# mrluin/TextualDegRemoval

Measured on AMD Instinct MI355X. Metric: train images/sec (512x512, bs=4/GPU), higher is better.
Workload: dtype f32 (3xbf16-split MFMA: 24-bit operand significands on the full fp32 exponent range, fp32 accumulate; unscaled gradients, no loss scale, no step-skip guard; tensors fp32 -- the MASA-encoder ResidualBlock activations / gradients as three bf16 planes whose sum IS the fp32 value, bit for bit)

## Files before the change

include/tdr.h:

```cpp
#ifndef TDR_H
#define TDR_H
#include <stdint.h>
#ifdef __cplusplus
extern "C" {
#endif

#define TDR_ABI_VERSION 112
int tdr_version(void);
const char* tdr_last_error(void);

typedef struct TdrStepGuard {
    float scale, inv_scale, max_scale;
    int good, growth_interval;
    int step, skipped, finite;
    float bc1, bc2_sqrt;
} TdrStepGuard;

typedef struct TdrConvDesc {
    int N, Cin, H, W;
    int Cout, OH, OW;
    int KH, stride, dil, pad;
    const float* in;  int64_t in_ns;
    int gate;
    const float* kscale; int64_t kscale_ns;
    const void* wp;  int64_t wp_ns;  int Mpad;
    int wp_fmt;
    float* out; int64_t out_ns;
    int epi;
    const float* bias;  int64_t bias_ns;
    const float* scale; int64_t scale_ns;
    const float* bias2; int64_t bias2_ns; float bias2_mul;
    const float* res;   int64_t res_ns;
    const float* mask;  int64_t mask_ns;
    const float* aux;   int64_t aux_ns;
    int relu;
} TdrConvDesc;

int tdr_conv_forward(const TdrConvDesc* d, void* stream);

int tdr_conv_ck(int KH_eff);
int64_t tdr_packed_weight_floats(int M, int Kch, int KH_eff);
int tdr_pack_weights(const float* w, int Cout, int Cin, int KH, int mode, float* wp, void* stream);
int64_t tdr_packed_weight_bytes_bx3(int M, int Kch, int KH_eff);
int tdr_pack_weights_bx3(const float* w, int Cout, int Cin, int KH, int mode, void* wp, void* stream);
int tdr_pack_weights_bx3_batch(const float* w, int64_t w_stride, int B, int Cout, int Cin, int KH, int mode, void* wp,
                               void* stream);
int64_t tdr_packed_weight_bytes_hx2(int M, int Kch, int KH_eff);
int tdr_pack_weights_hx2(const float* w, int Cout, int Cin, int KH, int mode, void* wp, void* stream);
int tdr_conv_force_cfg(int kh, int cfg);
int tdr_conv1x1_bx3_staged_set(int on);
int tdr_conv1x1_bx3_staged_takes(const TdrConvDesc* d);
typedef struct TdrPackJob {
    const float* w; void* wp;
    int Cout, Cin, KH, mode, fmt;
    int M, Kch, KHe, CK, Mx;
    int64_t total;
    int64_t first_block;
} TdrPackJob;
int tdr_pack_job_init(TdrPackJob* job, const float* w, int Cout, int Cin, int KH, int mode, int fmt, void* wp);
int tdr_pack_weights_multi(const TdrPackJob* jobs_dev, int n_jobs, int64_t total_blocks, void* stream);
int tdr_pack_patches(const float* blk, int B, int G, int C, int BH, int BW, int PH, int PW, int pstep, int dil,
                     int off, float* wp, void* stream);

typedef struct TdrConvP16Desc {
    int N, Cin, H, W, Cout;
    const void* in;
    const void* wp; int Mpad; int wp_fmt;
    const float* bias;
    const float* res32;  int64_t res32_ns;
    const void*  res16;
    const float* mask32; int64_t mask32_ns;
    const void*  mask16;
    int relu;
    float* out32; int64_t out32_ns;
    void*  out16;
} TdrConvP16Desc;
int64_t tdr_p16_bytes(int N, int C, int H, int W);
int tdr_p16_from_f32(const float* src, int64_t src_ns, int N, int C, int H, int W, void* dst, void* stream);
int tdr_p16_to_f32(const void* src, int N, int C, int H, int W, float* dst, int64_t dst_ns, void* stream);
int64_t tdr_p16_bytes_fmt(int N, int C, int H, int W, int fmt);
int tdr_p16_from_f32_fmt(const float* src, int64_t src_ns, int N, int C, int H, int W, void* dst, int fmt, void* stream);
int tdr_p16_to_f32_fmt(const void* src, int N, int C, int H, int W, float* dst, int64_t dst_ns, int fmt, void* stream);
int tdr_conv3x3_p16(const TdrConvP16Desc* d, void* stream);
int tdr_conv3x3_p16_force_cfg(int cfg);
typedef struct TdrWgradP16Desc {
    int N, Cin, H, W, Cout;
    const void* in16;
    const void* dout16;
    float* g;
    float* db;
    float* ws; int64_t ws_floats;
    int fmt;
} TdrWgradP16Desc;
int64_t tdr_wgrad3x3_p16_ws_floats(const TdrWgradP16Desc* d);
int tdr_wgrad3x3_p16(const TdrWgradP16Desc* d, void* stream);

typedef struct TdrWgradDesc {
    int N, Cin, H, W, Cout, OH, OW, KH, stride, pad;
    const float* in;   int64_t in_ns;  int gate;
    const float* dout; int64_t dout_ns;
    float* g;
    float* db;
    int per_image;
    float* ws; int64_t ws_floats;
    int math;
} TdrWgradDesc;
int64_t tdr_wgrad_ws_floats(const TdrWgradDesc* d);
int tdr_conv_wgrad(const TdrWgradDesc* d, void* stream);

typedef struct TdrWg1GroupEntry {
    const float* in; const float* dout; float* part; float* dbpart; float* g; float* db;
} TdrWg1GroupEntry;
int tdr_wgrad1x1_group_supported(const TdrWgradDesc* d);
int64_t tdr_wgrad1x1_group_ws_floats(const TdrWgradDesc* d, int nprob);
int tdr_wgrad1x1_group(const TdrWgradDesc* d, int nprob, const void* table, void* stream);

int64_t tdr_wgrad3x3_p16_group_ws_floats(const TdrWgradP16Desc* d, int nprob);
int tdr_wgrad3x3_p16_group_plan(const TdrWgradP16Desc* d, int nprob, int* nsplit, int* units, int* units_per_wg);
int tdr_wgrad3x3_p16_group(const TdrWgradP16Desc* d, int nprob, const void* table, void* stream);

int tdr_layernorm2d_fwd(const float* x, int64_t x_ns, const float* w, const float* b, float eps, int center,
                        int N, int C, int HW, float* y, float* mu, float* rstd, void* stream);
int64_t tdr_ln_ws_floats(int N, int C, int HW);
int tdr_layernorm2d_bwd(const float* go, const float* x, int64_t x_ns, const float* mu, const float* rstd,
                        const float* w, const float* add, int64_t add_ns, int add_C, int center,
                        int N, int C, int HW, float* gx, float* gw, float* gb, float* ws, void* stream);

int64_t tdr_dwsg_ws_floats(int N, int C, int H, int W);
int tdr_dwsg_fwd(const float* t, const float* w, const float* b, int N, int C, int H, int W,
                 float* g, float* pooled, float* ws, void* stream);
int tdr_dwsg_bwd(const float* dg, const float* t, const float* w, const float* b, int N, int C, int H, int W,
                 float* dt, float* dw, float* db, float* ws, void* stream);
int tdr_dwsg_bwd_biased(const float* dg, const float* dg_bias, float dg_bias_mul, const float* t, const float* w, const float* b,
                        int N, int C, int H, int W, float* dt, float* dw, float* db, float* ws, void* stream);
int tdr_dwsg_bwd_parts_supported(int W);
int tdr_dw_param_finish(const float* ws, int N, int C, int H, int W, float* dw , float* db , void* stream);

int tdr_dwgelu_fwd(const float* t, const float* w, const float* b, int N, int C, int H, int W, float* g, void* stream);
int tdr_dwgelu_bwd(const float* dg, const float* t, const float* w, const float* b, int N, int C, int H, int W,
                   float* dt, float* dw, float* db, float* ws, void* stream);
int tdr_dwconv_fwd(const float* t, const float* w, const float* b, int N, int planes, int H, int W, float* out,
                   void* stream);
int tdr_dwconv_bwd(const float* dout, const float* t, const float* w, int N, int planes, int H, int W, float* dt,
                   float* dw, float* db, float* ws, void* stream);
int tdr_dwconv_act_fwd(const float* t, const float* w, const float* b, int N, int planes, int H, int W, int relu, float* out,
                       void* stream);
int tdr_dwconv_act_bwd(const float* dout, const float* act, const float* t, const float* w, int N, int planes, int H, int W,
                       float* dt, float* dw, float* db, float* ws, void* stream);
int tdr_dwpair_fwd(const float* t, const float* w, const float* b, int N, int C, int H, int W, int relu, float* out,
                   int64_t out_ns, void* stream);
int tdr_dwpair_bwd(const float* dout, int64_t dout_ns, const float* act, int64_t act_ns, const float* t, const float* w, int N,
                   int C, int H, int W, float* dt, float* dw, float* db, float* ws, void* stream);
int tdr_dwconv_halves_fwd(const float* t, const float* w, const float* b, int N, int planes, int H, int W, int relu, float* outA,
                          float* outB, int64_t out_ns, void* stream);
int tdr_dwconv_halves_bwd(const float* doutA, const float* doutB, int64_t dout_ns, const float* actA, const float* actB,
                          int64_t act_ns, const float* t, const float* w, int N, int planes, int H, int W, float* dt, float* dw,
                          float* db, float* ws, void* stream);

int tdr_row_sumsq(const float* x, int64_t x_ns, int N, int rows, int HW, float* out, void* stream);
int tdr_mdta_pad(int C);
int tdr_mdta_softmax(const float* G, const float* ss, const float* temp, int N, int C, int heads, float* A, float* AT,
                     void* stream);
int tdr_mdta_bwd(const float* G, const float* ss, const float* temp, const float* A, const float* dA, int N, int C,
                 int heads, float* W, float* dtemp, float* ws, void* stream);
int tdr_attn_fold_proj(const float* AT, const float* Wo, int N, int C, int heads, float* Wf, void* stream);
int tdr_axpby_dev(const float* a, const float* alpha, const float* b, int64_t numel, float* out, void* stream);
int tdr_dot(const float* a, const float* b, int64_t numel, float* out, float* ws, void* stream);
int tdr_pixel_shuffle2(const float* in, int N, int C, int H, int W, float* out, void* stream);

int tdr_sca_fwd(const float* pooled, const float* wsca, const float* bsca, int N, int C, float* s, void* stream);
int tdr_sca_bwd(const float* G3, const float* S3, const float* w3, const float* b3, const float* beta,
                const float* s, const float* pooled, const float* wsca, int N, int C,
                float* dw3, float* db3, float* dbeta, float* dwsca, float* dbsca, float* dpooled,
                float* ws , void* stream);
int tdr_scaled_conv_param_grads(const float* G, const float* S, const float* w, const float* b,
                                const float* gamma, int Cout, int Cin, float* dw, float* db, float* dgamma,
                                void* stream);

int64_t tdr_chansum_ws_floats(int N, int C, int HW);
int tdr_channel_sum(const float* x, int64_t x_ns, int N, int C, int HW, float* out, float* ws, void* stream);

int tdr_copy_rows(const float* src, int64_t src_ns, float* dst, int64_t dst_ns, int N, int64_t len, void* stream);
int tdr_add_rows(const float* src, int64_t src_ns, float* dst, int64_t dst_ns, int N, int64_t len, void* stream);
int tdr_pixel_unshuffle2(const float* in, int N, int C, int H, int W, float* out, void* stream);
int tdr_pad_crop(const float* src, int N, int C, int Hs, int Ws, float* dst, int Hd, int Wd, void* stream);
int tdr_crop_augment(const float* src, int64_t src_ns, int N, int C, int Hs, int Ws, const int* top, const int* left,
                     const int* mode, const float* noise, const float* sigma, int P, float* out, void* stream);

int64_t tdr_ssim3d_ws_floats(int H, int W);
int tdr_ssim3d(const float* img1, const float* img2, int H, int W, int C, float max_value, float* ws, float* out,
               void* stream);

int64_t tdr_ssim_y64_ws_doubles(int H, int W);
int tdr_ssim_y64(const float* img1, const float* img2, int H, int W, double* ws, double* out, void* stream);

int64_t tdr_niqe_ws_floats(int H, int W);
int tdr_niqe_features(const float* y, int H, int W, int block, const double* window, const double* tables, int table_len,
                      float* ws, double* feats_out, void* stream);
int tdr_img_u8_to_planes(const uint8_t* img, int N, int H, int W, int C, int swap_rb, float* out, int Hp, int Wp, void* stream);
int tdr_planes_to_img_u8(const float* in, int N, int C, int Hp, int Wp, int swap_rb, uint8_t* img, int H, int W, void* stream);

int64_t tdr_local_avgpool_ws_floats(int planes, int H, int W, int k1);
int tdr_local_avgpool(const float* in, int planes, int H, int W, int k1, int k2, float* ws, float* out, void* stream);

int tdr_relu_bwd(const float* go, const float* act, int64_t numel, float* out, void* stream);

int tdr_l1_loss(const float* pred, const float* target, int64_t numel, float loss_weight, float grad_scale,
                float* loss, float* dpred, float* ws, void* stream);
int tdr_l1_loss_guarded(const float* pred, const float* target, int64_t numel, float loss_weight, const TdrStepGuard* guard,
                        float* loss, float* dpred, float* ws, void* stream);

int tdr_pixel_loss(int kind, const float* pred, const float* target, int N, int64_t chw, int64_t hw, float loss_weight, float eps,
                   float grad_scale, const TdrStepGuard* guard, float* loss, float* dpred, float* ws, void* stream);

int tdr_lr_blocks_fwd(const float* feat, int N, int C, int H, int W, int py, int px, int ky, int kx,
                      float* blk, void* stream);
int tdr_lr_blocks_bwd(const float* dblk, int N, int C, int H, int W, int py, int px, int ky, int kx,
                      float* dfeat, void* stream);
int tdr_patch_inv_norm(const float* x, int B, int C, int H, int W, int OH, int OW, int dil, int pad,
                       int step, int off, float* inv, void* stream);
int tdr_coarse_argmax_box(const float* dots, const float* invq, const float* invk, int ND, int N, int P, int Hr,
                          int Wr, int diameter, int* index, int* y1, int* x1, void* stream);
int tdr_gather_ref_block(const float* feat, int N, int C, int H, int W, const int* y1, const int* x1, int P,
                         int side, int s, float* out, void* stream);
int tdr_fine_argmax(const float* dots, const float* invq, const float* invk, int B, int P, int R,
                    int* index_all, float* soft_att, void* stream);
int tdr_fine_search_bwd(const float* datt, const float* soft_att, const int* index_all, const float* lrb,
                        const float* refb, const float* invq, const float* invk, int B, int C, int K, int D,
                        float* dlrb, float* drefb, void* stream);
int tdr_transfer_fwd(const float* feat, int N, int C, int H, int W, const int* y1, const int* x1,
                     const int* index_all, const float* soft_att, int py, int px, int K, int side, int s,
                     float* out, int64_t out_ns, void* stream);
int64_t tdr_transfer_ws_floats(int N, int C, int H, int W, int py, int px, int K, int s);
int tdr_transfer_bwd(const float* dout, int64_t dout_ns, const float* feat, int N, int C, int H, int W,
                     const int* y1, const int* x1, const int* index_all, const float* soft_att, int py, int px,
                     int K, int side, int s, int deterministic, float* dfeat, float* datt, float* ws, void* stream);
int tdr_scatter_ref_block(const float* dblk, int N, int C, int H, int W, const int* y1, const int* x1, int P,
                          int side, float* dfeat, void* stream);

int tdr_absmax_bits(const float* x, int64_t x_ns, int N, int64_t per, unsigned* slot, void* stream);

int tdr_tksa_softmax(const float* G, const float* ss, const float* temp, const float* am, const int* k4 , int N, int C,
                     int heads, float* A, float* AT, void* stream);
int tdr_tksa_bwd(const float* G, const float* ss, const float* temp, const float* am, const int* k4 , const float* dA, int N,
                 int C, int heads, float* W, float* dtemp, float* dam, float* ws, void* stream);
int tdr_dwk_fwd(const float* x, int64_t x_ns, const float* w, const float* b , int N, int Cout, int mult, int H, int W,
                int K, int dil , int relu, float* y, int64_t y_ns, void* stream);
int64_t tdr_dwk_bwd_ws_floats(int N, int Cout, int mult, int H, int W, int K);
int tdr_dwk_bwd(const float* dy, int64_t dy_ns, const float* yact, int64_t y_ns, const float* x, int64_t x_ns, const float* w, int N,
                int Cout, int mult, int H, int W, int K, int dil, float* dx, int64_t dx_ns, float* dw, float* db ,
                float* ws , void* stream);
int tdr_dwk_bwd_can_accumulate(int W, int K, int dil, int64_t dy_ns, int64_t y_ns, int64_t x_ns, int64_t dx_ns);
int tdr_dwk_bwd_acc(const float* dy, int64_t dy_ns, const float* yact, int64_t y_ns, const float* x, int64_t x_ns, const float* w,
                    int N, int Cout, int mult, int H, int W, int K, int dil, float* dx, int64_t dx_ns, int accumulate, float* dw,
                    float* db, float* ws, void* stream);
int tdr_avgpool3(const float* in, int planes, int H, int W, int adjoint, float* out, void* stream);
int tdr_add_relu(const float* a, const float* b, int64_t numel, float* out, void* stream);
int tdr_linear_small_fwd(const float* x, const float* W, const float* b, int N, int Cin, int Cout, int relu, float* y, void* stream);
int tdr_linear_small_bwd(const float* dy, const float* yact , const float* x, const float* W, int N, int Cin, int Cout,
                         float* dx, float* dW, float* db, void* stream);
int tdr_softmax_rows(const float* x, const float* dy , int rows, int L, float* out, void* stream);
int tdr_scale_copy(const float* src, int64_t src_ns, const float* w, int w_stride, int N, int64_t len, float* dst, int64_t dst_ns,
                   void* stream);
int tdr_rows_dot(const float* a, int64_t a_ns, const float* b, int64_t b_ns, int N, int64_t len, float* out, int out_stride, float* ws,
                 void* stream);

int tdr_plane_mean(const float* x, int64_t x_ns, int N, int C, int HW, float* out , void* stream);
int tdr_plane_add(float* x, int64_t x_ns, const float* v, float scale, int N, int C, int HW, void* stream);
int tdr_prompt_weights_fwd(const float* emb, const float* W , const float* b , int N, int C, int L,
                           float* w , void* stream);
int tdr_prompt_weights_bwd(const float* emb, const float* W, const float* w, const float* dw, int N, int C, int L,
                           float* dW, float* db , float* demb , void* stream);
int tdr_prompt_mix_fwd(const float* w, const float* P , int N, int L, int64_t E, float* out , void* stream);
int64_t tdr_prompt_mix_bwd_ws_floats(int N, int L);
int tdr_prompt_mix_bwd(const float* w, const float* P, const float* d , int N, int L, int64_t E, float* dP ,
                       float* dw , float* ws, void* stream);
int tdr_resize_bilinear_bwd(const float* ddst, int planes, int Hs, int Ws, int Hd, int Wd, float* dsrc, void* stream);

int tdr_resize_bilinear(const float* src, int planes, int Hs, int Ws, float* dst, int Hd, int Wd, void* stream);
int tdr_unfold_windows(const float* ref, int B, int C, int Hr, int Wr, int h, int stride, float* out, void* stream);
int tdr_patchify(const float* x, int B, int Ci, int H, int W, int p, int LD, int flat, float* out, void* stream);
int tdr_vit_assemble(float* tok, const float* cls, const float* pos, int B, int D, int T, int LD, int flat, void* stream);
int tdr_attention_fwd(const float* qkv, int B, int C, int heads, int T, int LD, float scale, float* out, void* stream);
int tdr_attention_fwd_math(const float* qkv, int B, int C, int heads, int T, int LD, float scale, int math, int flat,
                           float* out, void* stream);
int tdr_token_match(const float* fl, const float* fr, const float* windows, int B, int N, int D, int T1, int LD, int64_t per,
                    float* corr, int* index, float* ref_in, void* stream);

int tdr_transpose_f32(const float* src, int batch, int R, int C, float* dst, void* stream);
int tdr_tok_layernorm(const float* x, const float* w, const float* b, int64_t P, int D, float eps, int out_f16, void* out,
                      void* stream);
int tdr_tok16_gemm(const void* x16, const void* w16, const float* bias, int64_t P, int N, int K, int epi, void* y16, float* res,
                   const float* ls, void* stream);
int tdr_tok16x2_gemm(const void* x16x2, const void* w16x2, const float* bias, int64_t P, int N, int K, int epi, int act, void* y16x2,
                     float* out32, void* stream);
int tdr_cm_to_tok16x2(const float* src, int C, int64_t P, void* dst16x2, void* stream);
int tdr_tok16x3_gemm(const void* x16x3, const void* w16x3, const float* bias, int64_t P, int N, int K, int epi, int act, void* y16x3,
                     float* out32, const float* ls, void* stream);
int tdr_cm_to_tok16x3(const float* src, int C, int64_t P, void* dst16x3, void* stream);
int tdr_tok16_attention(const void* qkv16, int B, int C, int heads, int T, int LD, float scale, void* out16, void* stream);

int tdr_leaky_relu_fwd(const float* x, int64_t numel, float slope, float* y, void* stream);
int tdr_leaky_relu_bwd(const float* go, const float* y, int64_t numel, float slope, float* gx, void* stream);
int tdr_gather_col(const float* src, int B, int D, int LD, int col, float* dst, void* stream);
int tdr_mapper_combine(const float* cls, const float* patch, int B, int D, int LD, int T, int words, int word, float* out,
                       void* stream);
int tdr_mapper_combine_bwd(const float* go, int B, int D, int LD, int T, int words, int word, float* dcls, float* dpatch,
                           void* stream);
int tdr_cross_attention_fwd(const float* q, const float* k, const float* v, int B, int C, int heads, int Tq, int LDq,
                            int Tk, int LDk, float scale, float* out, float* lse, void* stream);
int tdr_cross_attention_bwd(const float* q, const float* k, const float* v, const float* out, const float* dout,
                            const float* lse, int B, int C, int heads, int Tq, int LDq, int Tk, int LDk, float scale,
                            float* dq, float* dk, float* dv, float* ws, void* stream);
int tdr_transpose_pad(const float* src, int B, int R, int C, int LDd, float* dst, void* stream);
int tdr_group_ln_act_fwd(const float* z, const float* w, const float* b, float eps, float slope, int G, int C, int P,
                         float* y, float* mu, float* rstd, void* stream);
int64_t tdr_group_ln_ws_floats(int G, int C, int P);
int tdr_group_ln_act_bwd(const float* dy, const float* y, const float* z, const float* mu, const float* rstd, const float* w,
                         float slope, int G, int C, int P, float* dz, float* gw, float* gb, float* gs, float* ws, void* stream);
int tdr_mapper_combine_all(const float* cls, const float* patch, int B, int G, int D, int LD, int T, float* out, void* stream);
int tdr_mapper_combine_all_bwd(const float* go, int B, int G, int D, int LD, int T, float* dcls, float* dpatch,
                               float* gsum , void* stream);
int tdr_gather_col_strided(const float* src, int B, int D, int64_t img_stride, int64_t ch_stride, int col, float* dst, void* stream);
int tdr_splitk_finish(const float* part, int S, int C, int64_t P, const float* bias, const float* scale, const float* res, int relu,
                      float* out, void* stream);
int tdr_text_inject_fwd(const int* ids, const float* tok_emb, const float* pos_emb, const float* inj, const int* idx,
                        int B, int S, int D, int L, int LD, float* out, void* stream);
int tdr_text_inject_bwd(const float* dnew, const int* idx, int B, int S, int D, int L, int LD, float* dinj, void* stream);
int tdr_add_noise(const float* x, const float* noise, const int* t, const float* alphas_cumprod, int B, int64_t per,
                  float* out, void* stream);
int tdr_pool_time(const float* x, const int* t, int B, int C, int H, int W, int f, float* out, void* stream);
int tdr_upsample_nearest_add(const float* src, int planes, int H, int W, int f, int accumulate, float* dst, void* stream);
int tdr_pool_sum(const float* src, int planes, int H, int W, int f, float* dst, void* stream);

int tdr_optim_chunk(void);
int tdr_multi_copy(const float* const* src, float* const* dst, const int64_t* sizes, const int* chunk_tensor,
                   const int* chunk_index, int n_chunks, float scale, void* stream);
int tdr_grad_sumsq(const float* const* grads, const int64_t* sizes, const int* chunk_tensor, const int* chunk_index,
                   int n_chunks, double* partial, double* sumsq, void* stream);
int tdr_adamw_step(float* const* params, const float* const* grads, float* const* exp_avg, float* const* exp_avg_sq,
                   const int64_t* sizes, const int* group, const int* chunk_tensor, const int* chunk_index, int n_chunks,
                   const double* sumsq, const float* group_lr, int n_groups, float max_norm, int use_clip, float beta1,
                   float beta2, float eps, float weight_decay, int step, void* stream);
int tdr_adamw_step_dev(float* const* params, const float* const* grads, float* const* exp_avg, float* const* exp_avg_sq,
                       const int64_t* sizes, const int* group, const int* chunk_tensor, const int* chunk_index, int n_chunks,
                       const double* sumsq, const float* hp, float max_norm, int use_clip, float beta1, float beta2,
                       float eps, float weight_decay, void* stream);
typedef struct TdrNafTailDesc {
    int N, C, HW, w_fmt;
    int c_out;
    float eps;
    const float* g;   int64_t g_ns;
    const float* sca;
    const float* x;   int64_t x_ns;
    const void *w3, *w4, *w5;
    const float *b3, *beta, *lnw, *lnb, *b4, *b5, *gamma;
    float* y;   int64_t y_ns;
    float *mu, *rs;
    float* yn;  int64_t yn_ns;
    float* t4;  int64_t t4_ns;
    float* out; int64_t out_ns;
} TdrNafTailDesc;
int tdr_naf_tail_supported(int C, int HW);
int tdr_naf_tail_fwd(const TdrNafTailDesc* d, void* stream);
int tdr_naf_tail_infer(const TdrNafTailDesc* d, void* stream);
typedef struct TdrNafTailLocalDesc {
    int N, C, HW, w_fmt;
    float eps;
    const float* g;    int64_t g_ns;
    const float* pool; int64_t pool_ns;
    const float* x;    int64_t x_ns;
    const void *wsca, *w3, *w4, *w5;
    const float *bsca, *b3, *beta, *lnw, *lnb, *b4, *b5, *gamma;
    float* out; int64_t out_ns;
} TdrNafTailLocalDesc;
int tdr_naf_tail_infer_local(const TdrNafTailLocalDesc* d, void* stream);
typedef struct TdrNafTailBwdDesc {
    int N, C, HW, w_fmt;
    int c_out;
    const float* dout; int64_t dout_ns;
    const float* gamma;
    const float* t4;   int64_t t4_ns;
    const float* y;    int64_t y_ns;
    const float *mu, *rs, *lnw;
    const void *w5t, *w4t;
    float* dt4; int64_t dt4_ns;
    float* dy;  int64_t dy_ns;
    float *gw, *gb;
    float* ws;
    const void* w3t; const float* beta; const float* sca ;
    float* dgp; int64_t dgp_ns;
} TdrNafTailBwdDesc;
int64_t tdr_naf_tail_bwd_ws_floats(int N, int C, int HW);
int tdr_naf_tail_bwd(const TdrNafTailBwdDesc* d, void* stream);
typedef struct TdrNafHeadFwdDesc {
    int N, C, HW, w_fmt;
    const float* x; int64_t x_ns;
    const float *lnw, *lnb; float eps;
    const void* w1; const float* b1;
    float *mu, *rs;
    float* xn; int64_t xn_ns;
    float* t1; int64_t t1_ns;
} TdrNafHeadFwdDesc;
int tdr_naf_head_fwd(const TdrNafHeadFwdDesc* d, void* stream);
int tdr_naf_head_infer(const TdrNafHeadFwdDesc* d, void* stream);
typedef struct TdrNafHeadBwdDesc {
    int N, C, HW, w_fmt;
    const float* dt1; int64_t dt1_ns;
    const float* x;   int64_t x_ns;
    const float *mu, *rs, *lnw;
    const void* w1t;
    const float* res; int64_t res_ns;
    float* dx; int64_t dx_ns;
    float *gw, *gb;
    float* ws;
} TdrNafHeadBwdDesc;
int tdr_naf_head_bwd(const TdrNafHeadBwdDesc* d, void* stream);
int64_t tdr_pair_sum_mid_floats(int nparts, int C);
int tdr_pair_sum_partials(const float* part, int nparts, int C, float* o0, float* o1, float* mid, void* stream);
int tdr_pair_sum_partials_multi(const void* table, int nprob, int max_C, void* stream);
int tdr_dw_param_finish_nb(int H, int W);
int tdr_dw_param_finish_multi(const void* table, int nprob, int max_C, void* stream);
int tdr_scaled_conv_param_grads_multi(const void* table, int nprob, int max_Cout, void* stream);

typedef struct TdrComm TdrComm;
int tdr_comm_available(void);
int tdr_comm_unique_id_bytes(void);
int tdr_comm_unique_id(void* id_out);
int tdr_comm_init(TdrComm** comm, int rank, int world, const void* unique_id);
int tdr_comm_allreduce(TdrComm* comm, float* buf, int64_t count, int average, void* stream);
int tdr_comm_reduce(TdrComm* comm, float* buf, int64_t count, int root, void* stream);
int tdr_comm_broadcast(TdrComm* comm, float* buf, int64_t count, int root, void* stream);
int tdr_comm_rank(const TdrComm* comm);
int tdr_comm_world(const TdrComm* comm);
int tdr_comm_destroy(TdrComm* comm);

int tdr_multi_ema(const float* const* src, float* const* dst, const int64_t* sizes, const int* chunk_tensor,
                  const int* chunk_index, int n_chunks, float decay, void* stream);
int tdr_multi_copy_guarded(const float* const* src, float* const* dst, const int64_t* sizes, const int* chunk_tensor,
                           const int* chunk_index, int n_chunks, const TdrStepGuard* guard, void* stream);
int tdr_grad_sumsq_guarded(const float* const* grads, const int64_t* sizes, const int* group, const int* chunk_tensor,
                           const int* chunk_index, int n_chunks, double* partial, double* sumsq, TdrStepGuard* guard,
                           float beta1, float beta2, void* stream);
int tdr_adamw_step_guarded(float* const* params, const float* const* grads, float* const* exp_avg, float* const* exp_avg_sq,
                           const int64_t* sizes, const int* group, const int* chunk_tensor, const int* chunk_index,
                           int n_chunks, const double* sumsq, const float* hp, const TdrStepGuard* guard, float max_norm,
                           int use_clip, int coupled_decay, float beta1, float beta2, float eps, float weight_decay,
                           void* stream);

int tdr_gelu_fwd(const float* x, const float* bias, int C, int HW, float* z_out, float* y, int64_t n, void* stream);
int tdr_gelu_bwd(const float* dy, const float* z, float* dz, int64_t n, void* stream);
int tdr_subsample2(const float* x, int planes, int H, int W, float* y, void* stream);
int tdr_instnorm_fwd(const float* x, const float* w, const float* b, float eps, int N, int C, int HW, float* y, float* mu, float* rs, void* stream);
int tdr_instnorm_bwd(const float* dy, const float* x, const float* mu, const float* rs, const float* w, int N, int C, int HW, float* dx,
                     float* dw, float* db, float* ws, void* stream);
int tdr_region_affine_fwd(const float* x, int64_t x_ns, const float* ph, const float* pl, float shift, int q, int N, int C, int H, int W,
                          float* y, int64_t y_ns, float* mean, void* stream);
int tdr_region_affine_bwd(const float* dy, int64_t dy_ns, const float* x, int64_t x_ns, const float* ph, const float* pl, float shift,
                          const float* mean, int q, int N, int C, int H, int W, float* dx, int64_t dx_ns, float* dph, float* dpl, float* ws,
                          void* stream);
typedef struct TdrSfDynVecDesc {
    int N, c, GK, KK, d;
    float eps, momentum;
    const float *ap, *wconv, *bn_w, *bn_b, *fc_w, *fc_b, *f0_w, *f0_b, *f1_w, *f1_b;
    float *run_mean, *run_var; int64_t* nbt;
    float *taps, *ah, *al, *xhat, *rstd, *z, *att;
    int use_running;
} TdrSfDynVecDesc;
int tdr_sf_dyn_vec_fwd(const TdrSfDynVecDesc* d, void* stream);
typedef struct TdrSfDynVecBwdDesc {
    int N, c, GK, KK, d;
    const float *ap, *wconv, *bn_w, *fc_w, *f0_w, *f1_w, *taps, *xhat, *rstd, *z, *att, *dtaps, *dah, *dal;
    float *dap, *g_wconv, *g_bn_w, *g_bn_b, *g_fc_w, *g_fc_b, *g_f0_w, *g_f0_b, *g_f1_w, *g_f1_b;
    float* ws;
} TdrSfDynVecBwdDesc;
int tdr_sf_dyn_vec_bwd(const TdrSfDynVecBwdDesc* d, void* stream);
int tdr_sf_dynfilt_fwd(const float* x, int64_t x_ns, const float* taps, const float* ah, const float* al, int N, int C, int groups, int H,
                       int W, int k, float* low, float* mix, void* stream);
int tdr_sf_dynfilt_bwd_reduce(const float* dmix, const float* x, int64_t x_ns, const float* low, const float* ah, const float* al, int N, int C,
                              int groups, int H, int W, int k, float* dah, float* dal, float* dtaps, void* stream);
int tdr_sf_dynfilt_bwd_dx(const float* dmix, const float* taps, const float* ah, const float* al, const float* dap, int N, int C, int groups,
                          int H, int W, int k, float* dx, int64_t dx_ns, void* stream);
int tdr_convt4_weight_to_3x3(const float* w, const float* b, int Cin, int Cout, float* w3, float* b4, void* stream);
int tdr_convt4_grad_from_3x3(const float* dw3, const float* db4, int Cin, int Cout, float* dw, float* db, void* stream);
int tdr_sf_region_split(const float* x, int64_t x_ns, int q, int N, int C, int H, int W, float* out, void* stream);
int tdr_sf_local_affine(const float* x, int64_t x_ns, const float* m, const float* ph, const float* pl, float shift, int q, int N, int C, int H, int W,
                        float* y, int64_t y_ns, void* stream);
int tdr_sf_emerge(const float* x, int64_t x_ns, const float* low, int N, int C, int HW, float* out, void* stream);
int tdr_sf_softmax_mix(const float* x, int64_t x_ns, const float* low, const float* lh, const float* ll, int N, int C, int HW, float* mix, void* stream);

int tdr_kvproj_tile_rows(void);
int tdr_kvproj_fwd(const void* table, int nseg, int64_t ntiles, const float* kv, int N, int K, float* out, int64_t ld, void* stream);
int tdr_kvproj_wgrad(const void* table, const void* gtable, int nseg, int64_t ntiles, const float* kv, const float* dk, int64_t ld, int N,
                     int K, void* stream);
int tdr_kvproj_dkv_parts(int64_t ntiles);
int64_t tdr_kvproj_dkv_ws_floats(int64_t ntiles, int N, int K);
int tdr_kvproj_dkv(const void* table, int nseg, int64_t ntiles, const float* dk, int64_t ld, int N, int K, float* dkv, float* ws,
                   void* stream);
int tdr_modln_fwd(const float* x, const float* a, const float* b, int64_t ab_ns, const float* w, const float* lb, float eps, int N, int C,
                  int HW, float* y, float* mu, float* rstd, void* stream);
int tdr_nc_affine(const float* x, const float* a, const float* b, int64_t ab_ns, int N, int C, int HW, float* y, void* stream);
int tdr_nc_affine_bwd(const float* dm, const float* x, const float* a, int64_t ab_ns, const float* add, int N, int C, int HW, float* dx,
                      float* da, float* db, int64_t d_ns, void* stream);
int tdr_modgate_fwd(const float* t, const float* a, const float* b, int64_t ab_ns, int N, int c, int HW, float* g, float* pooled,
                    void* stream);
int tdr_modgate_bwd(const float* dg, const float* dgb, float dgb_mul, const float* t, const float* a, const float* b, int64_t ab_ns, int N,
                    int c, int HW, float* dt, float* da, float* db, int64_t d_ns, void* stream);
typedef struct TdrDynHeadDesc {
    int N, C, HW, w_fmt;
    const float* x; int64_t x_ns;
    const float *a0, *b0; int64_t ab_ns;
    const float *lnw, *lnb; float eps;
    const void* w1; const float* b1;
    float* t1; int64_t t1_ns;
} TdrDynHeadDesc;
int tdr_dyn_head_infer(const TdrDynHeadDesc* d, void* stream);
typedef struct TdrDynDwsgDesc {
    int N, C, H, W;
    const float* t;
    const float *w, *b;
    const float *a1, *b1; int64_t ab_ns;
    float* g;
    float* pooled;
    float* ws;
} TdrDynDwsgDesc;
int64_t tdr_dyn_dwsg_ws_floats(int N, int C, int H, int W);
int tdr_dyn_dwsg_fwd(const TdrDynDwsgDesc* d, void* stream);
typedef struct TdrDynTailDesc {
    int N, C, HW, w_fmt;
    float eps;
    const float* g;   int64_t g_ns;
    const float* sca;
    const float* x;   int64_t x_ns;
    const void *w3, *w4, *w5;
    const float *b3, *beta, *lnw, *lnb, *b4, *b5, *gamma;
    const float *a2, *b2; int64_t ab_ns;
    float* out; int64_t out_ns;
} TdrDynTailDesc;
int tdr_dyn_tail_infer(const TdrDynTailDesc* d, void* stream);
// ... 6 lines not shown
```

textualdegremoval_amd/_lib.py:

```python
import ctypes as C
import os

import torch

_HERE = os.path.dirname(os.path.abspath(__file__))
LIB_PATH = os.environ.get('TDR_LIB_PATH', os.path.join(_HERE, 'libtdr_hip.so'))

ABI_VERSION = 112
c_fp = C.c_void_p
i32, i64, f32 = C.c_int, C.c_int64, C.c_float


class TdrConvDesc(C.Structure):
    _fields_ = [
        ('N', i32), ('Cin', i32), ('H', i32), ('W', i32),
        ('Cout', i32), ('OH', i32), ('OW', i32),
        ('KH', i32), ('stride', i32), ('dil', i32), ('pad', i32),
        ('inp', c_fp), ('in_ns', i64),
        ('gate', i32),
        ('kscale', c_fp), ('kscale_ns', i64),
        ('wp', c_fp), ('wp_ns', i64), ('Mpad', i32), ('wp_fmt', i32),
        ('out', c_fp), ('out_ns', i64),
        ('epi', i32),
        ('bias', c_fp), ('bias_ns', i64),
        ('scale', c_fp), ('scale_ns', i64),
        ('bias2', c_fp), ('bias2_ns', i64), ('bias2_mul', f32),
        ('res', c_fp), ('res_ns', i64),
        ('mask', c_fp), ('mask_ns', i64),
        ('aux', c_fp), ('aux_ns', i64),
        ('relu', i32),
    ]


class TdrConvP16Desc(C.Structure):
    _fields_ = [
        ('N', i32), ('Cin', i32), ('H', i32), ('W', i32), ('Cout', i32),
        ('inp', c_fp),
        ('wp', c_fp), ('Mpad', i32), ('wp_fmt', i32),
        ('bias', c_fp),
        ('res32', c_fp), ('res32_ns', i64),
        ('res16', c_fp),
        ('mask32', c_fp), ('mask32_ns', i64),
        ('mask16', c_fp),
        ('relu', i32),
        ('out32', c_fp), ('out32_ns', i64),
        ('out16', c_fp),
    ]


class TdrWgradP16Desc(C.Structure):
    _fields_ = [('N', i32), ('Cin', i32), ('H', i32), ('W', i32), ('Cout', i32),
                ('in16', c_fp), ('dout16', c_fp), ('g', c_fp), ('db', c_fp), ('ws', c_fp), ('ws_floats', i64), ('fmt', i32)]


class TdrPackJob(C.Structure):
    _fields_ = [
        ('w', c_fp), ('wp', c_fp),
        ('Cout', i32), ('Cin', i32), ('KH', i32), ('mode', i32), ('fmt', i32),
        ('M', i32), ('Kch', i32), ('KHe', i32), ('CK', i32), ('Mx', i32),
        ('total', i64), ('first_block', i64),
    ]


class TdrWgradDesc(C.Structure):
    _fields_ = [
        ('N', i32), ('Cin', i32), ('H', i32), ('W', i32), ('Cout', i32), ('OH', i32), ('OW', i32),
        ('KH', i32), ('stride', i32), ('pad', i32),
        ('inp', c_fp), ('in_ns', i64), ('gate', i32),
        ('dout', c_fp), ('dout_ns', i64),
        ('g', c_fp),
        ('db', c_fp),
        ('per_image', i32),
        ('ws', c_fp), ('ws_floats', i64),
        ('math', i32),
    ]


class TdrNafTailDesc(C.Structure):
    _fields_ = [('N', i32), ('C', i32), ('HW', i32), ('w_fmt', i32), ('c_out', i32), ('eps', f32),
                ('g', c_fp), ('g_ns', i64), ('sca', c_fp), ('x', c_fp), ('x_ns', i64),
                ('w3', c_fp), ('w4', c_fp), ('w5', c_fp),
                ('b3', c_fp), ('beta', c_fp), ('lnw', c_fp), ('lnb', c_fp), ('b4', c_fp), ('b5', c_fp), ('gamma', c_fp),
                ('y', c_fp), ('y_ns', i64), ('mu', c_fp), ('rs', c_fp), ('yn', c_fp), ('yn_ns', i64),
                ('t4', c_fp), ('t4_ns', i64), ('out', c_fp), ('out_ns', i64)]


class TdrNafTailLocalDesc(C.Structure):
    _fields_ = [('N', i32), ('C', i32), ('HW', i32), ('w_fmt', i32), ('eps', f32),
                ('g', c_fp), ('g_ns', i64), ('pool', c_fp), ('pool_ns', i64), ('x', c_fp), ('x_ns', i64),
                ('wsca', c_fp), ('w3', c_fp), ('w4', c_fp), ('w5', c_fp),
                ('bsca', c_fp), ('b3', c_fp), ('beta', c_fp), ('lnw', c_fp), ('lnb', c_fp), ('b4', c_fp), ('b5', c_fp), ('gamma', c_fp),
                ('out', c_fp), ('out_ns', i64)]


class TdrNafTailBwdDesc(C.Structure):
    _fields_ = [('N', i32), ('C', i32), ('HW', i32), ('w_fmt', i32), ('c_out', i32),
                ('dout', c_fp), ('dout_ns', i64), ('gamma', c_fp), ('t4', c_fp), ('t4_ns', i64), ('y', c_fp), ('y_ns', i64),
                ('mu', c_fp), ('rs', c_fp), ('lnw', c_fp), ('w5t', c_fp), ('w4t', c_fp),
                ('dt4', c_fp), ('dt4_ns', i64), ('dy', c_fp), ('dy_ns', i64), ('gw', c_fp), ('gb', c_fp), ('ws', c_fp),
                ('w3t', c_fp), ('beta', c_fp), ('sca', c_fp), ('dgp', c_fp), ('dgp_ns', i64)]


class TdrNafHeadBwdDesc(C.Structure):
    _fields_ = [('N', i32), ('C', i32), ('HW', i32), ('w_fmt', i32),
                ('dt1', c_fp), ('dt1_ns', i64), ('x', c_fp), ('x_ns', i64), ('mu', c_fp), ('rs', c_fp), ('lnw', c_fp),
                ('w1t', c_fp), ('res', c_fp), ('res_ns', i64), ('dx', c_fp), ('dx_ns', i64), ('gw', c_fp), ('gb', c_fp), ('ws', c_fp)]


class TdrNafHeadFwdDesc(C.Structure):
    _fields_ = [('N', i32), ('C', i32), ('HW', i32), ('w_fmt', i32),
                ('x', c_fp), ('x_ns', i64), ('lnw', c_fp), ('lnb', c_fp), ('eps', f32), ('w1', c_fp), ('b1', c_fp),
                ('mu', c_fp), ('rs', c_fp), ('xn', c_fp), ('xn_ns', i64), ('t1', c_fp), ('t1_ns', i64)]


class TdrDynHeadDesc(C.Structure):
    _fields_ = [('N', i32), ('C', i32), ('HW', i32), ('w_fmt', i32),
                ('x', c_fp), ('x_ns', i64), ('a0', c_fp), ('b0', c_fp), ('ab_ns', i64), ('lnw', c_fp), ('lnb', c_fp), ('eps', f32),
                ('w1', c_fp), ('b1', c_fp), ('t1', c_fp), ('t1_ns', i64)]


class TdrDynDwsgDesc(C.Structure):
    _fields_ = [('N', i32), ('C', i32), ('H', i32), ('W', i32),
                ('t', c_fp), ('w', c_fp), ('b', c_fp), ('a1', c_fp), ('b1', c_fp), ('ab_ns', i64), ('g', c_fp), ('pooled', c_fp), ('ws', c_fp)]


class TdrDynTailDesc(C.Structure):
    _fields_ = [('N', i32), ('C', i32), ('HW', i32), ('w_fmt', i32), ('eps', f32),
                ('g', c_fp), ('g_ns', i64), ('sca', c_fp), ('x', c_fp), ('x_ns', i64),
                ('w3', c_fp), ('w4', c_fp), ('w5', c_fp),
                ('b3', c_fp), ('beta', c_fp), ('lnw', c_fp), ('lnb', c_fp), ('b4', c_fp), ('b5', c_fp), ('gamma', c_fp),
                ('a2', c_fp), ('b2', c_fp), ('ab_ns', i64), ('out', c_fp), ('out_ns', i64)]


class TdrSfDynVecDesc(C.Structure):
    _fields_ = [('N', i32), ('c', i32), ('GK', i32), ('KK', i32), ('d', i32), ('eps', f32), ('momentum', f32)] + \
               [(k, c_fp) for k in ('ap', 'wconv', 'bn_w', 'bn_b', 'fc_w', 'fc_b', 'f0_w', 'f0_b', 'f1_w', 'f1_b', 'run_mean', 'run_var', 'nbt',
                                    'taps', 'ah', 'al', 'xhat', 'rstd', 'z', 'att')] + [('use_running', i32)]


class TdrSfDynVecBwdDesc(C.Structure):
    _fields_ = [('N', i32), ('c', i32), ('GK', i32), ('KK', i32), ('d', i32)] + \
               [(k, c_fp) for k in ('ap', 'wconv', 'bn_w', 'fc_w', 'f0_w', 'f1_w', 'taps', 'xhat', 'rstd', 'z', 'att', 'dtaps', 'dah', 'dal',
                                    'dap', 'g_wconv', 'g_bn_w', 'g_bn_b', 'g_fc_w', 'g_fc_b', 'g_f0_w', 'g_f0_b', 'g_f1_w', 'g_f1_b', 'ws')]


class TdrStepGuard(C.Structure):
    _fields_ = [('scale', f32), ('inv_scale', f32), ('max_scale', f32), ('good', i32), ('growth_interval', i32),
                ('step', i32), ('skipped', i32), ('finite', i32), ('bc1', f32), ('bc2_sqrt', f32)]


SIGNATURES = {
    'tdr_version': (i32, []),
    'tdr_last_error': (C.c_char_p, []),
    'tdr_conv_forward': (i32, [C.POINTER(TdrConvDesc), c_fp]),
    'tdr_conv_ck': (i32, [i32]),
    'tdr_ssim_y64_ws_doubles': (i64, [i32, i32]),
    'tdr_ssim_y64': (i32, [c_fp, c_fp, i32, i32, c_fp, c_fp, c_fp]),
    'tdr_local_avgpool_ws_floats': (i64, [i32, i32, i32, i32]),
    'tdr_local_avgpool': (i32, [c_fp, i32, i32, i32, i32, i32, c_fp, c_fp, c_fp]),
    'tdr_p16_bytes': (i64, [i32, i32, i32, i32]),
    'tdr_p16_bytes_fmt': (i64, [i32, i32, i32, i32, i32]),
    'tdr_p16_from_f32_fmt': (i32, [c_fp, i64, i32, i32, i32, i32, c_fp, i32, c_fp]),
    'tdr_p16_to_f32_fmt': (i32, [c_fp, i32, i32, i32, i32, c_fp, i64, i32, c_fp]),
    'tdr_p16_from_f32': (i32, [c_fp, i64, i32, i32, i32, i32, c_fp, c_fp]),
    'tdr_p16_to_f32': (i32, [c_fp, i32, i32, i32, i32, c_fp, i64, c_fp]),
    'tdr_conv3x3_p16': (i32, [C.POINTER(TdrConvP16Desc), c_fp]),
    'tdr_conv3x3_p16_force_cfg': (i32, [i32]),
    'tdr_wgrad3x3_p16_ws_floats': (i64, [C.POINTER(TdrWgradP16Desc)]),
    'tdr_wgrad3x3_p16': (i32, [C.POINTER(TdrWgradP16Desc), c_fp]),
    'tdr_packed_weight_floats': (i64, [i32, i32, i32]),
    'tdr_pack_weights': (i32, [c_fp, i32, i32, i32, i32, c_fp, c_fp]),
    'tdr_packed_weight_bytes_bx3': (i64, [i32, i32, i32]),
    'tdr_pack_weights_bx3': (i32, [c_fp, i32, i32, i32, i32, c_fp, c_fp]),
    'tdr_pack_job_init': (i32, [C.POINTER(TdrPackJob), c_fp, i32, i32, i32, i32, i32, c_fp]),
    'tdr_pack_weights_multi': (i32, [c_fp, i32, i64, c_fp]),
    'tdr_pack_patches': (i32, [c_fp, i32, i32, i32, i32, i32, i32, i32, i32, i32, i32, c_fp, c_fp]),
    'tdr_wgrad_ws_floats': (i64, [C.POINTER(TdrWgradDesc)]),
    'tdr_conv_wgrad': (i32, [C.POINTER(TdrWgradDesc), c_fp]),
    'tdr_wgrad1x1_group_supported': (i32, [C.POINTER(TdrWgradDesc)]),
    'tdr_wgrad1x1_group_ws_floats': (i64, [C.POINTER(TdrWgradDesc), i32]),
    'tdr_wgrad1x1_group': (i32, [C.POINTER(TdrWgradDesc), i32, c_fp, c_fp]),
    'tdr_wgrad3x3_p16_group_ws_floats': (i64, [C.POINTER(TdrWgradP16Desc), i32]),
    'tdr_wgrad3x3_p16_group_plan': (i32, [C.POINTER(TdrWgradP16Desc), i32, C.POINTER(i32), C.POINTER(i32), C.POINTER(i32)]),
    'tdr_wgrad3x3_p16_group': (i32, [C.POINTER(TdrWgradP16Desc), i32, c_fp, c_fp]),
    'tdr_layernorm2d_fwd': (i32, [c_fp, i64, c_fp, c_fp, f32, i32, i32, i32, i32, c_fp, c_fp, c_fp, c_fp]),
    'tdr_ln_ws_floats': (i64, [i32, i32, i32]),
    'tdr_layernorm2d_bwd': (i32, [c_fp, c_fp, i64, c_fp, c_fp, c_fp, c_fp, i64, i32, i32, i32, i32, i32, c_fp, c_fp, c_fp,
                                  c_fp, c_fp]),
    'tdr_dwsg_ws_floats': (i64, [i32, i32, i32, i32]),
    'tdr_dwsg_fwd': (i32, [c_fp, c_fp, c_fp, i32, i32, i32, i32, c_fp, c_fp, c_fp, c_fp]),
    'tdr_dwsg_bwd': (i32, [c_fp, c_fp, c_fp, c_fp, i32, i32, i32, i32, c_fp, c_fp, c_fp, c_fp, c_fp]),
    'tdr_dwsg_bwd_biased': (i32, [c_fp, c_fp, f32, c_fp, c_fp, c_fp, i32, i32, i32, i32, c_fp, c_fp, c_fp, c_fp, c_fp]),
    'tdr_dwsg_bwd_parts_supported': (i32, [i32]),
    'tdr_dw_param_finish': (i32, [c_fp, i32, i32, i32, i32, c_fp, c_fp, c_fp]),
    'tdr_dwgelu_fwd': (i32, [c_fp, c_fp, c_fp, i32, i32, i32, i32, c_fp, c_fp]),
    'tdr_dwgelu_bwd': (i32, [c_fp, c_fp, c_fp, c_fp, i32, i32, i32, i32, c_fp, c_fp, c_fp, c_fp, c_fp]),
    'tdr_dwconv_fwd': (i32, [c_fp, c_fp, c_fp, i32, i32, i32, i32, c_fp, c_fp]),
    'tdr_dwconv_act_fwd': (i32, [c_fp, c_fp, c_fp, i32, i32, i32, i32, i32, c_fp, c_fp]),
    'tdr_dwconv_act_bwd': (i32, [c_fp, c_fp, c_fp, c_fp, i32, i32, i32, i32, c_fp, c_fp, c_fp, c_fp, c_fp]),
    'tdr_dwpair_fwd': (i32, [c_fp, c_fp, c_fp, i32, i32, i32, i32, i32, c_fp, i64, c_fp]),
    'tdr_dwpair_bwd': (i32, [c_fp, i64, c_fp, i64, c_fp, c_fp, i32, i32, i32, i32, c_fp, c_fp, c_fp, c_fp, c_fp]),
    'tdr_dwconv_halves_fwd': (i32, [c_fp, c_fp, c_fp, i32, i32, i32, i32, i32, c_fp, c_fp, i64, c_fp]),
    'tdr_dwconv_halves_bwd': (i32, [c_fp, c_fp, i64, c_fp, c_fp, i64, c_fp, c_fp, i32, i32, i32, i32, c_fp, c_fp, c_fp, c_fp, c_fp]),
    'tdr_dwconv_bwd': (i32, [c_fp, c_fp, c_fp, i32, i32, i32, i32, c_fp, c_fp, c_fp, c_fp, c_fp]),
    'tdr_row_sumsq': (i32, [c_fp, i64, i32, i32, i32, c_fp, c_fp]),
    'tdr_mdta_pad': (i32, [i32]),
    'tdr_mdta_softmax': (i32, [c_fp, c_fp, c_fp, i32, i32, i32, c_fp, c_fp, c_fp]),
    'tdr_mdta_bwd': (i32, [c_fp, c_fp, c_fp, c_fp, c_fp, i32, i32, i32, c_fp, c_fp, c_fp, c_fp]),
    'tdr_attn_fold_proj': (i32, [c_fp, c_fp, i32, i32, i32, c_fp, c_fp]),
    'tdr_axpby_dev': (i32, [c_fp, c_fp, c_fp, i64, c_fp, c_fp]),
    'tdr_dot': (i32, [c_fp, c_fp, i64, c_fp, c_fp, c_fp]),
    'tdr_pixel_shuffle2': (i32, [c_fp, i32, i32, i32, i32, c_fp, c_fp]),
    'tdr_leaky_relu_fwd': (i32, [c_fp, i64, f32, c_fp, c_fp]),
    'tdr_leaky_relu_bwd': (i32, [c_fp, c_fp, i64, f32, c_fp, c_fp]),
    'tdr_gather_col': (i32, [c_fp, i32, i32, i32, i32, c_fp, c_fp]),
    'tdr_mapper_combine': (i32, [c_fp, c_fp, i32, i32, i32, i32, i32, i32, c_fp, c_fp]),
    'tdr_mapper_combine_bwd': (i32, [c_fp, i32, i32, i32, i32, i32, i32, c_fp, c_fp, c_fp]),
    'tdr_cross_attention_fwd': (i32, [c_fp, c_fp, c_fp, i32, i32, i32, i32, i32, i32, i32, f32, c_fp, c_fp, c_fp]),
    'tdr_cross_attention_bwd': (i32, [c_fp, c_fp, c_fp, c_fp, c_fp, c_fp, i32, i32, i32, i32, i32, i32, i32, f32, c_fp, c_fp,
                                      c_fp, c_fp, c_fp]),
    'tdr_transpose_pad': (i32, [c_fp, i32, i32, i32, i32, c_fp, c_fp]),
    'tdr_conv_force_cfg': (i32, [i32, i32]),
    'tdr_conv1x1_bx3_staged_set': (i32, [i32]),
    'tdr_conv1x1_bx3_staged_takes': (i32, [C.POINTER(TdrConvDesc)]),
    'tdr_packed_weight_bytes_hx2': (i64, [i32, i32, i32]),
    'tdr_pack_weights_hx2': (i32, [c_fp, i32, i32, i32, i32, c_fp, c_fp]),
    'tdr_pack_weights_bx3_batch': (i32, [c_fp, i64, i32, i32, i32, i32, i32, c_fp, c_fp]),
    'tdr_sca_fwd': (i32, [c_fp, c_fp, c_fp, i32, i32, c_fp, c_fp]),
    'tdr_sca_bwd': (i32, [c_fp] * 8 + [i32, i32] + [c_fp] * 7 + [c_fp]),
    'tdr_gelu_fwd': (i32, [c_fp, c_fp, i32, i32, c_fp, c_fp, i64, c_fp]),
    'tdr_gelu_bwd': (i32, [c_fp, c_fp, c_fp, i64, c_fp]),
    'tdr_subsample2': (i32, [c_fp, i32, i32, i32, c_fp, c_fp]),
    'tdr_instnorm_fwd': (i32, [c_fp, c_fp, c_fp, f32, i32, i32, i32, c_fp, c_fp, c_fp, c_fp]),
    'tdr_instnorm_bwd': (i32, [c_fp] * 5 + [i32, i32, i32] + [c_fp] * 5),
    'tdr_region_affine_fwd': (i32, [c_fp, i64, c_fp, c_fp, f32, i32, i32, i32, i32, i32, c_fp, i64, c_fp, c_fp]),
    'tdr_region_affine_bwd': (i32, [c_fp, i64, c_fp, i64, c_fp, c_fp, f32, c_fp, i32, i32, i32, i32, i32, c_fp, i64, c_fp, c_fp, c_fp, c_fp]),
    'tdr_sf_dyn_vec_fwd': (i32, [C.POINTER(TdrSfDynVecDesc), c_fp]),
    'tdr_sf_dyn_vec_bwd': (i32, [C.POINTER(TdrSfDynVecBwdDesc), c_fp]),
    'tdr_sf_dynfilt_fwd': (i32, [c_fp, i64, c_fp, c_fp, c_fp, i32, i32, i32, i32, i32, i32, c_fp, c_fp, c_fp]),
    'tdr_sf_dynfilt_bwd_reduce': (i32, [c_fp, c_fp, i64, c_fp, c_fp, c_fp, i32, i32, i32, i32, i32, i32, c_fp, c_fp, c_fp, c_fp]),
    'tdr_sf_dynfilt_bwd_dx': (i32, [c_fp] * 5 + [i32] * 6 + [c_fp, i64, c_fp]),
    'tdr_convt4_weight_to_3x3': (i32, [c_fp, c_fp, i32, i32, c_fp, c_fp, c_fp]),
    'tdr_convt4_grad_from_3x3': (i32, [c_fp, c_fp, i32, i32, c_fp, c_fp, c_fp]),
    'tdr_sf_region_split': (i32, [c_fp, i64, i32, i32, i32, i32, i32, c_fp, c_fp]),
    'tdr_sf_local_affine': (i32, [c_fp, i64, c_fp, c_fp, c_fp, f32, i32, i32, i32, i32, i32, c_fp, i64, c_fp]),
    'tdr_sf_emerge': (i32, [c_fp, i64, c_fp, i32, i32, i32, c_fp, c_fp]),
    'tdr_sf_softmax_mix': (i32, [c_fp, i64, c_fp, c_fp, c_fp, i32, i32, i32, c_fp, c_fp]),
    'tdr_scaled_conv_param_grads': (i32, [c_fp] * 5 + [i32, i32] + [c_fp] * 3 + [c_fp]),
    'tdr_pair_sum_partials_multi': (i32, [c_fp, i32, i32, c_fp]),
    'tdr_dw_param_finish_nb': (i32, [i32, i32]),
    'tdr_dw_param_finish_multi': (i32, [c_fp, i32, i32, c_fp]),
    'tdr_scaled_conv_param_grads_multi': (i32, [c_fp, i32, i32, c_fp]),
    'tdr_chansum_ws_floats': (i64, [i32, i32, i32]),
    'tdr_channel_sum': (i32, [c_fp, i64, i32, i32, i32, c_fp, c_fp, c_fp]),
    'tdr_copy_rows': (i32, [c_fp, i64, c_fp, i64, i32, i64, c_fp]),
    'tdr_add_rows': (i32, [c_fp, i64, c_fp, i64, i32, i64, c_fp]),
    'tdr_pixel_unshuffle2': (i32, [c_fp, i32, i32, i32, i32, c_fp, c_fp]),
    'tdr_pad_crop': (i32, [c_fp, i32, i32, i32, i32, c_fp, i32, i32, c_fp]),
    'tdr_relu_bwd': (i32, [c_fp, c_fp, i64, c_fp, c_fp]),
    'tdr_l1_loss': (i32, [c_fp, c_fp, i64, f32, f32, c_fp, c_fp, c_fp, c_fp]),
    'tdr_lr_blocks_fwd': (i32, [c_fp] + [i32] * 8 + [c_fp, c_fp]),
    'tdr_lr_blocks_bwd': (i32, [c_fp] + [i32] * 8 + [c_fp, c_fp]),
    'tdr_patch_inv_norm': (i32, [c_fp] + [i32] * 10 + [c_fp, c_fp]),
    'tdr_coarse_argmax_box': (i32, [c_fp, c_fp, c_fp] + [i32] * 6 + [c_fp, c_fp, c_fp, c_fp]),
    'tdr_gather_ref_block': (i32, [c_fp, i32, i32, i32, i32, c_fp, c_fp, i32, i32, i32, c_fp, c_fp]),
    'tdr_scatter_ref_block': (i32, [c_fp, i32, i32, i32, i32, c_fp, c_fp, i32, i32, c_fp, c_fp]),
    'tdr_fine_argmax': (i32, [c_fp, c_fp, c_fp, i32, i32, i32, c_fp, c_fp, c_fp]),
    'tdr_fine_search_bwd': (i32, [c_fp] * 7 + [i32] * 4 + [c_fp, c_fp, c_fp]),
    'tdr_transfer_fwd': (i32, [c_fp, i32, i32, i32, i32, c_fp, c_fp, c_fp, c_fp, i32, i32, i32, i32, i32, c_fp, i64, c_fp]),
    'tdr_transfer_ws_floats': (i64, [i32, i32, i32, i32, i32, i32, i32, i32]),
    'tdr_transfer_bwd': (i32, [c_fp, i64, c_fp, i32, i32, i32, i32, c_fp, c_fp, c_fp, c_fp, i32, i32, i32, i32, i32, i32,
                               c_fp, c_fp, c_fp, c_fp]),
    'tdr_resize_bilinear': (i32, [c_fp, i32, i32, i32, c_fp, i32, i32, c_fp]),
    'tdr_unfold_windows': (i32, [c_fp, i32, i32, i32, i32, i32, i32, c_fp, c_fp]),
    'tdr_patchify': (i32, [c_fp, i32, i32, i32, i32, i32, i32, i32, c_fp, c_fp]),
    'tdr_vit_assemble': (i32, [c_fp, c_fp, c_fp, i32, i32, i32, i32, i32, c_fp]),
    'tdr_attention_fwd_math': (i32, [c_fp, i32, i32, i32, i32, i32, f32, i32, i32, c_fp, c_fp]),
    'tdr_attention_fwd': (i32, [c_fp, i32, i32, i32, i32, i32, f32, c_fp, c_fp]),
    'tdr_token_match': (i32, [c_fp, c_fp, c_fp, i32, i32, i32, i32, i32, i64, c_fp, c_fp, c_fp, c_fp]),
    'tdr_transpose_f32': (i32, [c_fp, i32, i32, i32, c_fp, c_fp]),
    'tdr_tok_layernorm': (i32, [c_fp, c_fp, c_fp, i64, i32, f32, i32, c_fp, c_fp]),
    'tdr_tok16_gemm': (i32, [c_fp, c_fp, c_fp, i64, i32, i32, i32, c_fp, c_fp, c_fp, c_fp]),
    'tdr_tok16x2_gemm': (i32, [c_fp, c_fp, c_fp, i64, i32, i32, i32, i32, c_fp, c_fp, c_fp]),
    'tdr_cm_to_tok16x2': (i32, [c_fp, i32, i64, c_fp, c_fp]),
    'tdr_tok16x3_gemm': (i32, [c_fp, c_fp, c_fp, i64, i32, i32, i32, i32, c_fp, c_fp, c_fp, c_fp]),
    'tdr_cm_to_tok16x3': (i32, [c_fp, i32, i64, c_fp, c_fp]),
    'tdr_tok16_attention': (i32, [c_fp, i32, i32, i32, i32, i32, f32, c_fp, c_fp]),
    'tdr_optim_chunk': (i32, []),
    'tdr_multi_copy': (i32, [c_fp, c_fp, c_fp, c_fp, c_fp, i32, f32, c_fp]),
    'tdr_grad_sumsq': (i32, [c_fp, c_fp, c_fp, c_fp, i32, c_fp, c_fp, c_fp]),
    'tdr_adamw_step': (i32, [c_fp] * 8 + [i32, c_fp, C.POINTER(f32), i32, f32, i32, f32, f32, f32, f32, i32, c_fp]),
    'tdr_adamw_step_dev': (i32, [c_fp] * 8 + [i32, c_fp, c_fp, f32, i32, f32, f32, f32, f32, c_fp]),
    'tdr_naf_tail_supported': (i32, [i32, i32]),
    'tdr_naf_tail_fwd': (i32, [C.POINTER(TdrNafTailDesc), c_fp]),
    'tdr_naf_tail_bwd_ws_floats': (i64, [i32, i32, i32]),
    'tdr_naf_tail_bwd': (i32, [C.POINTER(TdrNafTailBwdDesc), c_fp]),
    'tdr_naf_head_bwd': (i32, [C.POINTER(TdrNafHeadBwdDesc), c_fp]),
    'tdr_naf_head_fwd': (i32, [C.POINTER(TdrNafHeadFwdDesc), c_fp]),
    'tdr_naf_tail_infer': (i32, [C.POINTER(TdrNafTailDesc), c_fp]),
    'tdr_naf_head_infer': (i32, [C.POINTER(TdrNafHeadFwdDesc), c_fp]),
    'tdr_naf_tail_infer_local': (i32, [C.POINTER(TdrNafTailLocalDesc), c_fp]),
    'tdr_absmax_bits': (i32, [c_fp, i64, i32, i64, c_fp, c_fp]),
    'tdr_pair_sum_partials': (i32, [c_fp, i32, i32, c_fp, c_fp, c_fp, c_fp]),
    'tdr_pair_sum_mid_floats': (i64, [i32, i32]),
    'tdr_tksa_softmax': (i32, [c_fp, c_fp, c_fp, c_fp, C.POINTER(i32), i32, i32, i32, c_fp, c_fp, c_fp]),
    'tdr_tksa_bwd': (i32, [c_fp, c_fp, c_fp, c_fp, C.POINTER(i32), c_fp, i32, i32, i32, c_fp, c_fp, c_fp, c_fp, c_fp]),
    'tdr_dwk_fwd': (i32, [c_fp, i64, c_fp, c_fp, i32, i32, i32, i32, i32, i32, i32, i32, c_fp, i64, c_fp]),
    'tdr_dwk_bwd_can_accumulate': (i32, [i32, i32, i32, i64, i64, i64, i64]),
    'tdr_dwk_bwd_acc': (i32, [c_fp, i64, c_fp, i64, c_fp, i64, c_fp, i32, i32, i32, i32, i32, i32, i32, c_fp, i64, i32, c_fp, c_fp, c_fp, c_fp]),
    'tdr_dwk_bwd': (i32, [c_fp, i64, c_fp, i64, c_fp, i64, c_fp, i32, i32, i32, i32, i32, i32, i32, c_fp, i64, c_fp, c_fp, c_fp, c_fp]),
    'tdr_avgpool3': (i32, [c_fp, i32, i32, i32, i32, c_fp, c_fp]),
    'tdr_add_relu': (i32, [c_fp, c_fp, i64, c_fp, c_fp]),
    'tdr_linear_small_fwd': (i32, [c_fp, c_fp, c_fp, i32, i32, i32, i32, c_fp, c_fp]),
    'tdr_linear_small_bwd': (i32, [c_fp, c_fp, c_fp, c_fp, i32, i32, i32, c_fp, c_fp, c_fp, c_fp]),
    'tdr_softmax_rows': (i32, [c_fp, c_fp, i32, i32, c_fp, c_fp]),
    'tdr_scale_copy': (i32, [c_fp, i64, c_fp, i32, i32, i64, c_fp, i64, c_fp]),
    'tdr_rows_dot': (i32, [c_fp, i64, c_fp, i64, i32, i64, c_fp, i32, c_fp, c_fp]),
    'tdr_dwk_bwd_ws_floats': (i64, [i32, i32, i32, i32, i32, i32]),
    'tdr_crop_augment': (i32, [c_fp, i64, i32, i32, i32, i32, c_fp, c_fp, c_fp, c_fp, c_fp, i32, c_fp, c_fp]),
    'tdr_ssim3d_ws_floats': (i64, [i32, i32]),
    'tdr_ssim3d': (i32, [c_fp, c_fp, i32, i32, i32, f32, c_fp, c_fp, c_fp]),
    'tdr_plane_mean': (i32, [c_fp, i64, i32, i32, i32, c_fp, c_fp]),
    'tdr_plane_add': (i32, [c_fp, i64, c_fp, f32, i32, i32, i32, c_fp]),
    'tdr_prompt_weights_fwd': (i32, [c_fp, c_fp, c_fp, i32, i32, i32, c_fp, c_fp]),
    'tdr_prompt_weights_bwd': (i32, [c_fp, c_fp, c_fp, c_fp, i32, i32, i32, c_fp, c_fp, c_fp, c_fp]),
    'tdr_prompt_mix_fwd': (i32, [c_fp, c_fp, i32, i32, i64, c_fp, c_fp]),
    'tdr_prompt_mix_bwd_ws_floats': (i64, [i32, i32]),
    'tdr_prompt_mix_bwd': (i32, [c_fp, c_fp, c_fp, i32, i32, i64, c_fp, c_fp, c_fp, c_fp]),
    'tdr_resize_bilinear_bwd': (i32, [c_fp, i32, i32, i32, i32, i32, c_fp, c_fp]),
    'tdr_group_ln_act_fwd': (i32, [c_fp, c_fp, c_fp, f32, f32, i32, i32, i32, c_fp, c_fp, c_fp, c_fp]),
    'tdr_group_ln_ws_floats': (i64, [i32, i32, i32]),
    'tdr_group_ln_act_bwd': (i32, [c_fp, c_fp, c_fp, c_fp, c_fp, c_fp, f32, i32, i32, i32, c_fp, c_fp, c_fp, c_fp, c_fp, c_fp]),
    'tdr_mapper_combine_all': (i32, [c_fp, c_fp, i32, i32, i32, i32, i32, c_fp, c_fp]),
    'tdr_mapper_combine_all_bwd': (i32, [c_fp, i32, i32, i32, i32, i32, c_fp, c_fp, c_fp, c_fp]),
    'tdr_gather_col_strided': (i32, [c_fp, i32, i32, i64, i64, i32, c_fp, c_fp]),
    'tdr_splitk_finish': (i32, [c_fp, i32, i32, i64, c_fp, c_fp, c_fp, i32, c_fp, c_fp]),
    'tdr_text_inject_fwd': (i32, [c_fp, c_fp, c_fp, c_fp, c_fp, i32, i32, i32, i32, i32, c_fp, c_fp]),
    'tdr_text_inject_bwd': (i32, [c_fp, c_fp, i32, i32, i32, i32, i32, c_fp, c_fp]),
    'tdr_add_noise': (i32, [c_fp, c_fp, c_fp, c_fp, i32, i64, c_fp, c_fp]),
    'tdr_pool_time': (i32, [c_fp, c_fp, i32, i32, i32, i32, i32, c_fp, c_fp]),
    'tdr_upsample_nearest_add': (i32, [c_fp, i32, i32, i32, i32, i32, c_fp, c_fp]),
    'tdr_pool_sum': (i32, [c_fp, i32, i32, i32, i32, c_fp, c_fp]),
    'tdr_comm_available': (i32, []),
    'tdr_comm_unique_id_bytes': (i32, []),
    'tdr_comm_unique_id': (i32, [c_fp]),
    'tdr_comm_init': (i32, [C.POINTER(c_fp), i32, i32, c_fp]),
    'tdr_comm_allreduce': (i32, [c_fp, c_fp, i64, i32, c_fp]),
    'tdr_comm_reduce': (i32, [c_fp, c_fp, i64, i32, c_fp]),
    'tdr_comm_broadcast': (i32, [c_fp, c_fp, i64, i32, c_fp]),
    'tdr_comm_rank': (i32, [c_fp]),
    'tdr_comm_world': (i32, [c_fp]),
    'tdr_comm_destroy': (i32, [c_fp]),
    'tdr_multi_ema': (i32, [c_fp, c_fp, c_fp, c_fp, c_fp, i32, f32, c_fp]),
    'tdr_pixel_loss': (i32, [i32, c_fp, c_fp, i32, i64, i64, f32, f32, f32, c_fp, c_fp, c_fp, c_fp, c_fp]),
    'tdr_l1_loss_guarded': (i32, [c_fp, c_fp, i64, f32, c_fp, c_fp, c_fp, c_fp, c_fp]),
    'tdr_multi_copy_guarded': (i32, [c_fp, c_fp, c_fp, c_fp, c_fp, i32, c_fp, c_fp]),
    'tdr_grad_sumsq_guarded': (i32, [c_fp] * 5 + [i32, c_fp, c_fp, c_fp, f32, f32, c_fp]),
    'tdr_adamw_step_guarded': (i32, [c_fp] * 8 + [i32, c_fp, c_fp, c_fp, f32, i32, i32, f32, f32, f32, f32, c_fp]),
    'tdr_kvproj_tile_rows': (i32, []),
    'tdr_kvproj_fwd': (i32, [c_fp, i32, i64, c_fp, i32, i32, c_fp, i64, c_fp]),
    'tdr_kvproj_wgrad': (i32, [c_fp, c_fp, i32, i64, c_fp, c_fp, i64, i32, i32, c_fp]),
    'tdr_kvproj_dkv_parts': (i32, [i64]),
    'tdr_kvproj_dkv_ws_floats': (i64, [i64, i32, i32]),
    'tdr_kvproj_dkv': (i32, [c_fp, i32, i64, c_fp, i64, i32, i32, c_fp, c_fp, c_fp]),
    'tdr_modln_fwd': (i32, [c_fp, c_fp, c_fp, i64, c_fp, c_fp, f32, i32, i32, i32, c_fp, c_fp, c_fp, c_fp]),
    'tdr_nc_affine': (i32, [c_fp, c_fp, c_fp, i64, i32, i32, i32, c_fp, c_fp]),
    'tdr_nc_affine_bwd': (i32, [c_fp, c_fp, c_fp, i64, c_fp, i32, i32, i32, c_fp, c_fp, c_fp, i64, c_fp]),
    'tdr_modgate_fwd': (i32, [c_fp, c_fp, c_fp, i64, i32, i32, i32, c_fp, c_fp, c_fp]),
    'tdr_dyn_head_infer': (i32, [C.POINTER(TdrDynHeadDesc), c_fp]),
    'tdr_dyn_dwsg_ws_floats': (i64, [i32, i32, i32, i32]),
    'tdr_dyn_dwsg_fwd': (i32, [C.POINTER(TdrDynDwsgDesc), c_fp]),
    'tdr_dyn_tail_infer': (i32, [C.POINTER(TdrDynTailDesc), c_fp]),
    'tdr_modgate_bwd': (i32, [c_fp, c_fp, f32, c_fp, c_fp, c_fp, i64, i32, i32, i32, c_fp, c_fp, c_fp, i64, c_fp]),
    'tdr_niqe_ws_floats': (i64, [i32, i32]),
    'tdr_niqe_features': (i32, [c_fp, i32, i32, i32, c_fp, c_fp, i32, c_fp, c_fp, c_fp]),
    'tdr_img_u8_to_planes': (i32, [c_fp, i32, i32, i32, i32, i32, c_fp, i32, i32, c_fp]),
    'tdr_planes_to_img_u8': (i32, [c_fp, i32, i32, i32, i32, i32, c_fp, i32, i32, c_fp]),
}

_lib = None


class TdrError(RuntimeError):
    pass


def load():
    global _lib
    if _lib is not None:
        return _lib
    if not os.path.exists(LIB_PATH):
        raise TdrError(f'{LIB_PATH} is missing: build it first (python -c "import __graft_entry__ as g; g.build()"). '
                       'There is no CPU fallback on the product path.')
    lib = C.CDLL(LIB_PATH)
    for name, (res, args) in SIGNATURES.items():
        fn = getattr(lib, name)
        fn.restype = res
        fn.argtypes = args
    have = lib.tdr_version()
    if have != ABI_VERSION:
        raise TdrError(f'{LIB_PATH} exports C-ABI version {have}, this package binds version {ABI_VERSION}: a stale build would be '
                       'called with shifted arguments -- rebuild it (python -c "import __graft_entry__ as g; g.build()")')
    _lib = lib
    return lib


def check(rc, what):
    if rc != 0:
        msg = load().tdr_last_error().decode('utf-8', 'replace')
        raise TdrError(f'{what} failed (code {rc}): {msg}')
```

textualdegremoval_amd/csrc/tdr_masa.hip:

```cpp
#include "tdr_common.h"
#include "../../include/tdr.h"

namespace {

__device__ __forceinline__ int wrap_idx(int v, int n) { return v < 0 ? v + n : v; }

__global__ void lr_blocks_fwd_kernel(const float* __restrict__ feat, int C, int H, int W, int py, int px, int ky, int kx,
                                     long total, float* __restrict__ blk) {
    const int BH = ky + 2, BW = kx + 2;
    for (long i = blockIdx.x * (long)blockDim.x + threadIdx.x; i < total; i += (long)gridDim.x * blockDim.x) {
        const int u = (int)(i % BW); long r = i / BW;
        const int v = (int)(r % BH); r /= BH;
        const int c = (int)(r % C); r /= C;
        const int p = (int)(r % (py * px)); const long n = r / (py * px);
        const int by = p / px, bx = p % px;
        const int y = min(max(by * ky + v - 1, 0), H - 1), x = min(max(bx * kx + u - 1, 0), W - 1);
        blk[i] = feat[((n * C + c) * H + y) * W + x];
    }
}

__global__ void lr_blocks_bwd_kernel(const float* __restrict__ dblk, int C, int H, int W, int py, int px, int ky, int kx,
                                     long total, float* __restrict__ dfeat) {
    const int BH = ky + 2, BW = kx + 2, P = py * px;
    for (long i = blockIdx.x * (long)blockDim.x + threadIdx.x; i < total; i += (long)gridDim.x * blockDim.x) {
        const int x = (int)(i % W); long r = i / W;
        const int y = (int)(r % H); r /= H;
        const int c = (int)(r % C); const long n = r / C;
        float s = 0.f;
        for (int Y = (y == 0 ? 0 : y + 1); Y <= (y == H - 1 ? H + 1 : y + 1); ++Y) {
            for (int X = (x == 0 ? 0 : x + 1); X <= (x == W - 1 ? W + 1 : x + 1); ++X) {
                for (int by = max(0, (Y - 2) / ky - 1); by < py && by * ky <= Y; ++by) {
                    const int v = Y - by * ky;
                    if (v < 0 || v >= BH) continue;
                    for (int bx = max(0, (X - 2) / kx - 1); bx < px && bx * kx <= X; ++bx) {
                        const int u = X - bx * kx;
                        if (u < 0 || u >= BW) continue;
                        s += dblk[(((n * P + by * px + bx) * C + c) * BH + v) * BW + u];
                    }
                }
            }
        }
        dfeat[i] = s;
    }
}

__global__ __launch_bounds__(1024) void patch_inv_norm_kernel(const float* __restrict__ x, int C, int H, int W, int OH,
                                                             int OW, int dil, int step, int off, long npos,
                                                             float* __restrict__ inv) {
    __shared__ float red[16][64];
    const int lane = threadIdx.x & 63, sl = threadIdx.x >> 6;
    const long pos = blockIdx.x * 64L + lane;
    const bool live = pos < npos;
    const long pc = live ? pos : npos - 1;
    const int ox = (int)(pc % OW); const long r = pc / OW;
    const int oy = (int)(r % OH); const long b = r / OH;
    int offs[9];
#pragma unroll
    for (int k = 0; k < 9; ++k) {
        const int yy = oy * step + off + (k / 3) * dil, xx = ox * step + off + (k % 3) * dil;
        offs[k] = (yy >= 0 && yy < H && xx >= 0 && xx < W) ? yy * W + xx : -1;
    }
    float s = 0.f;
    const long HW = (long)H * W;
    for (int c = sl; c < C; c += 16) {
        const float* xc = x + (b * C + c) * HW;
#pragma unroll
        for (int k = 0; k < 9; ++k) {
            const float v = offs[k] >= 0 ? xc[offs[k]] : 0.f;
            s += v * v;
        }
    }
    red[sl][lane] = s;
    __syncthreads();
    if (sl == 0 && live) {
        float t = 0.f;
#pragma unroll
        for (int q = 0; q < 16; ++q) t += red[q][lane];
        inv[pos] = 1.0f / fmaxf(sqrtf(t), 1e-12f);
    }
}

__global__ __launch_bounds__(256) void patch_inv_norm_wave_kernel(const float* __restrict__ x, int C, int H, int W, int OH,
                                                                 int OW, int dil, int step, int off, long npos,
                                                                 float* __restrict__ inv) {
    const long pos = blockIdx.x * 4L + (threadIdx.x >> 6);
    if (pos >= npos) return;
    const int lane = threadIdx.x & 63;
    const int ox = (int)(pos % OW); long r = pos / OW;
    const int oy = (int)(r % OH); const long b = r / OH;
    float s = 0.f;
    for (int c = lane; c < C; c += 64) {
        const float* xc = x + (b * C + c) * (long)H * W;
#pragma unroll
        for (int k = 0; k < 9; ++k) {
            const int yy = oy * step + off + (k / 3) * dil, xx = ox * step + off + (k % 3) * dil;
            if (yy >= 0 && yy < H && xx >= 0 && xx < W) {
                const float v = xc[(long)yy * W + xx];
                s += v * v;
            }
        }
    }
    s = wave_sum(s);
    if (lane == 0) inv[pos] = 1.0f / fmaxf(sqrtf(s), 1e-12f);
}

__device__ __forceinline__ int box_start(int idx, int size, int diameter) {
    int lo = idx - diameter / 2 - 1, hi = idx + diameter / 2 + 1;
    if (lo < 0) { lo = 0; hi = diameter + 1; }
    if (hi > size - 1) { hi = size - 1; lo = hi - (diameter + 1); }
    return lo;
}

__global__ __launch_bounds__(256) void coarse_argmax_box_kernel(const float* __restrict__ dots,
                                                               const float* __restrict__ invq,
                                                               const float* __restrict__ invk, int ND, int N, int P,
                                                               int Hr, int Wr, int diameter, int* __restrict__ index,
                                                               int* __restrict__ y1, int* __restrict__ x1) {
    __shared__ float sv[256];
    __shared__ int si[256];
    const int np = blockIdx.x, n = np / P;
    const int R = Hr * Wr;
    float best = -INFINITY; int bi = 0x7fffffff;
    for (int r = threadIdx.x; r < R; r += 256) {
        float s = 0.f;
        for (int d = 0; d < ND; ++d)
            s += dots[((long)d * N * P + np) * R + r] * invq[(long)d * N * P + np] * invk[((long)d * N + n) * R + r];
        if (s > best) { best = s; bi = r; }
    }
    sv[threadIdx.x] = best; si[threadIdx.x] = bi;
    __syncthreads();
    for (int o = 128; o > 0; o >>= 1) {
        if (threadIdx.x < o) {
            const float v2 = sv[threadIdx.x + o]; const int i2 = si[threadIdx.x + o];
            if (v2 > sv[threadIdx.x] || (v2 == sv[threadIdx.x] && i2 < si[threadIdx.x])) { sv[threadIdx.x] = v2; si[threadIdx.x] = i2; }
        }
        __syncthreads();
    }
    if (threadIdx.x == 0) {
        const int idx = si[0];
        index[np] = idx;
        x1[np] = box_start(idx % Wr, Wr, diameter);
        y1[np] = box_start(idx / Wr, Hr, diameter);
    }
}

__global__ void gather_ref_block_kernel(const float* __restrict__ feat, int C, int H, int W, const int* __restrict__ y1,
                                        const int* __restrict__ x1, int P, int side, int s, long total,
                                        float* __restrict__ out) {
    const int SS = side * s;
    for (long i = blockIdx.x * (long)blockDim.x + threadIdx.x; i < total; i += (long)gridDim.x * blockDim.x) {
        const int u = (int)(i % SS); long r = i / SS;
        const int v = (int)(r % SS); r /= SS;
        const int c = (int)(r % C); const long b = r / C;
        const long n = b / P;
        const int y = wrap_idx(y1[b] * s + v, H), x = wrap_idx(x1[b] * s + u, W);
        out[i] = feat[((n * C + c) * H + y) * W + x];
    }
}

__global__ void scatter_ref_block_kernel(const float* __restrict__ dblk, int C, int H, int W, const int* __restrict__ y1,
                                         const int* __restrict__ x1, int P, int side, long total,
                                         float* __restrict__ dfeat) {
    for (long i = blockIdx.x * (long)blockDim.x + threadIdx.x; i < total; i += (long)gridDim.x * blockDim.x) {
        const int x = (int)(i % W); long r = i / W;
        const int y = (int)(r % H); r /= H;
        const int c = (int)(r % C); const long n = r / C;
        float acc = 0.f;
        for (int p = 0; p < P; ++p) {
            const long b = n * P + p;
            const int by = y1[b], bx = x1[b];
#pragma unroll
            for (int wy = 0; wy < 2; ++wy) {
                const int v = y - wy * H - by;
                if (v < 0 || v >= side || (wy == 1) != (by + v < 0)) continue;
#pragma unroll
                for (int wx = 0; wx < 2; ++wx) {
                    const int u = x - wx * W - bx;
                    if (u < 0 || u >= side || (wx == 1) != (bx + u < 0)) continue;
                    acc += dblk[((b * C + c) * side + v) * side + u];
                }
            }
        }
        dfeat[i] += acc;
    }
}

__global__ __launch_bounds__(256) void fine_argmax_kernel(const float* __restrict__ dots, const float* __restrict__ invq,
                                                         const float* __restrict__ invk, long rows, int P, int R,
                                                         int* __restrict__ index_all, float* __restrict__ soft_att) {
    const long row = blockIdx.x * 4L + (threadIdx.x >> 6);
    if (row >= rows) return;
    const int lane = threadIdx.x & 63;
    const long b = row / P;
    const float iq = invq[row];
    float best = -INFINITY; int bi = 0x7fffffff;
    for (int r = lane; r < R; r += 64) {
        const float v = dots[row * R + r] * iq * invk[b * R + r];
        if (v > best) { best = v; bi = r; }
    }
#pragma unroll
    for (int o = 32; o > 0; o >>= 1) {
        const float v2 = __shfl_xor(best, o, 64); const int i2 = __shfl_xor(bi, o, 64);
        if (v2 > best || (v2 == best && i2 < bi)) { best = v2; bi = i2; }
    }
    if (lane == 0) { index_all[row] = bi; soft_att[row] = best; }
}

__global__ __launch_bounds__(256) void fine_search_bwd_kernel(const float* __restrict__ datt,
                                                             const float* __restrict__ soft_att,
                                                             const int* __restrict__ index_all,
                                                             const float* __restrict__ lrb, const float* __restrict__ refb,
                                                             const float* __restrict__ invq, const float* __restrict__ invk,
                                                             int C, int K, int D, float* __restrict__ dlrb,
                                                             float* __restrict__ drefb) {
    extern __shared__ float sm[];
    const int b = blockIdx.y, c = blockIdx.x;
    const int P = K * K, BS = K + 2, R1 = D - 2;
    float* s_da = sm;
    float* s_at = s_da + P;
    float* s_iq = s_at + P;
    float* s_ik = s_iq + P;
    int* s_ix = reinterpret_cast<int*>(s_ik + P);
    float* s_q = reinterpret_cast<float*>(s_ix + P);
    float* s_k = s_q + BS * BS;
    int* s_ry = reinterpret_cast<int*>(s_k + D * D);
    int* s_rx = s_ry + P;
    int* s_qo = s_rx + P;
    for (int p = threadIdx.x; p < P; p += 256) {
        const int ix = index_all[(long)b * P + p];
        s_da[p] = datt[(long)b * P + p];
        s_at[p] = soft_att[(long)b * P + p];
        s_iq[p] = invq[(long)b * P + p];
        s_ik[p] = invk[(long)b * R1 * R1 + ix];
        s_ix[p] = ix;
        s_ry[p] = ix / R1;
        s_rx[p] = ix % R1;
        s_qo[p] = (p / K) * BS + (p % K);
    }
    for (int i = threadIdx.x; i < BS * BS; i += 256) s_q[i] = lrb[((long)b * C + c) * BS * BS + i];
    for (int i = threadIdx.x; i < D * D; i += 256) s_k[i] = refb[((long)b * C + c) * D * D + i];
    __syncthreads();
    for (int i = threadIdx.x; i < BS * BS; i += 256) {
        const int y = i / BS, x = i % BS;
        float s = 0.f;
#pragma unroll
        for (int k = 0; k < 9; ++k) {
            const int pyy = y - k / 3, pxx = x - k % 3;
            if (pyy < 0 || pyy >= K || pxx < 0 || pxx >= K) continue;
            const int p = pyy * K + pxx;
            const int ry = s_ry[p], rx = s_rx[p];
            const float kv = s_k[(ry + k / 3) * D + rx + k % 3];
            s += s_da[p] * s_iq[p] * (kv * s_ik[p] - s_at[p] * s_q[i] * s_iq[p]);
        }
        dlrb[((long)b * C + c) * BS * BS + i] = s;
    }
    for (int i = threadIdx.x; i < D * D; i += 256) {
        const int v = i / D, u = i % D;
        float s = 0.f;
        for (int p = 0; p < P; ++p) {
            const int kyy = v - s_ry[p], kxx = u - s_rx[p];
            if (kyy < 0 || kyy > 2 || kxx < 0 || kxx > 2) continue;
            const float qv = s_q[s_qo[p] + kyy * BS + kxx];
            s += s_da[p] * s_ik[p] * (qv * s_iq[p] - s_at[p] * s_k[i] * s_ik[p]);
        }
        drefb[((long)b * C + c) * D * D + i] = s;
    }
}

struct TrGeom {
    int src[9];
    float wgt;
    float inv_cnt;
    int a00, a01, a10, a11; float w00, w01, w10, w11;
};

__device__ __forceinline__ void tr_geometry(int Yl, int Xl, int b, const int* __restrict__ y1, const int* __restrict__ x1,
                                            const int* __restrict__ index_all, const float* __restrict__ soft_att, int K,
                                            int side, int s, int H, int W, TrGeom& g) {
    const int R1 = side - 2;
    const int i0 = Yl / s, j0 = Xl / s;
    int cnt = 0;
#pragma unroll
    for (int k = 0; k < 9; ++k) {
        const int i = i0 + k / 3 - 1, j = j0 + k % 3 - 1;
        g.src[k] = -1;
        if (i < 0 || i >= K || j < 0 || j >= K) continue;
        const int idx = index_all[(long)b * K * K + i * K + j];
        const int ry = idx / R1, rx = idx % R1;
        const int sy = ry * s + Yl - i * s + s, sx = rx * s + Xl - j * s + s;
        const int gy = wrap_idx(y1[b] * s + sy, H), gx = wrap_idx(x1[b] * s + sx, W);
        g.src[k] = gy * W + gx;
        ++cnt;
    }
    g.inv_cnt = 1.0f / (float)cnt;
    const float fy = fmaxf(((float)Yl + 0.5f) / (float)s - 0.5f, 0.f), fx = fmaxf(((float)Xl + 0.5f) / (float)s - 0.5f, 0.f);
    const int yy0 = min((int)fy, K - 1), xx0 = min((int)fx, K - 1);
    const int yy1 = min(yy0 + 1, K - 1), xx1 = min(xx0 + 1, K - 1);
    const float ly = fy - (float)yy0, lx = fx - (float)xx0;
    g.a00 = yy0 * K + xx0; g.a01 = yy0 * K + xx1; g.a10 = yy1 * K + xx0; g.a11 = yy1 * K + xx1;
    g.w00 = (1.f - ly) * (1.f - lx); g.w01 = (1.f - ly) * lx; g.w10 = ly * (1.f - lx); g.w11 = ly * lx;
    const float* at = soft_att + (long)b * K * K;
    const float top = at[g.a00] * (1.f - lx) + at[g.a01] * lx;
    const float bot = at[g.a10] * (1.f - lx) + at[g.a11] * lx;
    g.wgt = (top * (1.f - ly) + bot * ly);
}

constexpr int TR_CG = 8;

__global__ __launch_bounds__(256) void transfer_fwd_kernel(const float* __restrict__ feat, int C, int H, int W,
                                                          const int* __restrict__ y1, const int* __restrict__ x1,
                                                          const int* __restrict__ index_all,
                                                          const float* __restrict__ soft_att, int py, int px, int K,
                                                          int side, int s, float* __restrict__ out, long out_ns) {
    const int OW = px * K * s, OH = py * K * s;
    const int pix = blockIdx.x * 256 + threadIdx.x, n = blockIdx.z;
    if (pix >= OH * OW) return;
    const int Y = pix / OW, X = pix % OW;
    const int by = Y / (K * s), bx = X / (K * s);
    const int b = (n * py + by) * px + bx;
    TrGeom g;
    tr_geometry(Y - by * K * s, X - bx * K * s, b, y1, x1, index_all, soft_att, K, side, s, H, W, g);
    const long HWf = (long)H * W, HWo = (long)OH * OW;
    float mult[9];
#pragma unroll
    for (int k = 0; k < 9; ++k) {
        int m = 0;
        bool first = g.src[k] >= 0;
#pragma unroll
        for (int q = 0; q < 9; ++q) {
            const bool same = g.src[q] == g.src[k];
            m += same ? 1 : 0;
            if (q < k && same) first = false;
        }
        mult[k] = first ? (float)m : 0.f;
    }
    const int c0 = blockIdx.y * TR_CG;
    float accs[TR_CG];
#pragma unroll
    for (int i = 0; i < TR_CG; ++i) {
        const float* f = feat + ((long)n * C + min(c0 + i, C - 1)) * HWf;
        float acc = 0.f;
#pragma unroll
        for (int k = 0; k < 9; ++k)
            if (mult[k] != 0.f) acc += mult[k] * f[g.src[k]];
        accs[i] = acc;
    }
#pragma unroll
    for (int i = 0; i < TR_CG; ++i)
        if (c0 + i < C) out[(long)n * out_ns + (long)(c0 + i) * HWo + pix] = accs[i] * g.inv_cnt * g.wgt;
}

__global__ __launch_bounds__(256) void absmax_bits_kernel(const float* __restrict__ x, long x_ns, long per4, int N,
                                                         unsigned* __restrict__ out) {
    float m = 0.f;
    const f32x4* p = reinterpret_cast<const f32x4*>(x + (long)blockIdx.y * x_ns);
    for (long i = blockIdx.x * 256L + threadIdx.x; i < per4; i += (long)gridDim.x * 256) {
        const f32x4 v = p[i];
        m = fmaxf(fmaxf(m, fmaxf(fabsf(v[0]), fabsf(v[1]))), fmaxf(fabsf(v[2]), fabsf(v[3])));
    }
    m = wave_max(m);
    if ((threadIdx.x & 63) == 0) atomicMax(out, __float_as_uint(m));
}
__device__ __forceinline__ int fixed_shift(unsigned amax_bits) {
    const int e = (int)((amax_bits >> 23) & 0xff) - 127;
    return 46 - (e + 1);
}
__global__ void fixed_to_float_kernel(const long long* __restrict__ acc, long n, const unsigned* __restrict__ amax_bits,
                                      float* __restrict__ out) {
    const double inv = ldexp(1.0, -fixed_shift(amax_bits[0]));
    for (long i = blockIdx.x * 256L + threadIdx.x; i < n; i += (long)gridDim.x * 256) out[i] += (float)((double)acc[i] * inv);
}

template <bool FIXED>
__global__ __launch_bounds__(256) void transfer_bwd_kernel(const float* __restrict__ dout, long dout_ns,
                                                          const float* __restrict__ feat, int C, int H, int W,
                                                          const int* __restrict__ y1, const int* __restrict__ x1,
                                                          const int* __restrict__ index_all,
                                                          const float* __restrict__ soft_att, int py, int px, int K,
                                                          int side, int s, int cpb , int N,
                                                          const unsigned* __restrict__ amax_bits,
                                                          unsigned long long* __restrict__ dfacc ,
                                                          float* __restrict__ dfeat ,
                                                          float* __restrict__ dA ) {
    const int OW = px * K * s, OH = py * K * s;
    const int pix = blockIdx.x * 256 + threadIdx.x, n = blockIdx.z;
    if (pix >= OH * OW) return;
    const int Y = pix / OW, X = pix % OW;
    const int by = Y / (K * s), bx = X / (K * s);
    const int b = (n * py + by) * px + bx;
    TrGeom g;
    tr_geometry(Y - by * K * s, X - bx * K * s, b, y1, x1, index_all, soft_att, K, side, s, H, W, g);
    const long HWf = (long)H * W, HWo = (long)OH * OW;
    const float coef = g.inv_cnt * g.wgt;
    float mult[9];
#pragma unroll
    for (int k = 0; k < 9; ++k) {
        int m = 0;
        bool first = g.src[k] >= 0;
#pragma unroll
        for (int q = 0; q < 9; ++q) {
            const bool same = g.src[q] == g.src[k];
            m += same ? 1 : 0;
            if (q < k && same) first = false;
        }
        mult[k] = first ? (float)m : 0.f;
    }
    float da = 0.f;
    const int c0 = blockIdx.y * cpb, c1 = min(c0 + cpb, C);
    const float fscale = FIXED ? ldexpf(1.f, fixed_shift(amax_bits[0])) : 1.f;
    for (int c = c0; c < c1; ++c) {
        const float* f = feat + ((long)n * C + c) * HWf;
        const float go = dout[(long)n * dout_ns + (long)c * HWo + pix];
        float acc = 0.f;
        const float gv = go * coef;
#pragma unroll
        for (int k = 0; k < 9; ++k)
            if (mult[k] > 0.f) {
                acc += mult[k] * f[g.src[k]];
                if (FIXED) atomicAdd(&dfacc[((long)n * C + c) * HWf + g.src[k]], (unsigned long long)__float2ll_rn(gv * mult[k] * fscale));
                else atomicAdd(&dfeat[((long)n * C + c) * HWf + g.src[k]], gv * mult[k]);
            }
        da += go * acc * g.inv_cnt;
    }
    dA[((long)blockIdx.y * N + n) * HWo + pix] = da;
}

__global__ __launch_bounds__(64) void transfer_datt_kernel(const float* __restrict__ dA, int py, int px, int K, int s,
                                                          int chunks, long chunk_stride, float* __restrict__ datt) {
    const int b = blockIdx.x, e = blockIdx.y;
    const int P = py * px, n = b / P, by = (b % P) / px, bx = b % px;
    const int i = e / K, j = e % K;
    const int OW = px * K * s, OH = py * K * s, KS = K * s;
    const int ylo = max((i - 1) * s, 0), yhi = min((i + 2) * s, KS);
    const int xlo = max((j - 1) * s, 0), xhi = min((j + 2) * s, KS);
    const int nw = xhi - xlo, tot = (yhi - ylo) * nw;
    float acc = 0.f;
    for (int t = threadIdx.x; t < tot; t += 64) {
        const int Yl = ylo + t / nw, Xl = xlo + t % nw;
        const float fy = fmaxf(((float)Yl + 0.5f) / (float)s - 0.5f, 0.f), fx = fmaxf(((float)Xl + 0.5f) / (float)s - 0.5f, 0.f);
        const int yy0 = min((int)fy, K - 1), xx0 = min((int)fx, K - 1);
        const int yy1 = min(yy0 + 1, K - 1), xx1 = min(xx0 + 1, K - 1);
        const float ly = fy - (float)yy0, lx = fx - (float)xx0;
        float wgt = 0.f;
        if (yy0 == i && xx0 == j) wgt += (1.f - ly) * (1.f - lx);
        if (yy0 == i && xx1 == j) wgt += (1.f - ly) * lx;
        if (yy1 == i && xx0 == j) wgt += ly * (1.f - lx);
        if (yy1 == i && xx1 == j) wgt += ly * lx;
        if (wgt != 0.f) {
            const long o = (long)n * OH * OW + (long)(by * KS + Yl) * OW + bx * KS + Xl;
            float v = 0.f;
            for (int q = 0; q < chunks; ++q) v += dA[q * chunk_stride + o];
            acc += wgt * v;
        }
    }
    acc = wave_sum(acc);
    if (threadIdx.x == 0) datt[(long)b * K * K + e] += acc;
}

inline int grid1d(long total, int cap = 8192) {
    long b = (total + 255) / 256;
    return (int)(b < cap ? (b < 1 ? 1 : b) : cap);
}

}

extern "C" int tdr_lr_blocks_fwd(const float* feat, int N, int C, int H, int W, int py, int px, int ky, int kx, float* blk,
                                 void* stream) {
    TDR_REQUIRE(feat && blk, "tdr_lr_blocks_fwd: null pointer");
    const long total = (long)N * py * px * C * (ky + 2) * (kx + 2);
    hipLaunchKernelGGL(lr_blocks_fwd_kernel, dim3(grid1d(total)), dim3(256), 0, (hipStream_t)stream, feat, C, H, W, py, px, ky,
                       kx, total, blk);
    TDR_LAUNCH_CHECK("lr_blocks_fwd");
    return TDR_OK;
}

extern "C" int tdr_lr_blocks_bwd(const float* dblk, int N, int C, int H, int W, int py, int px, int ky, int kx,
                                 float* dfeat, void* stream) {
    TDR_REQUIRE(dblk && dfeat, "tdr_lr_blocks_bwd: null pointer");
    const long total = (long)N * C * H * W;
    hipLaunchKernelGGL(lr_blocks_bwd_kernel, dim3(grid1d(total)), dim3(256), 0, (hipStream_t)stream, dblk, C, H, W, py, px, ky,
                       kx, total, dfeat);
    TDR_LAUNCH_CHECK("lr_blocks_bwd");
    return TDR_OK;
}

extern "C" int tdr_patch_inv_norm(const float* x, int B, int C, int H, int W, int OH, int OW, int dil, int pad, int step,
                                  int off, float* inv, void* stream) {
    TDR_REQUIRE(x && inv, "tdr_patch_inv_norm: null pointer");
    const long npos = (long)B * OH * OW;
    if (npos >= 1024)
        hipLaunchKernelGGL(patch_inv_norm_kernel, dim3((unsigned)((npos + 63) / 64)), dim3(1024), 0, (hipStream_t)stream, x, C, H,
                           W, OH, OW, dil, step, off - pad, npos, inv);
    else
        hipLaunchKernelGGL(patch_inv_norm_wave_kernel, dim3((unsigned)((npos + 3) / 4)), dim3(256), 0, (hipStream_t)stream, x, C,
                           H, W, OH, OW, dil, step, off - pad, npos, inv);
    TDR_LAUNCH_CHECK("patch_inv_norm");
    return TDR_OK;
}

extern "C" int tdr_coarse_argmax_box(const float* dots, const float* invq, const float* invk, int ND, int N, int P, int Hr,
                                     int Wr, int diameter, int* index, int* y1, int* x1, void* stream) {
    TDR_REQUIRE(dots && invq && invk && index && y1 && x1, "tdr_coarse_argmax_box: null pointer");
    hipLaunchKernelGGL(coarse_argmax_box_kernel, dim3(N * P), dim3(256), 0, (hipStream_t)stream, dots, invq, invk, ND, N, P, Hr,
                       Wr, diameter, index, y1, x1);
    TDR_LAUNCH_CHECK("coarse_argmax_box");
    return TDR_OK;
}

extern "C" int tdr_gather_ref_block(const float* feat, int N, int C, int H, int W, const int* y1, const int* x1, int P,
                                    int side, int s, float* out, void* stream) {
    TDR_REQUIRE(feat && y1 && x1 && out, "tdr_gather_ref_block: null pointer");
    const long total = (long)N * P * C * side * s * side * s;
    hipLaunchKernelGGL(gather_ref_block_kernel, dim3(grid1d(total)), dim3(256), 0, (hipStream_t)stream, feat, C, H, W, y1, x1,
                       P, side, s, total, out);
    TDR_LAUNCH_CHECK("gather_ref_block");
    return TDR_OK;
}

extern "C" int tdr_scatter_ref_block(const float* dblk, int N, int C, int H, int W, const int* y1, const int* x1, int P,
                                     int side, float* dfeat, void* stream) {
    TDR_REQUIRE(dblk && y1 && x1 && dfeat, "tdr_scatter_ref_block: null pointer");
    const long total = (long)N * C * H * W;
    hipLaunchKernelGGL(scatter_ref_block_kernel, dim3(grid1d(total)), dim3(256), 0, (hipStream_t)stream, dblk, C, H, W, y1, x1,
                       P, side, total, dfeat);
    TDR_LAUNCH_CHECK("scatter_ref_block");
    return TDR_OK;
}

extern "C" int tdr_fine_argmax(const float* dots, const float* invq, const float* invk, int B, int P, int R, int* index_all,
                               float* soft_att, void* stream) {
    TDR_REQUIRE(dots && invq && invk && index_all && soft_att, "tdr_fine_argmax: null pointer");
    const long rows = (long)B * P;
    hipLaunchKernelGGL(fine_argmax_kernel, dim3((unsigned)((rows + 3) / 4)), dim3(256), 0, (hipStream_t)stream, dots, invq, invk,
                       rows, P, R, index_all, soft_att);
    TDR_LAUNCH_CHECK("fine_argmax");
    return TDR_OK;
}

extern "C" int tdr_fine_search_bwd(const float* datt, const float* soft_att, const int* index_all, const float* lrb,
                                   const float* refb, const float* invq, const float* invk, int B, int C, int K, int D,
                                   float* dlrb, float* drefb, void* stream) {
    TDR_REQUIRE(datt && soft_att && index_all && lrb && refb && invq && invk && dlrb && drefb, "tdr_fine_search_bwd: null pointer");
    const size_t lds = (size_t)(8 * K * K + (K + 2) * (K + 2) + D * D) * sizeof(float);
    hipLaunchKernelGGL(fine_search_bwd_kernel, dim3(C, B), dim3(256), lds, (hipStream_t)stream, datt, soft_att, index_all, lrb,
                       refb, invq, invk, C, K, D, dlrb, drefb);
    TDR_LAUNCH_CHECK("fine_search_bwd");
    return TDR_OK;
}

extern "C" int tdr_transfer_fwd(const float* feat, int N, int C, int H, int W, const int* y1, const int* x1,
                                const int* index_all, const float* soft_att, int py, int px, int K, int side, int s,
                                float* out, int64_t out_ns, void* stream) {
    TDR_REQUIRE(feat && y1 && x1 && index_all && soft_att && out, "tdr_transfer_fwd: null pointer");
    const long opix = (long)py * K * s * px * K * s;
    hipLaunchKernelGGL(transfer_fwd_kernel, dim3((unsigned)((opix + 255) / 256), tdr_cdiv(C, TR_CG), N), dim3(256), 0,
                       (hipStream_t)stream, feat, C, H, W, y1, x1, index_all, soft_att, py, px, K, side, s, out, (long)out_ns);
    TDR_LAUNCH_CHECK("transfer_fwd");
    return TDR_OK;
}

static int tdr_transfer_chunks(int N, int C, int py, int px, int K, int s) {
    const long opix = (long)py * K * s * px * K * s;
    const long pix_blocks = ((opix + 255) / 256) * N;
    long chunks = (1024 + pix_blocks - 1) / pix_blocks;
    if (chunks > C / 8) chunks = C / 8;
    if (chunks < 1) chunks = 1;
    return (int)chunks;
}

extern "C" int64_t tdr_transfer_ws_floats(int N, int C, int H, int W, int py, int px, int K, int s) {
    const int64_t opix = (int64_t)py * K * s * px * K * s;
    return (int64_t)tdr_transfer_chunks(N, C, py, px, K, s) * N * opix + 4 + 2 * (int64_t)N * C * H * W;
}

extern "C" int tdr_transfer_bwd(const float* dout, int64_t dout_ns, const float* feat, int N, int C, int H, int W,
                                const int* y1, const int* x1, const int* index_all, const float* soft_att, int py, int px,
                                int K, int side, int s, int deterministic, float* dfeat, float* datt, float* ws, void* stream) {
    TDR_REQUIRE(dout && feat && y1 && x1 && index_all && soft_att && dfeat && datt && ws, "tdr_transfer_bwd: null pointer");
    const long opix = (long)py * K * s * px * K * s;
    hipStream_t st = (hipStream_t)stream;
    const int chunks = tdr_transfer_chunks(N, C, py, px, K, s);
    const int cpb = tdr_cdiv(C, chunks);
    float* dA = ws;
    const dim3 grid((unsigned)((opix + 255) / 256), tdr_cdiv(C, cpb), N);
    if (!deterministic) {
        hipLaunchKernelGGL(transfer_bwd_kernel<false>, grid, dim3(256), 0, st, dout, (long)dout_ns, feat, C, H, W, y1, x1, index_all,
                           soft_att, py, px, K, side, s, cpb, N, (const unsigned*)nullptr, (unsigned long long*)nullptr, dfeat, dA);
    } else {
        TDR_REQUIRE(opix % 4 == 0 && dout_ns % 4 == 0 && (reinterpret_cast<uintptr_t>(dout) & 15) == 0, "tdr_transfer_bwd: dout must be 16-byte aligned");
        char* tail = reinterpret_cast<char*>(ws + (long)chunks * N * opix);
        tail += (8 - reinterpret_cast<uintptr_t>(tail) % 8) % 8;
        unsigned* amax = reinterpret_cast<unsigned*>(tail);
        unsigned long long* acc = reinterpret_cast<unsigned long long*>(tail + 8);
        const long nacc = (long)N * C * H * W;
        if (hipMemsetAsync(tail, 0, 8 + (size_t)nacc * 8, st) != hipSuccess) {
            tdr_set_error("tdr_transfer_bwd: hipMemsetAsync failed");
            return TDR_ERR_HIP;
        }
        const long per4 = (long)C * opix / 4;
        hipLaunchKernelGGL(absmax_bits_kernel, dim3(grid1d(per4, 512), N), dim3(256), 0, st, dout, (long)dout_ns, per4, N, amax);
        hipLaunchKernelGGL(transfer_bwd_kernel<true>, grid, dim3(256), 0, st, dout, (long)dout_ns, feat, C, H, W, y1, x1, index_all,
                           soft_att, py, px, K, side, s, cpb, N, amax, acc, (float*)nullptr, dA);
        hipLaunchKernelGGL(fixed_to_float_kernel, dim3(grid1d(nacc, 4096)), dim3(256), 0, st, reinterpret_cast<const long long*>(acc),
                           nacc, amax, dfeat);
    }
    hipLaunchKernelGGL(transfer_datt_kernel, dim3(N * py * px, K * K), dim3(64), 0, st, ws, py, px, K, s, tdr_cdiv(C, cpb),
                       (long)N * opix, datt);
    TDR_LAUNCH_CHECK("transfer_bwd");
    return TDR_OK;
}

__global__ __launch_bounds__(256) void absmax_bits_any_kernel(const float* __restrict__ x, long x_ns, long per, unsigned* __restrict__ slot) {
    const float* p = x + (long)blockIdx.y * x_ns;
    float m = 0.f;
    unsigned bad = 0;
    for (long i = blockIdx.x * 256L + threadIdx.x; i < per; i += (long)gridDim.x * 256) {
        const float v = fabsf(p[i]);
        if (!(v <= 3.4028235e38f)) bad = 0x7fc00000u;
        m = fmaxf(m, v);
    }
    unsigned b = __float_as_uint(m) | bad;
#pragma unroll
    for (int o = 32; o > 0; o >>= 1) b = max(b, (unsigned)__shfl_xor((int)b, o, 64));
    if ((threadIdx.x & 63) == 0) atomicMax(slot, b);
}

extern "C" int tdr_absmax_bits(const float* x, int64_t x_ns, int N, int64_t per, unsigned* slot, void* stream) {
    TDR_REQUIRE(x && slot && N > 0 && per > 0, "tdr_absmax_bits: bad argument");
    hipLaunchKernelGGL(absmax_bits_any_kernel, dim3(grid1d(per, 256), N), dim3(256), 0, (hipStream_t)stream, x, (long)x_ns, (long)per, slot);
    TDR_LAUNCH_CHECK("absmax_bits");
    return TDR_OK;
}
```

textualdegremoval_amd/engine.py:

```python
import contextlib
import os
import types

import torch

from . import kernels as K
from . import leaves as L
from .kernels import (EPI_GATEBWD, EPI_PSHUF, PACK_DGRAD_2X2S2, PACK_DGRAD_3X3S2, PACK_DGRAD_S1, PACK_FWD)

LN_EPS = 1e-6
FUSE_TAIL = True
FUSE_HEAD = True
FUSE_CONV3_DGRAD = True
INFER_KERNELS = True
LOCAL_KERNELS = True


def _sub(P, pre):
    n = len(pre)
    return {k[n:]: v for k, v in P.items() if k.startswith(pre)}


def _put(G, pre, g):
    for k, v in g.items():
# ... 208 lines not shown

def conv_fwd(x, w, b, stride, pad, res=None, relu=False, out=None):
    Cout, Cin, KH, _ = w.shape
    wp, mp, *_ = K.pack_weights(w, PACK_FWD)
    out = K.conv_forward(x, wp, mp, Cout, KH, stride=stride, pad=pad, bias=b, res=res, relu=relu, out=out)
    return out


def conv_bwd(dout, x, w, stride, pad, need_dx=True, add_to_dx=None, bias=True, into=None):
    Cout, Cin, KH, _ = w.shape

    def leaf():
        if bias:
            gw, gb = K.conv_wgrad(x, dout, Cout, Cin, KH, stride=stride, pad=pad, want_db=True)
        else:
            gw, gb = K.conv_wgrad(x, dout, Cout, Cin, KH, stride=stride, pad=pad), None
        return gw.view(Cout, Cin, KH, KH), gb
    dw = db = None
    if into is not None:
        Gc, wname, bname = into
        L.set_prefix('')

        def leaf_named():
            gw, gb = leaf()
            return {wname: gw} if (gb is None or bname is None) else {wname: gw, bname: gb}
        L.leaf((x, dout), leaf_named, Gc)
    else:
        with K.on_side(x, dout):
            dw, db = leaf()
    dx = None
    if need_dx:
        N, _, OH, OW = dout.shape
        if stride == 1:
            wp, mp, *_ = K.pack_weights(w, PACK_DGRAD_S1)
            dx = K.conv_forward(dout, wp, mp, Cin, KH, pad=KH - 1 - pad, res=add_to_dx)
        elif KH == 2 and stride == 2 and pad == 0:
            wp, mp, *_ = K.pack_weights(w, PACK_DGRAD_2X2S2)
            dx = K.conv_forward(dout, wp, mp, 4 * Cin, 1, epi=EPI_PSHUF, res=add_to_dx)
        elif KH == 3 and stride == 2 and pad == 1:
            wp, mp, *_ = K.pack_weights(w, PACK_DGRAD_3X3S2)
            dx = K.conv_forward(dout, wp, mp, 4 * Cin, 2, pad=0, OH=OH, OW=OW, epi=EPI_PSHUF, res=add_to_dx)
        else:
            raise NotImplementedError(f'conv dgrad KH={KH} stride={stride} pad={pad}')
    L.maybe_join()
    return dx, dw, db


def up_fwd(x, w, skip):
    C2 = w.shape[0]
    wp, mp, *_ = K.pack_weights(w, PACK_FWD)
    return K.conv_forward(x, wp, mp, C2, 1, epi=EPI_PSHUF, res=skip)


def up_bwd(dout, x, w, into=None):
    C2, Cc = w.shape[0], w.shape[1]
    dT = K.pixel_unshuffle2(dout)
    dw = None
    if into is not None:
        L.set_prefix('')
        L.leaf((x, dT), lambda: {into[1]: K.conv_wgrad(x, dT, C2, Cc, 1).view(C2, Cc, 1, 1)}, into[0])
    else:
        with K.on_side(x, dT):
            dw = K.conv_wgrad(x, dT, C2, Cc, 1).view(C2, Cc, 1, 1)
    wp, mp, *_ = K.pack_weights(w, PACK_DGRAD_S1)
    dx = K.conv_forward(dT, wp, mp, Cc, 1)
    L.maybe_join()
    return dx, dw


def _enc_counts(ext):
    return [ext[0], ext[1], ext[2], ext[2], ext[2]]


P16_ON = True
P16_MIN_C = None


def _p16_level(Cc, n_blocks):
    fmt = K.plane_fmt()
    min_c = P16_MIN_C if P16_MIN_C is not None else (32 if fmt == K.FMT_BX3 else 64)
    return P16_ON and n_blocks > 0 and fmt is not None and K.p16_supported(Cc) and Cc >= min_c


def encoder_fwd(x, P, pre, ext_n_blocks, levels=5, keep=True, deep_only=False):
    feats, saved = [], []
    cnt = _enc_counts(ext_n_blocks)
    for lvl in range(levels):
        k = lvl + 1
        xin = x
        a = conv_fwd(xin, P[f'{pre}conv_L{k}.weight'], P[f'{pre}conv_L{k}.bias'], 1 if lvl == 0 else 2, 1, relu=True)
        blocks = []
        x = a
        Cc = a.shape[1]
        if _p16_level(Cc, cnt[lvl]):
            fmt = K.plane_fmt()
            tri = fmt == K.FMT_BX3
            x16, x32 = K.p16_from_f32(a, fmt=fmt), a
            for i in range(cnt[lvl]):
                bp = f'{pre}blk_L{k}.{i}.'
                wp1, mp1, *_ = K.pack_weights(P[bp + 'conv1.weight'], PACK_FWD)
                wp2, mp2, *_ = K.pack_weights(P[bp + 'conv2.weight'], PACK_FWD)
                last = i == cnt[lvl] - 1
                _, h16 = K.conv3x3_p16(x16, wp1, mp1, Cc, bias=P[bp + 'conv1.bias'], relu=True, want32=False, want16=True)
                o32, o16 = K.conv3x3_p16(h16, wp2, mp2, Cc, bias=P[bp + 'conv2.bias'], res=x16 if tri else x32,
                                         want32=last or not tri, want16=not last)
                if keep:
                    blocks.append((x16, h16))
                x16, x32 = o16, o32
            x = x32
        else:
            for i in range(cnt[lvl]):
                bp = f'{pre}blk_L{k}.{i}.'
                h = conv_fwd(x, P[bp + 'conv1.weight'], P[bp + 'conv1.bias'], 1, 1, relu=True)
                o = conv_fwd(h, P[bp + 'conv2.weight'], P[bp + 'conv2.bias'], 1, 1, res=x)
                if keep:
                    blocks.append((x, h))
                x = o
        feats.append(x if not deep_only or lvl == levels - 1 else None)
        if keep:
            saved.append((xin, a, blocks))
    return feats, (saved if keep else None)


def encoder_bwd(dfeats, P, pre, ext_n_blocks, saved, G):
    cnt = _enc_counts(ext_n_blocks)
    dnext = None
    with L.deferred_join():
        _encoder_bwd_levels(dfeats, P, pre, cnt, saved, G, dnext)
    L.maybe_join()
    return None


def _encoder_bwd_levels(dfeats, P, pre, cnt, saved, G, dnext):
    for lvl in reversed(range(len(dfeats))):
        k = lvl + 1
        xin, a, blocks = saved[lvl]
        d = dnext if dnext is not None else dfeats[lvl]
        if d is None:
            continue
        if blocks and isinstance(blocks[0][0], K.P16):
            d16, d32 = K.p16_from_f32(d, fmt=blocks[0][0].fmt), d
            fmts = {t.fmt for bl in blocks for t in bl} | {d16.fmt}
            grouped = GROUP_LEAVES and 2 * cnt[lvl] > 1 and len(fmts) == 1
            late = []
            for i in reversed(range(cnt[lvl])):
                bp = f'{pre}blk_L{k}.{i}.'
                x16, h16 = blocks[i]
                w1, w2 = P[bp + 'conv1.weight'], P[bp + 'conv2.weight']
                Cc = w1.shape[0]
                if grouped:
                    late.append((bp + 'conv2', h16, d16))
                else:
                    with K.on_side(h16.buf, d16.buf):
                        gw, G[bp + 'conv2.bias'] = K.wgrad3x3_p16(h16, d16, want_db=True)
                        G[bp + 'conv2.weight'] = gw.view(Cc, Cc, 3, 3)
                wp, mp, *_ = K.pack_weights(w2, PACK_DGRAD_S1)
                _, dh16 = K.conv3x3_p16(d16, wp, mp, Cc, mask=h16, want32=False, want16=True)
                if grouped:
                    late.append((bp + 'conv1', x16, dh16))
                else:
                    with K.on_side(x16.buf, dh16.buf):
                        gw, G[bp + 'conv1.bias'] = K.wgrad3x3_p16(x16, dh16, want_db=True)
                        G[bp + 'conv1.weight'] = gw.view(Cc, Cc, 3, 3)
                wp, mp, *_ = K.pack_weights(w1, PACK_DGRAD_S1)
                first = i == 0
                d32, d16 = K.conv3x3_p16(dh16, wp, mp, Cc, res=d32 if d32 is not None else d16, mask=a if first else None,
                                         want32=first, want16=not first)
            if late:
                with K.on_side(*[t.buf for _, x16, g16 in late for t in (x16, g16)]):
                    res = K.wgrad3x3_p16_group([(x16, g16) for _, x16, g16 in late], seq=('enc3x3', pre, lvl), want_db=True)
                    for (name, x16, g16), (gw, gb) in zip(late, res):
                        G[name + '.bias'] = gb
                        G[name + '.weight'] = gw.view(g16.C, x16.C, 3, 3)
                late.clear()
            d = d32
        else:
            for i in reversed(range(cnt[lvl])):
                bp = f'{pre}blk_L{k}.{i}.'
                x_in, h = blocks[i]
                w1, w2 = P[bp + 'conv1.weight'], P[bp + 'conv2.weight']
                Cc = w1.shape[0]
                with K.on_side(h, d):
                    gw, G[bp + 'conv2.bias'] = K.conv_wgrad(h, d, Cc, Cc, 3, pad=1, want_db=True)
                    G[bp + 'conv2.weight'] = gw.view(Cc, Cc, 3, 3)
                wp, mp, *_ = K.pack_weights(w2, PACK_DGRAD_S1)
                dh = K.conv_forward(d, wp, mp, Cc, 3, pad=1, mask=h)
                with K.on_side(x_in, dh):
                    gw, G[bp + 'conv1.bias'] = K.conv_wgrad(x_in, dh, Cc, Cc, 3, pad=1, want_db=True)
                    G[bp + 'conv1.weight'] = gw.view(Cc, Cc, 3, 3)
                wp, mp, *_ = K.pack_weights(w1, PACK_DGRAD_S1)
                d = K.conv_forward(dh, wp, mp, Cc, 3, pad=1, res=d, mask=a if i == 0 else None)
        dpre = d if cnt[lvl] > 0 else K.relu_bwd(d, a)
        w = P[f'{pre}conv_L{k}.weight']
        dnext, G[f'{pre}conv_L{k}.weight'], G[f'{pre}conv_L{k}.bias'] = conv_bwd(
            dpre, xin, w, 1 if lvl == 0 else 2, 1, need_dx=(lvl > 0), add_to_dx=dfeats[lvl - 1] if lvl > 0 else None)
    L.maybe_join()
    return None


class MasaGeom:
    def __init__(self, h, w, hr, wr, n_enc, lr_block_size, ref_down_block_size, dilations):
        padder = 2 ** n_enc
        self.px = w // padder // lr_block_size
        self.py = h // padder // lr_block_size
        self.kx = w // padder // self.px
        self.ky = h // padder // self.py
        self.dia_x = 2 * int(wr // padder // (2 * self.px) * ref_down_block_size) + 1
        self.dia_y = 2 * int(hr // padder // (2 * self.py) * ref_down_block_size) + 1
        if self.dia_x != self.dia_y or self.kx != self.ky:
            raise ValueError('MASA geometry must be square (the reference only runs for square geometry, :668-669)')
        self.dilations = list(dilations)
        self.P = self.py * self.px
        self.K = self.kx
        self.side = self.dia_x + 2


class Pyramids:
    __slots__ = ('N', 'stacked', 'inp_p', 'geo', 'feats', 'sv_enc', 'lq_deep', 'ref_feats', 'levels')


def pyramids_fwd(P, cfg, inp, ref, padder_log2, levels, keep=True):
    N, Ci, H0, W0 = inp.shape
    mult = (2 ** padder_log2) * cfg['lr_block_size']
    Hp, Wp = -(-H0 // mult) * mult, -(-W0 // mult) * mult
    Hr0, Wr0 = ref.shape[-2:]
    Hrp, Wrp = -(-Hr0 // mult) * mult, -(-Wr0 // mult) * mult
    if ref.shape[0] != N:
        raise ValueError('inp and ref must have the same batch size')
    py = Pyramids()
    py.N, py.levels = N, levels
    py.geo = MasaGeom(Hp, Wp, Hrp, Wrp, padder_log2, cfg['lr_block_size'], cfg['ref_down_block_size'], cfg['dilations'])
    py.stacked = (Hrp, Wrp) == (Hp, Wp)
    if py.stacked:
        both = torch.empty(2 * N, Ci, Hp, Wp, dtype=torch.float32, device=inp.device)
        _pad_into(inp.contiguous(), both[:N])
        _pad_into(ref.contiguous(), both[N:])
        py.inp_p = both[:N]
        py.feats, py.sv_enc = encoder_fwd(both, P, 'masa_enc.', cfg['ext_n_blocks'], levels=levels, keep=keep)
        py.lq_deep = py.feats[levels - 1][:N]
        py.ref_feats = [f[N:] for f in py.feats]
    else:
        py.inp_p = torch.empty(N, Ci, Hp, Wp, dtype=torch.float32, device=inp.device)
        ref_p = torch.empty(N, Ci, Hrp, Wrp, dtype=torch.float32, device=inp.device)
        _pad_into(inp.contiguous(), py.inp_p)
        _pad_into(ref.contiguous(), ref_p)
        fl, svl = encoder_fwd(py.inp_p, P, 'masa_enc.', cfg['ext_n_blocks'], levels=levels, keep=keep, deep_only=not keep)
        fr, svr = encoder_fwd(ref_p, P, 'masa_enc.', cfg['ext_n_blocks'], levels=levels, keep=keep)
        py.feats, py.sv_enc = (fl, fr), (svl, svr)
        py.lq_deep, py.ref_feats = fl[levels - 1], fr
    if not keep:
        py.feats = py.sv_enc = None
    return py, (H0, W0, Hp, Wp)


def pyramids_bwd(dwarp, py, P, cfg, sv_masa, G):
    N, L = py.N, py.levels
    if py.stacked:
        dfeats = [torch.zeros_like(f) for f in py.feats]
        masa_bwd(dwarp, py.lq_deep, py.ref_feats, N, py.geo, sv_masa, dfeats[L - 1][:N], [d[N:] for d in dfeats])
        encoder_bwd(dfeats, P, 'masa_enc.', cfg['ext_n_blocks'], py.sv_enc, G)
        return
    fl, fr = py.feats
    dlq = torch.empty_like(fl[L - 1])
    dref = [torch.zeros_like(f) for f in fr]
    masa_bwd(dwarp, py.lq_deep, py.ref_feats, N, py.geo, sv_masa, dlq, dref)
    Gl, Gr = {}, {}
    encoder_bwd([None] * (L - 1) + [dlq], P, 'masa_enc.', cfg['ext_n_blocks'], py.sv_enc[0], Gl)
    encoder_bwd(dref, P, 'masa_enc.', cfg['ext_n_blocks'], py.sv_enc[1], Gr)
    for k, g in Gr.items():
        G[k] = K.add_(g.contiguous().view(1, -1), Gl[k].contiguous().view(1, -1)).view(g.shape) if k in Gl else g


def masa_fwd(lq4, ref_feats, N, geo, outs=None, keep=True):
    P, Kk, side = geo.P, geo.K, geo.side
    L = len(ref_feats)
    ref4 = ref_feats[L - 1]
    _, Cc, H, W = lq4.shape
    Hr, Wr = ref4.shape[-2:]
    dev = lq4.device
    lrb = K.lr_blocks_fwd(lq4, geo.py, geo.px, Kk, Kk)
    ND = len(geo.dilations)
    R = Hr * Wr
    dots = torch.empty(ND, N, P, Hr, Wr, dtype=torch.float32, device=dev)
    invq = torch.empty(ND, N * P, dtype=torch.float32, device=dev)
    invk = torch.empty(ND, N, R, dtype=torch.float32, device=dev)
    cc = (Kk + 2) // 2
    for di, d in enumerate(geo.dilations):
        wp, mp, per_b = K.pack_patches(lrb, P, 1, 1, 1, d, cc - d)
        K.conv_forward(ref4, wp, mp, P, 3, dil=d, pad=d, wp_ns=per_b, out=dots[di])
        K.patch_inv_norm(lrb, 1, 1, dil=d, off=cc - d, out=invq[di])
        K.patch_inv_norm(ref4, Hr, Wr, dil=d, pad=d, out=invk[di])
    index, y1, x1 = K.coarse_argmax_box(dots, invq, invk, N, P, Hr, Wr, geo.dia_x)
    if not keep:
        dots = invq = invk = wp = None
    refb = K.gather_ref_block(ref4, y1, x1, P, side, 1)
    wp, mp, per_b = K.pack_patches(lrb, 1, Kk, Kk, 1, 1, 0)
    R1 = side - 2
    fdots = K.conv_forward(refb, wp, mp, Kk * Kk, 3, pad=0, wp_ns=per_b)
    finvq = K.patch_inv_norm(lrb, Kk, Kk)
    finvk = K.patch_inv_norm(refb, R1, R1)
    index_all, soft_att = K.fine_argmax(fdots, finvq, finvk, N * P, Kk * Kk, R1 * R1)
    if not keep:
        lq4 = ref4 = lrb = refb = wp = fdots = finvq = finvk = None
    warp = []
    for lvl in range(L):
        s = 2 ** (L - 1 - lvl)
        warp.append(K.transfer_fwd(ref_feats[lvl], y1, x1, index_all, soft_att, geo.py, geo.px, Kk, side, s,
                                   out=None if outs is None else outs[lvl]))
        if not keep:
            ref_feats[lvl] = None
    if not keep:
        return warp, None
    saved = (lrb, refb, finvq, finvk, index, y1, x1, index_all, soft_att)
    return warp, saved


def masa_bwd(dwarp, lq4, ref_feats, N, geo, saved, dlq_out, dref_out):
    lrb, refb, finvq, finvk, index, y1, x1, index_all, soft_att = saved
    P, Kk, side = geo.P, geo.K, geo.side
    L = len(ref_feats)
    dev = lq4.device
    datt = torch.zeros(N * P, Kk * Kk, dtype=torch.float32, device=dev)
    for lvl in range(L):
        s = 2 ** (L - 1 - lvl)
        K.transfer_bwd(dwarp[lvl], ref_feats[lvl], y1, x1, index_all, soft_att, geo.py, geo.px, Kk, side, s,
                       dref_out[lvl], datt)
    dlrb, drefb = K.fine_search_bwd(datt, soft_att, index_all, lrb, refb, finvq, finvk, Kk, side)
    K.scatter_ref_block(drefb, dref_out[L - 1], y1, x1, P, side)
    _, Cc, H, W = lq4.shape
    dlq4 = K.lr_blocks_bwd(dlrb, N, Cc, H, W, geo.py, geo.px, Kk, Kk)
    K.copy_rows(dlq4, Cc * H * W, dlq_out, Cc * H * W, N, Cc * H * W)


def _pad_into(src, dst_view):
    N, Cc, Hs, Ws = src.shape
    _, _, Hd, Wd = dst_view.shape
    if (Hs, Ws) == (Hd, Wd):
        K.copy_rows(src, Cc * Hs * Ws, dst_view, Cc * Hd * Wd, N, Cc * Hs * Ws)
    else:
        tmp = K.pad_crop(src, Hd, Wd)
        K.copy_rows(tmp, Cc * Hd * Wd, dst_view, Cc * Hd * Wd, N, Cc * Hd * Wd)


def tlsc_kernel_sizes(cfg, train_size):
    _, _, Ht, Wt = train_size
    n_enc = len(cfg['enc_blk_nums'])
    mult = 1 << n_enc
    Hp, Wp = -(-Ht // mult) * mult, -(-Wt // mult) * mult
    bh, bw = int(Ht * 1.5), int(Wt * 1.5)
    return [((Hp >> l) * bh // Ht, (Wp >> l) * bw // Wt) for l in range(n_enc + 1)]


def _level(cfg, l):
    if l == len(cfg['enc_blk_nums']):
        return 'middle_blks.', cfg['middle_blk_num'], 'masa_blk_middle.0.'
    return f'encoders.{l}.', cfg['enc_blk_nums'][l], f'masa_blk_enc.{l}.'


def walk_fwd(P, cfg, inp, ref=None, seq=naf_seq_fwd, local=None, keep=True):
    n_enc = len(cfg['enc_blk_nums'])
    N, _, H0, W0 = inp.shape
    chan = P['intro.weight'].shape[0]
    cats = sv_masa = None
    kw = {} if keep else {'keep': False}
    if ref is not None:
        pyr, sizes = pyramids_fwd(P, cfg, inp, ref, n_enc, n_enc + 1, **kw)
        Hp, Wp = sizes[2:]
        cats = [torch.empty(N, (chan << l) + pyr.ref_feats[l].shape[1], Hp >> l, Wp >> l, dtype=torch.float32, device=inp.device)
                for l in range(n_enc + 1)]
        warp, sv_masa = masa_fwd(pyr.lq_deep, pyr.ref_feats, N, pyr.geo, outs=[c[:, chan << l:] for l, c in enumerate(cats)], **kw)
        warp = None
        if not keep:
            pyr.lq_deep = pyr.ref_feats = None
    else:
        mult = 1 << n_enc
        Hp, Wp = -(-H0 // mult) * mult, -(-W0 // mult) * mult
        sizes = (H0, W0, Hp, Wp)
        pyr = types.SimpleNamespace(inp_p=inp.contiguous() if (Hp, Wp) == (H0, W0) else K.pad_crop(inp.contiguous(), Hp, Wp), geo=None)

    def stage(x, pre, n, l):
        return seq(x, P, pre, n, **kw) if local is None else seq(x, P, pre, n, local=local[l], **kw)
    S = types.SimpleNamespace(levels=[], dec=[]) if keep else None
    skips = []
    x = conv_fwd(pyr.inp_p, P['intro.weight'], P['intro.bias'], 1, 1, out=cats[0][:, :chan] if cats else None)
    for l in range(n_enc + 1):
        pre, n, fus = _level(cfg, l)
        sv_f = None
        if cats:
            x = None
            x, sv_f = naf_seq_fwd(cats[l] if keep else _take(cats, l), P, fus, cfg['reffusion_n_blocks'][l], c_out_last=chan << l, **kw)
        x, sv_e = stage(x, pre, n, l)
        skips.append(x if l < n_enc else None)
        if keep:
            S.levels.append((sv_f, sv_e, x))
        if l < n_enc:
            x = conv_fwd(x, P[f'downs.{l}.weight'], P[f'downs.{l}.bias'], 2, 0, out=cats[l + 1][:, :chan << (l + 1)] if cats else None)
    for l in range(len(cfg['dec_blk_nums'])):
        xin = x
        x = up_fwd(xin, P[f'ups.{l}.0.weight'], skips[n_enc - 1 - l] if keep else _take(skips, n_enc - 1 - l))
        if not keep:
            xin = None
        x, sv_d = stage(x, f'decoders.{l}.', cfg['dec_blk_nums'][l], n_enc - 1 - l)
        if keep:
            S.dec.append((xin, sv_d))
    out_p = conv_fwd(x, P['ending.weight'], P['ending.bias'], 1, 1, res=pyr.inp_p)
    out = out_p if (Hp, Wp) == (H0, W0) else K.pad_crop(out_p, H0, W0)
    if not keep:
        return out, None
    S.xe = x
    return out, (N, sizes, pyr.geo, pyr, None, None, sv_masa, S)


def _take(lst, i):
    t, lst[i] = lst[i], None
    return t


def walk_bwd(dout, P, cfg, saved, G=None, seq=naf_seq_bwd):
    G = {} if G is None else G
    N, (H0, W0, Hp, Wp), _, pyr, _, _, sv_masa, S = saved[:8]
    guided = sv_masa is not None
    n_enc = len(cfg['enc_blk_nums'])
    chan = P['intro.weight'].shape[0]
    with L.deferred_join(), (late_leaves(G, level_ok=True) if guided else contextlib.nullcontext()):
        dout = dout.contiguous()
        if (Hp, Wp) != (H0, W0):
            dout = K.pad_crop(dout, Hp, Wp)
        d, G['ending.weight'], G['ending.bias'] = conv_bwd(dout, S.xe, P['ending.weight'], 1, 1)
        dskips = [None] * n_enc
        for l in reversed(range(len(cfg['dec_blk_nums']))):
            xin, sv_d = S.dec[l]
            d = seq(d, P, f'decoders.{l}.', cfg['dec_blk_nums'][l], sv_d, G)
            L.level_end(G)
            dskips[n_enc - 1 - l] = d
            d, _ = up_bwd(d, xin, P[f'ups.{l}.0.weight'], into=(G, f'ups.{l}.0.weight'))
        dwarp = [None] * (n_enc + 1)
        for l in reversed(range(n_enc + 1)):
            pre, n, fus = _level(cfg, l)
            sv_f, sv_e, x_skip = S.levels[l]
            if l < n_enc:
                d, _, _ = conv_bwd(d, x_skip, P[f'downs.{l}.weight'], 2, 0, add_to_dx=dskips[l],
                                   into=(G, f'downs.{l}.weight', f'downs.{l}.bias'))
            d = seq(d, P, pre, n, sv_e, G)
            if guided:
                dcat = naf_seq_bwd(d, P, fus, cfg['reffusion_n_blocks'][l], sv_f, G)
                L.level_end(G)
                dwarp[l] = dcat[:, chan << l:]
                d = dcat[:, :chan << l]
        dinp, _, _ = conv_bwd(d, pyr.inp_p, P['intro.weight'], 1, 1, need_dx=not guided, add_to_dx=None if guided else dout,
                              into=(G, 'intro.weight', 'intro.bias'))
        if dinp is not None and (Hp, Wp) != (H0, W0):
            dinp = K.pad_crop(dinp, H0, W0)
        if guided:
            L.run_late_leaves(G, lambda: pyramids_bwd(dwarp, pyr, P, cfg, sv_masa, G))
    return dinp, G


def net_fwd(P, cfg, inp, ref, keep=True):
    return walk_fwd(P, cfg, inp, ref, keep=keep)


def net_bwd(dout, P, cfg, saved, G=None):
    return walk_bwd(dout, P, cfg, saved, G)[1]


def unet_fwd(P, cfg, inp, local=None, keep=True):
    return walk_fwd(P, cfg, inp, local=local, keep=keep)


def unet_bwd(dout, P, cfg, saved, G=None):
    return walk_bwd(dout, P, cfg, saved, G)
```

textualdegremoval_amd/kernels.py:

```python
import contextlib
import ctypes as C
import os

import torch

from . import _lib
from ._lib import TdrConvDesc, TdrConvP16Desc, TdrWgradDesc, TdrWgradP16Desc, check

EPI_STD, EPI_GATEBWD, EPI_PSHUF = 0, 1, 2
PACK_FWD, PACK_DGRAD_S1, PACK_DGRAD_2X2S2, PACK_DGRAD_3X3S2 = 0, 1, 2, 3

MATH = os.environ.get('TDR_MATH', 'bx3')
WGRAD_1X1_BX3 = True
FMT_F32, FMT_BX3, FMT_HX2, FMT_H1 = 0, 1, 2, 3


def fp16_path():
    return MATH in ('hx2', 'h1')


GRAD_SCALED = False
BACKWARD_PHASE = False


# ... 872 lines not shown
    return out


def naf_tail_infer_local(g, pooled, x, wscap, bsca, w3p, b3, beta, lnw, lnb, eps, w4p, b4, w5p, b5, gamma):
    N, Cc, H, W = g.shape
    assert pooled.shape == g.shape and x.shape == g.shape and g.is_contiguous() and pooled.is_contiguous() and x.is_contiguous()
    assert wscap.fmt == w3p.fmt == w4p.fmt == w5p.fmt
    out = torch.empty_like(g)
    d = _lib.TdrNafTailLocalDesc()
    d.N, d.C, d.HW, d.w_fmt, d.eps = N, Cc, H * W, w3p.fmt, float(eps)
    d.g, d.g_ns, d.pool, d.pool_ns, d.x, d.x_ns = g.data_ptr(), _dense_nchw(g), pooled.data_ptr(), _dense_nchw(pooled), x.data_ptr(), _dense_nchw(x)
    d.wsca, d.w3, d.w4, d.w5 = wscap.data_ptr(), w3p.data_ptr(), w4p.data_ptr(), w5p.data_ptr()
    d.bsca, d.b3, d.beta, d.lnw, d.lnb = bsca.data_ptr(), b3.data_ptr(), beta.data_ptr(), lnw.data_ptr(), lnb.data_ptr()
    d.b4, d.b5, d.gamma = b4.data_ptr(), b5.data_ptr(), gamma.data_ptr()
    d.out, d.out_ns = out.data_ptr(), _dense_nchw(out)
    check(_lib.load().tdr_naf_tail_infer_local(C.byref(d), _stream()), 'tdr_naf_tail_infer_local')
    return out


def _ln_partials_finish(ws, nparts, Cc):
    def fin():
        gw = torch.empty(Cc, dtype=torch.float32, device=ws.device)
        gb = torch.empty_like(gw)
        check(_lib.load().tdr_pair_sum_partials(ws.data_ptr(), nparts, Cc, gw.data_ptr(), gb.data_ptr(),
                                                ws.data_ptr() + 4 * nparts * 2 * Cc, _stream()), 'tdr_pair_sum_partials')
        return gw, gb
    return Finisher('ln' if nparts <= 1024 else None, ws, (nparts, Cc), fin)


def naf_tail_bwd(dout, gamma, t4, y, mu, rs, lnw, w5tp, w4tp, w3tp=None, beta=None, sca=None, defer_finish=False):
    lib = _lib.load()
    N, Cc, H, W = y.shape
    dev = y.device
    assert dout.is_contiguous()
    dt4 = torch.empty(N, 2 * Cc, H, W, dtype=torch.float32, device=dev)
    dy = torch.empty(N, Cc, H, W, dtype=torch.float32, device=dev)
    nws = lib.tdr_naf_tail_bwd_ws_floats(N, Cc, H * W)
    if defer_finish:
        gw = gb = None
        ws = torch.empty(int(nws), dtype=torch.float32, device=dev)
    else:
        gw = torch.empty(Cc, dtype=torch.float32, device=dev)
        gb = torch.empty_like(gw)
        ws = workspace(nws, dev, 'naftail')
    d = _lib.TdrNafTailBwdDesc()
    d.N, d.C, d.HW, d.c_out = N, Cc, H * W, dout.shape[1]
    assert w5tp.fmt == w4tp.fmt
    d.w_fmt = w5tp.fmt
    d.dout, d.dout_ns, d.gamma = dout.data_ptr(), _dense_nchw(dout), gamma.data_ptr()
    d.t4, d.t4_ns, d.y, d.y_ns = t4.data_ptr(), _dense_nchw(t4), y.data_ptr(), _dense_nchw(y)
    d.mu, d.rs, d.lnw, d.w5t, d.w4t = mu.data_ptr(), rs.data_ptr(), lnw.data_ptr(), w5tp.data_ptr(), w4tp.data_ptr()
    d.dt4, d.dt4_ns, d.dy, d.dy_ns = dt4.data_ptr(), _dense_nchw(dt4), dy.data_ptr(), _dense_nchw(dy)
    d.gw, d.gb, d.ws = _p(gw), _p(gb), ws.data_ptr()
    dgp = None
    if w3tp is not None:
        assert w3tp.fmt == w4tp.fmt and sca.is_contiguous()
        dgp = torch.empty(N, Cc, H, W, dtype=torch.float32, device=dev)
        d.w3t, d.beta, d.sca, d.dgp, d.dgp_ns = w3tp.data_ptr(), beta.data_ptr(), sca.data_ptr(), dgp.data_ptr(), _dense_nchw(dgp)
    if _survey is not None:
        _survey.probe(dout, 'grad')
    check(lib.tdr_naf_tail_bwd(C.byref(d), _stream()), 'tdr_naf_tail_bwd')
    if _survey is not None:
        _survey.probe(dt4, 'grad')
        if dgp is not None:
            _survey.probe(dy, 'grad')
    if defer_finish:
        gw = _ln_partials_finish(ws, N * (H * W // 64), Cc)
    return (dy, dt4, gw, gb) if dgp is None else (dy, dt4, gw, gb, dgp)


def _naf_head_desc(cls, x, lnw, lnb, eps, w1p, b1, t1):
    N, Cc, H, W = x.shape
    d = cls()
    d.N, d.C, d.HW, d.w_fmt = N, Cc, H * W, w1p.fmt
    d.x, d.x_ns, d.lnw, d.lnb, d.eps = x.data_ptr(), _dense_nchw(x), lnw.data_ptr(), lnb.data_ptr(), float(eps)
    d.w1, d.b1, d.t1, d.t1_ns = w1p.data_ptr(), b1.data_ptr(), t1.data_ptr(), _dense_nchw(t1)
    return d


def naf_head_fwd(x, lnw, lnb, eps, w1p, b1):
    lib = _lib.load()
    N, Cc, H, W = x.shape
    dev = x.device
    xn = torch.empty(N, Cc, H, W, dtype=torch.float32, device=dev)
    t1 = torch.empty(N, 2 * Cc, H, W, dtype=torch.float32, device=dev)
    mu = torch.empty(N, H * W, dtype=torch.float32, device=dev)
    rs = torch.empty_like(mu)
    d = _naf_head_desc(_lib.TdrNafHeadFwdDesc, x, lnw, lnb, eps, w1p, b1, t1)
    d.mu, d.rs, d.xn, d.xn_ns = mu.data_ptr(), rs.data_ptr(), xn.data_ptr(), _dense_nchw(xn)
    if _survey is not None:
        _survey.probe(x, 'fwd')
    check(lib.tdr_naf_head_fwd(C.byref(d), _stream()), 'tdr_naf_head_fwd')
    return xn, mu, rs, t1


def naf_head_infer(x, lnw, lnb, eps, w1p, b1):
    N, Cc, H, W = x.shape
    t1 = torch.empty(N, 2 * Cc, H, W, dtype=torch.float32, device=x.device)
    d = _naf_head_desc(_lib.TdrNafHeadFwdDesc, x, lnw, lnb, eps, w1p, b1, t1)
    check(_lib.load().tdr_naf_head_infer(C.byref(d), _stream()), 'tdr_naf_head_infer')
    return t1


def naf_head_bwd(dt1, x, mu, rs, lnw, w1tp, res, defer_finish=False):
    lib = _lib.load()
    N, Cc, H, W = x.shape
    dev = x.device
    assert dt1.is_contiguous()
    dx = torch.empty(N, Cc, H, W, dtype=torch.float32, device=dev)
    nws = lib.tdr_naf_tail_bwd_ws_floats(N, Cc, H * W)
    if defer_finish:
        gw = gb = None
        ws = torch.empty(int(nws), dtype=torch.float32, device=dev)
    else:
        gw = torch.empty(Cc, dtype=torch.float32, device=dev)
        gb = torch.empty_like(gw)
        ws = workspace(nws, dev, 'naftail')
    d = _lib.TdrNafHeadBwdDesc()
    d.N, d.C, d.HW, d.w_fmt = N, Cc, H * W, w1tp.fmt
    d.dt1, d.dt1_ns, d.x, d.x_ns = dt1.data_ptr(), _dense_nchw(dt1), x.data_ptr(), _dense_nchw(x)
    d.mu, d.rs, d.lnw, d.w1t = mu.data_ptr(), rs.data_ptr(), lnw.data_ptr(), w1tp.data_ptr()
    d.res, d.res_ns, d.dx, d.dx_ns = res.data_ptr(), _dense_nchw(res), dx.data_ptr(), _dense_nchw(dx)
    d.gw, d.gb, d.ws = _p(gw), _p(gb), ws.data_ptr()
    if _survey is not None:
        _survey.probe(dt1, 'grad')
    check(lib.tdr_naf_head_bwd(C.byref(d), _stream()), 'tdr_naf_head_bwd')
    if defer_finish:
        gw = _ln_partials_finish(ws, N * (H * W // 64), Cc)
    return dx, gw, gb


def sca_fwd(pooled, wsca, bsca):
    lib = _lib.load()
    N, Cc = pooled.shape
    s = torch.empty(N, Cc, dtype=torch.float32, device=pooled.device)
    check(lib.tdr_sca_fwd(pooled.data_ptr(), wsca.data_ptr(), bsca.data_ptr(), N, Cc, s.data_ptr(), _stream()), 'tdr_sca_fwd')
    return s


def sca_bwd(G3, S3, w3, b3, beta, s, pooled, wsca):
    lib = _lib.load()
    N, Cc = s.shape
    dev = s.device
    dw3 = torch.empty(Cc, Cc, 1, 1, dtype=torch.float32, device=dev)
    db3 = torch.empty(Cc, dtype=torch.float32, device=dev)
    dbeta = torch.empty(1, Cc, 1, 1, dtype=torch.float32, device=dev)
    dwsca = torch.empty(Cc, Cc, 1, 1, dtype=torch.float32, device=dev)
    dbsca = torch.empty(Cc, dtype=torch.float32, device=dev)
    dpooled = torch.empty(N, Cc, dtype=torch.float32, device=dev)
    ws = torch.empty(N * Cc, dtype=torch.float32, device=dev)
    check(lib.tdr_sca_bwd(G3.data_ptr(), S3.data_ptr(), w3.data_ptr(), b3.data_ptr(), beta.data_ptr(), s.data_ptr(),
                          pooled.data_ptr(), wsca.data_ptr(), N, Cc, dw3.data_ptr(), db3.data_ptr(), dbeta.data_ptr(),
                          dwsca.data_ptr(), dbsca.data_ptr(), dpooled.data_ptr(), ws.data_ptr(), _stream()), 'tdr_sca_bwd')
    return dw3, db3, dbeta, dwsca, dbsca, dpooled


def scaled_conv_param_grads(G, S, w, b, gamma):
    lib = _lib.load()
    Cout, Cin = G.shape[-2], G.shape[-1]
    dev = G.device
    dw = torch.empty(Cout, Cin, dtype=torch.float32, device=dev)
    db = torch.empty(Cout, dtype=torch.float32, device=dev)
    dg = torch.empty(Cout, dtype=torch.float32, device=dev)
    check(lib.tdr_scaled_conv_param_grads(G.data_ptr(), S.data_ptr(), w.data_ptr(), b.data_ptr(), gamma.data_ptr(), Cout,
                                          Cin, dw.data_ptr(), db.data_ptr(), dg.data_ptr(), _stream()),
          'tdr_scaled_conv_param_grads')
    return dw, db, dg


def channel_sum(x):
    lib = _lib.load()
    N, Cc, H, W = x.shape
    out = torch.empty(Cc, dtype=torch.float32, device=x.device)
    ws = workspace(lib.tdr_chansum_ws_floats(N, Cc, H * W), x.device)
    check(lib.tdr_channel_sum(x.data_ptr(), _dense_nchw(x), N, Cc, H * W, out.data_ptr(), ws.data_ptr(), _stream()),
          'tdr_channel_sum')
    return out


def multi_copy(src_tab, dst_tab, sizes, chunk_tensor, chunk_index, n_chunks, scale=1.0, guard=None):
    if guard is not None:
        check(_lib.load().tdr_multi_copy_guarded(src_tab.data_ptr(), dst_tab.data_ptr(), sizes.data_ptr(), chunk_tensor.data_ptr(),
                                                 chunk_index.data_ptr(), n_chunks, guard.data_ptr(), _stream()),
              'tdr_multi_copy_guarded')
        return
    check(_lib.load().tdr_multi_copy(src_tab.data_ptr(), dst_tab.data_ptr(), sizes.data_ptr(), chunk_tensor.data_ptr(),
                                     chunk_index.data_ptr(), n_chunks, float(scale), _stream()), 'tdr_multi_copy')


def copy_rows(src, src_ns, dst, dst_ns, N, length):
    check(_lib.load().tdr_copy_rows(src.data_ptr(), src_ns, dst.data_ptr(), dst_ns, N, length, _stream()), 'tdr_copy_rows')


def add_rows(src, src_ns, dst, dst_ns, N, length):
    check(_lib.load().tdr_add_rows(src.data_ptr(), src_ns, dst.data_ptr(), dst_ns, N, length, _stream()), 'tdr_add_rows')


def concat2(a, b):
    N, Ca, H, W = a.shape
    Cb = b.shape[1]
    out = torch.empty(N, Ca + Cb, H, W, dtype=torch.float32, device=a.device)
    tot = (Ca + Cb) * H * W
    copy_rows(a, _dense_nchw(a), out, tot, N, Ca * H * W)
    copy_rows(b, _dense_nchw(b), out[:, Ca:], tot, N, Cb * H * W)
    return out


def slice_channels(x, c0, c1):
    N, Cc, H, W = x.shape
    out = torch.empty(N, c1 - c0, H, W, dtype=torch.float32, device=x.device)
    copy_rows(x[:, c0:c1], _dense_nchw(x), out, (c1 - c0) * H * W, N, (c1 - c0) * H * W)
    return out


def add_(dst, src):
    N = dst.shape[0]
    per = dst[0].numel()
    add_rows(src, _dense_nchw(src) if src.dim() == 4 else per, dst, _dense_nchw(dst) if dst.dim() == 4 else per, N, per)
    return dst


def pixel_unshuffle2(x):
    N, Cc, H2, W2 = x.shape
    assert x.is_contiguous()
    out = torch.empty(N, 4 * Cc, H2 // 2, W2 // 2, dtype=torch.float32, device=x.device)
    check(_lib.load().tdr_pixel_unshuffle2(x.data_ptr(), N, Cc, H2 // 2, W2 // 2, out.data_ptr(), _stream()),
          'tdr_pixel_unshuffle2')
    return out


def pad_crop(x, Hd, Wd):
    N, Cc, Hs, Ws = x.shape
    assert x.is_contiguous()
    out = torch.empty(N, Cc, Hd, Wd, dtype=torch.float32, device=x.device)
    check(_lib.load().tdr_pad_crop(x.data_ptr(), N, Cc, Hs, Ws, out.data_ptr(), Hd, Wd, _stream()), 'tdr_pad_crop')
    return out


def img_u8_to_planes(img, Hp=None, Wp=None, swap_rb=True):
    assert img.dtype == torch.uint8 and img.dim() == 4 and img.is_contiguous()
    N, H, W, Cc = img.shape
    Hp, Wp = H if Hp is None else int(Hp), W if Wp is None else int(Wp)
    out = torch.empty(N, Cc, Hp, Wp, dtype=torch.float32, device=img.device)
    check(_lib.load().tdr_img_u8_to_planes(img.data_ptr(), N, H, W, Cc, int(bool(swap_rb)), out.data_ptr(), Hp, Wp, _stream()),
          'tdr_img_u8_to_planes')
    return out


def planes_to_img_u8(x, H=None, W=None, swap_rb=True):
    assert x.dtype == torch.float32 and x.dim() == 4 and x.is_contiguous()
    N, Cc, Hp, Wp = x.shape
    H, W = Hp if H is None else int(H), Wp if W is None else int(W)
    out = torch.empty(N, H, W, Cc, dtype=torch.uint8, device=x.device)
    check(_lib.load().tdr_planes_to_img_u8(x.data_ptr(), N, Cc, Hp, Wp, int(bool(swap_rb)), out.data_ptr(), H, W, _stream()),
          'tdr_planes_to_img_u8')
    return out


def relu_bwd(go, act):
    assert go.is_contiguous() and act.is_contiguous()
    out = torch.empty_like(go)
    check(_lib.load().tdr_relu_bwd(go.data_ptr(), act.data_ptr(), go.numel(), out.data_ptr(), _stream()), 'tdr_relu_bwd')
    return out


def l1_loss(pred, target, loss_weight=1.0, grad_scale=1.0, guard=None):
    assert pred.is_contiguous() and target.is_contiguous()
    loss = torch.empty(1, dtype=torch.float32, device=pred.device)
    dpred = torch.empty_like(pred)
    ws = workspace(4096, pred.device, 'l1')
    if guard is not None:
        check(_lib.load().tdr_l1_loss_guarded(pred.data_ptr(), target.data_ptr(), pred.numel(), float(loss_weight), guard.data_ptr(),
                                              loss.data_ptr(), dpred.data_ptr(), ws.data_ptr(), _stream()), 'tdr_l1_loss_guarded')
        return loss, dpred
    check(_lib.load().tdr_l1_loss(pred.data_ptr(), target.data_ptr(), pred.numel(), float(loss_weight), float(grad_scale), loss.data_ptr(),
                                  dpred.data_ptr(), ws.data_ptr(), _stream()), 'tdr_l1_loss')
    return loss, dpred


LOSS_L1, LOSS_MSE, LOSS_CHARBONNIER, LOSS_PSNR, LOSS_PSNR_Y = range(5)


def pixel_loss(kind, pred, target, loss_weight=1.0, eps=1e-3, grad_scale=1.0, guard=None):
    assert pred.is_contiguous() and target.is_contiguous() and pred.shape == target.shape and pred.dim() == 4
    N, Cc, H, W = pred.shape
    loss = torch.empty(1, dtype=torch.float32, device=pred.device)
    dpred = torch.empty_like(pred)
    ws = workspace(4096 + 128 * N, pred.device, 'l1')
    check(_lib.load().tdr_pixel_loss(int(kind), pred.data_ptr(), target.data_ptr(), N, Cc * H * W, H * W, float(loss_weight), float(eps),
                                     float(grad_scale), guard.data_ptr() if guard is not None else None, loss.data_ptr(),
                                     dpred.data_ptr(), ws.data_ptr(), _stream()), 'tdr_pixel_loss')
    return loss, dpred


def lr_blocks_fwd(feat, py, px, ky, kx):
    N, Cc, H, W = feat.shape
    assert feat.is_contiguous()
    blk = torch.empty(N * py * px, Cc, ky + 2, kx + 2, dtype=torch.float32, device=feat.device)
    check(_lib.load().tdr_lr_blocks_fwd(feat.data_ptr(), N, Cc, H, W, py, px, ky, kx, blk.data_ptr(), _stream()),
          'tdr_lr_blocks_fwd')
    return blk


def lr_blocks_bwd(dblk, N, Cc, H, W, py, px, ky, kx):
    dfeat = torch.empty(N, Cc, H, W, dtype=torch.float32, device=dblk.device)
    check(_lib.load().tdr_lr_blocks_bwd(dblk.data_ptr(), N, Cc, H, W, py, px, ky, kx, dfeat.data_ptr(), _stream()),
          'tdr_lr_blocks_bwd')
    return dfeat


def patch_inv_norm(x, OH, OW, dil=1, pad=0, step=1, off=0, out=None):
    B, Cc, H, W = x.shape
    assert x.is_contiguous()
    inv = out if out is not None else torch.empty(B, OH, OW, dtype=torch.float32, device=x.device)
    assert inv.is_contiguous() and inv.numel() == B * OH * OW
    check(_lib.load().tdr_patch_inv_norm(x.data_ptr(), B, Cc, H, W, OH, OW, dil, pad, step, off, inv.data_ptr(), _stream()),
          'tdr_patch_inv_norm')
    return inv


def coarse_argmax_box(dots, invq, invk, N, P, Hr, Wr, diameter):
    ND = dots.shape[0]
    dev = dots.device
    index = torch.empty(N * P, dtype=torch.int32, device=dev)
    y1 = torch.empty_like(index)
    x1 = torch.empty_like(index)
    check(_lib.load().tdr_coarse_argmax_box(dots.data_ptr(), invq.data_ptr(), invk.data_ptr(), ND, N, P, Hr, Wr, diameter,
                                            index.data_ptr(), y1.data_ptr(), x1.data_ptr(), _stream()),
          'tdr_coarse_argmax_box')
    return index, y1, x1


def gather_ref_block(feat, y1, x1, P, side, s):
    N, Cc, H, W = feat.shape
    out = torch.empty(N * P, Cc, side * s, side * s, dtype=torch.float32, device=feat.device)
    check(_lib.load().tdr_gather_ref_block(feat.data_ptr(), N, Cc, H, W, y1.data_ptr(), x1.data_ptr(), P, side, s,
                                           out.data_ptr(), _stream()), 'tdr_gather_ref_block')
    return out


def scatter_ref_block(dblk, dfeat, y1, x1, P, side):
    N, Cc, H, W = dfeat.shape
    check(_lib.load().tdr_scatter_ref_block(dblk.data_ptr(), N, Cc, H, W, y1.data_ptr(), x1.data_ptr(), P, side,
                                            dfeat.data_ptr(), _stream()), 'tdr_scatter_ref_block')


def fine_argmax(dots, invq, invk, B, P, R):
    dev = dots.device
    index_all = torch.empty(B, P, dtype=torch.int32, device=dev)
    soft_att = torch.empty(B, P, dtype=torch.float32, device=dev)
    check(_lib.load().tdr_fine_argmax(dots.data_ptr(), invq.data_ptr(), invk.data_ptr(), B, P, R, index_all.data_ptr(),
                                      soft_att.data_ptr(), _stream()), 'tdr_fine_argmax')
    return index_all, soft_att


def fine_search_bwd(datt, soft_att, index_all, lrb, refb, invq, invk, K, D):
    B, Cc = lrb.shape[0], lrb.shape[1]
    dlrb = torch.empty_like(lrb)
    drefb = torch.empty_like(refb)
    check(_lib.load().tdr_fine_search_bwd(datt.data_ptr(), soft_att.data_ptr(), index_all.data_ptr(), lrb.data_ptr(),
                                          refb.data_ptr(), invq.data_ptr(), invk.data_ptr(), B, Cc, K, D, dlrb.data_ptr(),
                                          drefb.data_ptr(), _stream()), 'tdr_fine_search_bwd')
    return dlrb, drefb


def transfer_fwd(feat, y1, x1, index_all, soft_att, py, px, K, side, s, out=None):
    N, Cc, H, W = feat.shape
    assert feat.is_contiguous()
    if out is None:
        out = torch.empty(N, Cc, py * K * s, px * K * s, dtype=torch.float32, device=feat.device)
    check(_lib.load().tdr_transfer_fwd(feat.data_ptr(), N, Cc, H, W, y1.data_ptr(), x1.data_ptr(), index_all.data_ptr(),
                                       soft_att.data_ptr(), py, px, K, side, s, out.data_ptr(), _dense_nchw(out),
                                       _stream()), 'tdr_transfer_fwd')
    return out


DETERMINISTIC = os.environ.get('TDR_DETERMINISTIC', '0') == '1'


def transfer_bwd(dout, feat, y1, x1, index_all, soft_att, py, px, K, side, s, dfeat, datt):
    N, Cc, H, W = feat.shape
    ws = workspace(_lib.load().tdr_transfer_ws_floats(N, Cc, H, W, py, px, K, s), feat.device, 'transfer')
    check(_lib.load().tdr_transfer_bwd(dout.data_ptr(), _dense_nchw(dout), feat.data_ptr(), N, Cc, H, W, y1.data_ptr(),
                                       x1.data_ptr(), index_all.data_ptr(), soft_att.data_ptr(), py, px, K, side, s,
                                       1 if DETERMINISTIC else 0, dfeat.data_ptr(), datt.data_ptr(), ws.data_ptr(), _stream()),
          'tdr_transfer_bwd')


def resize_bilinear(x, Hd, Wd):
    B, Cc, Hs, Ws = x.shape
    assert x.is_contiguous()
    out = torch.empty(B, Cc, Hd, Wd, dtype=torch.float32, device=x.device)
    check(_lib.load().tdr_resize_bilinear(x.data_ptr(), B * Cc, Hs, Ws, out.data_ptr(), Hd, Wd, _stream()), 'tdr_resize_bilinear')
    return out


def unfold_windows(ref, h, stride):
    B, Cc, Hr, Wr = ref.shape
    assert ref.is_contiguous()
    N = ((Hr - h) // stride + 1) * ((Wr - h) // stride + 1)
    out = torch.empty(B * N, Cc, h, h, dtype=torch.float32, device=ref.device)
    check(_lib.load().tdr_unfold_windows(ref.data_ptr(), B, Cc, Hr, Wr, h, stride, out.data_ptr(), _stream()), 'tdr_unfold_windows')
    return out, N


def token_ld(T):
    return (T + 1 + 31) // 32 * 32


def patchify(x, p, flat=False):
    B, Ci, H, W = x.shape
    assert x.is_contiguous()
    T = (H // p) * (W // p)
    LD = token_ld(T)
    shape = (1, Ci * p * p, B * LD // 32, 32) if flat else (B, Ci * p * p, LD // 32, 32)
    out = torch.empty(*shape, dtype=torch.float32, device=x.device)
    check(_lib.load().tdr_patchify(x.data_ptr(), B, Ci, H, W, p, LD, 1 if flat else 0, out.data_ptr(), _stream()), 'tdr_patchify')
    return out, T


def vit_assemble_(tok, cls, pos_cm, T, flat_batch=0):
    D = tok.shape[1]
    B = flat_batch or tok.shape[0]
    LD = tok.shape[2] * tok.shape[3] // (flat_batch or 1)
    check(_lib.load().tdr_vit_assemble(tok.data_ptr(), cls.data_ptr(), pos_cm.data_ptr(), B, D, T, LD, 1 if flat_batch else 0, _stream()),
          'tdr_vit_assemble')
    return tok


def attention_fwd(qkv, heads, scale, T1, flat_batch=0, single_product=False):
    B, C3 = (flat_batch or qkv.shape[0]), qkv.shape[1]
    Cc, LD = C3 // 3, qkv.shape[2] * qkv.shape[3] // (flat_batch or 1)
    assert qkv.is_contiguous()
    out = torch.empty(qkv.shape[0], Cc, qkv.shape[2], qkv.shape[3], dtype=torch.float32, device=qkv.device)
    math = 2 if (MATH in ('hx2', 'h1') and not ATTN_F32) else (1 if (MATH == 'bx3' and ATTN_BX3) else 0)
    if single_product and math == 2 and Cc // heads in (16, 32, 64):
        math = 3
    check(_lib.load().tdr_attention_fwd_math(qkv.data_ptr(), B, Cc, heads, T1, LD, float(scale), math, 1 if flat_batch else 0, out.data_ptr(),
                                             _stream()),
          'tdr_attention_fwd')
    return out


def transpose_f32(src):
    B, R, Cc = src.shape
    assert src.is_contiguous() and src.dtype == torch.float32
    dst = torch.empty(B, Cc, R, dtype=torch.float32, device=src.device)
    check(_lib.load().tdr_transpose_f32(src.data_ptr(), B, R, Cc, dst.data_ptr(), _stream()), 'tdr_transpose_f32')
    return dst


def tok_layernorm(x, w, b, eps, out_f16=True, planes=False):
    P, D = x.shape
    assert x.is_contiguous() and x.dtype == torch.float32
    planes = 2 if planes is True else int(planes)
    if planes == 3:
        out = torch.empty(3, P, D, dtype=torch.bfloat16, device=x.device)
    elif planes:
        out = torch.empty(2, P, D, dtype=torch.float16, device=x.device)
    else:
        out = torch.empty(P, D, dtype=torch.float16 if out_f16 else torch.float32, device=x.device)
    check(_lib.load().tdr_tok_layernorm(x.data_ptr(), w.data_ptr(), b.data_ptr(), P, D, float(eps), planes if planes else (1 if out_f16 else 0),
                                        out.data_ptr(), _stream()), 'tdr_tok_layernorm')
    return out


def split_planes(w):
    hi = w.to(torch.float16)
    return torch.stack([hi, (w - hi.to(torch.float32)).to(torch.float16)]).contiguous()


def split_planes3(w):
    h = w.to(torch.bfloat16)
    r = w - h.to(torch.float32)
    m = r.to(torch.bfloat16)
    return torch.stack([h, m, (r - m.to(torch.float32)).to(torch.bfloat16)]).contiguous()


def tok16x3_gemm(x3, w3, bias, epi, act=0, out32=None, ls=None):
    _, P, Kd = x3.shape
    N = w3.shape[1]
    assert x3.is_contiguous() and w3.is_contiguous() and x3.dtype == torch.bfloat16 and w3.dtype == torch.bfloat16 and w3.shape[2] == Kd
    assert x3.shape[0] == 3 and w3.shape[0] == 3
    y = None
    if epi == 2:
        assert out32 is not None and out32.is_contiguous() and out32.dtype == torch.float32 and tuple(out32.shape) == (P, N)
    elif epi == 3:
        out32 = torch.empty(N, P, dtype=torch.float32, device=x3.device)
    else:
        y = torch.empty(3, P, N, dtype=torch.bfloat16, device=x3.device)
    check(_lib.load().tdr_tok16x3_gemm(x3.data_ptr(), w3.data_ptr(), _p(bias), P, N, Kd, int(epi), int(act), _p(y), _p(out32), _p(ls),
                                       _stream()), 'tdr_tok16x3_gemm')
    return y if epi == 4 else out32


def cm_to_tok16x3(src):
    Cc, P = src.shape
    assert src.is_contiguous() and src.dtype == torch.float32
    out = torch.empty(3, P, Cc, dtype=torch.bfloat16, device=src.device)
    check(_lib.load().tdr_cm_to_tok16x3(src.data_ptr(), Cc, P, out.data_ptr(), _stream()), 'tdr_cm_to_tok16x3')
    return out


def tok16x2_gemm(x2, w2, bias, epi, act=0, out32=None):
    _, P, Kd = x2.shape
    N = w2.shape[1]
    assert x2.is_contiguous() and w2.is_contiguous() and x2.dtype == torch.float16 and w2.dtype == torch.float16 and w2.shape[2] == Kd
    y = None
    if epi == 2:
        assert out32 is not None and out32.is_contiguous() and out32.dtype == torch.float32 and tuple(out32.shape) == (P, N)
    elif epi == 3:
        out32 = torch.empty(N, P, dtype=torch.float32, device=x2.device)
    else:
        y = torch.empty(2, P, N, dtype=torch.float16, device=x2.device)
    check(_lib.load().tdr_tok16x2_gemm(x2.data_ptr(), w2.data_ptr(), _p(bias), P, N, Kd, int(epi), int(act), _p(y), _p(out32), _stream()),
          'tdr_tok16x2_gemm')
    return y if epi == 4 else out32


def cm_to_tok16x2(src):
    Cc, P = src.shape
    assert src.is_contiguous() and src.dtype == torch.float32
    out = torch.empty(2, P, Cc, dtype=torch.float16, device=src.device)
    check(_lib.load().tdr_cm_to_tok16x2(src.data_ptr(), Cc, P, out.data_ptr(), _stream()), 'tdr_cm_to_tok16x2')
    return out


def tok16_gemm(x16, w16, bias, epi=0, res=None, ls=None):
    P, Kd = x16.shape
    N = w16.shape[0]
    assert x16.is_contiguous() and w16.is_contiguous() and x16.dtype == torch.float16 and w16.dtype == torch.float16 and w16.shape[1] == Kd
    y = None
    if epi == 2:
        assert res is not None and res.is_contiguous() and res.dtype == torch.float32 and tuple(res.shape) == (P, N)
    else:
        y = torch.empty(P, N, dtype=torch.float16, device=x16.device)
    check(_lib.load().tdr_tok16_gemm(x16.data_ptr(), w16.data_ptr(), _p(bias), P, N, Kd, int(epi), _p(y), _p(res), _p(ls), _stream()),
          'tdr_tok16_gemm')
    return res if epi == 2 else y


def tok16_attention(qkv16, B, heads, scale, T1):
    P, C3 = qkv16.shape
    assert qkv16.is_contiguous() and qkv16.dtype == torch.float16 and P % B == 0
    out = torch.empty(P, C3 // 3, dtype=torch.float16, device=qkv16.device)
    check(_lib.load().tdr_tok16_attention(qkv16.data_ptr(), B, C3 // 3, heads, T1, P // B, float(scale), out.data_ptr(), _stream()),
          'tdr_tok16_attention')
    return out


def token_match(fl, fr, windows, N, T1):
    B, D = fl.shape[0], fl.shape[1]
    LD = fl.shape[2] * fl.shape[3]
    per = windows[0].numel()
    corr = torch.empty(B, N, dtype=torch.float32, device=fl.device)
    index = torch.empty(B, dtype=torch.int32, device=fl.device)
    ref_in = torch.empty((B,) + tuple(windows.shape[1:]), dtype=torch.float32, device=fl.device)
    check(_lib.load().tdr_token_match(fl.data_ptr(), fr.data_ptr(), windows.data_ptr(), B, N, D, T1, LD, per, corr.data_ptr(),
                                      index.data_ptr(), ref_in.data_ptr(), _stream()), 'tdr_token_match')
    return corr, index, ref_in


def dwgelu_fwd(t, w, b=None):
    N, C2, H, W = t.shape
    assert t.is_contiguous()
    g = torch.empty(N, C2 // 2, H, W, dtype=torch.float32, device=t.device)
    check(_lib.load().tdr_dwgelu_fwd(t.data_ptr(), w.data_ptr(), _p(b), N, C2 // 2, H, W, g.data_ptr(), _stream()), 'tdr_dwgelu_fwd')
    return g


def dwgelu_bwd(dg, t, w, b=None):
    lib = _lib.load()
    N, C2, H, W = t.shape
    Cc = C2 // 2
    assert dg.is_contiguous() and t.is_contiguous()
    dt = torch.empty_like(t)
    dw = torch.empty(C2, 1, 3, 3, dtype=torch.float32, device=t.device)
    db = torch.empty(C2, dtype=torch.float32, device=t.device) if b is not None else None
    ws = workspace(lib.tdr_dwsg_ws_floats(N, Cc, H, W), t.device)
    check(lib.tdr_dwgelu_bwd(dg.data_ptr(), t.data_ptr(), w.data_ptr(), _p(b), N, Cc, H, W, dt.data_ptr(), dw.data_ptr(),
                             _p(db), ws.data_ptr(), _stream()), 'tdr_dwgelu_bwd')
    return dt, dw, db


def dwconv_fwd(t, w, b=None):
    N, Pn, H, W = t.shape
    assert t.is_contiguous()
    out = torch.empty_like(t)
    check(_lib.load().tdr_dwconv_fwd(t.data_ptr(), w.data_ptr(), _p(b), N, Pn, H, W, out.data_ptr(), _stream()), 'tdr_dwconv_fwd')
    return out


def dwconv_bwd(dout, t, w, want_db=False):
    lib = _lib.load()
    N, Pn, H, W = t.shape
    assert dout.is_contiguous() and t.is_contiguous()
    dt = torch.empty_like(t)
    dw = torch.empty(Pn, 1, 3, 3, dtype=torch.float32, device=t.device)
    db = torch.empty(Pn, dtype=torch.float32, device=t.device) if want_db else None
    ws = workspace(lib.tdr_dwsg_ws_floats(N, Pn // 2, H, W), t.device)
    check(lib.tdr_dwconv_bwd(dout.data_ptr(), t.data_ptr(), w.data_ptr(), N, Pn, H, W, dt.data_ptr(), dw.data_ptr(), _p(db),
                             ws.data_ptr(), _stream()), 'tdr_dwconv_bwd')
    return dt, dw, db


def row_sumsq(x, rows):
    N, _, H, W = x.shape
    out = torch.empty(N, rows, dtype=torch.float32, device=x.device)
    check(_lib.load().tdr_row_sumsq(x.data_ptr(), _dense_nchw(x), N, rows, H * W, out.data_ptr(), _stream()), 'tdr_row_sumsq')
    return out


def pack_f32packed_to_bx3(Wt):
    lib = _lib.load()
    B, Kp, Mp = Wt.shape
    assert Wt.is_contiguous()
    per_b = lib.tdr_packed_weight_bytes_bx3(Mp, Kp, 1) // 4
    buf = torch.empty(B * per_b, dtype=torch.float32, device=Wt.device)
    check(lib.tdr_pack_weights_bx3_batch(Wt.data_ptr(), Kp * Mp, B, Kp, Mp, 1, 1, buf.data_ptr(), _stream()),
          'tdr_pack_weights_bx3_batch')
    return PackedWeights(buf, FMT_BX3), per_b


def mdta_pad(Cc):
    return (Cc + 31) // 32 * 32


def mdta_softmax(G, ss, temp, heads):
    N, Cc = G.shape[0], G.shape[-1]
    Cp = mdta_pad(Cc)
    A = torch.empty(N, Cp, Cp, dtype=torch.float32, device=G.device)
    AT = torch.empty_like(A)
    check(_lib.load().tdr_mdta_softmax(G.data_ptr(), ss.data_ptr(), temp.data_ptr(), N, Cc, heads, A.data_ptr(), AT.data_ptr(),
                                       _stream()), 'tdr_mdta_softmax')
    return A, AT


def attn_fold_proj(AT, w_out, heads):
    N, Cp = AT.shape[0], AT.shape[-1]
    Cc = w_out.shape[0]
    assert AT.is_contiguous() and w_out.is_contiguous() and AT.shape[1] == Cp == mdta_pad(Cc) and w_out.shape[1] == Cc
    Wf = torch.empty_like(AT)
    check(_lib.load().tdr_attn_fold_proj(AT.data_ptr(), w_out.data_ptr(), N, Cc, heads, Wf.data_ptr(), _stream()), 'tdr_attn_fold_proj')
    return Wf


def mdta_bwd(G, ss, temp, A, dA, heads):
    N, Cc = G.shape[0], G.shape[-1]
    Wp = mdta_pad(2 * Cc)
    W = torch.empty(N, Wp, Wp, dtype=torch.float32, device=G.device)
    dtemp = torch.empty(heads, 1, 1, dtype=torch.float32, device=G.device)
    ws = torch.empty(N * heads, dtype=torch.float32, device=G.device)
    check(_lib.load().tdr_mdta_bwd(G.data_ptr(), ss.data_ptr(), temp.data_ptr(), A.data_ptr(), dA.data_ptr(), N, Cc, heads,
                                   W.data_ptr(), dtemp.data_ptr(), ws.data_ptr(), _stream()), 'tdr_mdta_bwd')
    return W, dtemp


def axpby_dev(a, alpha, b=None):
    assert a.is_contiguous() and (b is None or b.is_contiguous())
    out = torch.empty_like(a)
    check(_lib.load().tdr_axpby_dev(a.data_ptr(), alpha.data_ptr(), _p(b), a.numel(), out.data_ptr(), _stream()), 'tdr_axpby_dev')
    return out


def dot(a, b):
    assert a.is_contiguous() and b.is_contiguous() and a.numel() == b.numel()
    out = torch.empty(1, dtype=torch.float32, device=a.device)
    ws = workspace(512, a.device, 'dot')
    check(_lib.load().tdr_dot(a.data_ptr(), b.data_ptr(), a.numel(), out.data_ptr(), ws.data_ptr(), _stream()), 'tdr_dot')
    return out


def pixel_shuffle2(x):
    N, C4, H, W = x.shape
    assert x.is_contiguous() and C4 % 4 == 0
    out = torch.empty(N, C4 // 4, 2 * H, 2 * W, dtype=torch.float32, device=x.device)
    check(_lib.load().tdr_pixel_shuffle2(x.data_ptr(), N, C4 // 4, H, W, out.data_ptr(), _stream()), 'tdr_pixel_shuffle2')
    return out


def leaky_relu_fwd(x, slope=0.01):
    assert x.is_contiguous()
    y = torch.empty_like(x)
    check(_lib.load().tdr_leaky_relu_fwd(x.data_ptr(), x.numel(), float(slope), y.data_ptr(), _stream()), 'tdr_leaky_relu_fwd')
    return y


def leaky_relu_bwd(go, y, slope=0.01):
    assert go.is_contiguous() and y.is_contiguous()
# ... 802 lines not shown
```

Baseline: 62.62.

## Batch MASA transfer levels into single launches and restructure fine-search backward

New measurement: 62.93, median of 6. Within noise of the previous version (+0.5%).

```diff
diff --git a/include/tdr.h b/include/tdr.h
--- a/include/tdr.h
+++ b/include/tdr.h
@@ -235,6 +235,20 @@
 int tdr_transfer_bwd(const float* dout, int64_t dout_ns, const float* feat, int N, int C, int H, int W,
                      const int* y1, const int* x1, const int* index_all, const float* soft_att, int py, int px,
                      int K, int side, int s, int deterministic, float* dfeat, float* datt, float* ws, void* stream);
+#define TDR_TRANSFER_MAX_LEVELS 8
+typedef struct TdrTransferLevel {
+    const float* feat;
+    int C, H, W, s;
+    float* io;
+    int64_t io_ns;
+    float* dfeat;
+} TdrTransferLevel;
+int tdr_transfer_fwd_levels(const TdrTransferLevel* lv, int L, int N, const int* y1, const int* x1, const int* index_all,
+                            const float* soft_att, int py, int px, int K, int side, void* stream);
+int64_t tdr_transfer_levels_ws_floats(const TdrTransferLevel* lv, int L, int N, int py, int px, int K, int deterministic);
+int tdr_transfer_bwd_levels(const TdrTransferLevel* lv, int L, int N, const int* y1, const int* x1, const int* index_all,
+                            const float* soft_att, int py, int px, int K, int side, int deterministic, float* datt,
+                            float* ws, void* stream);
 int tdr_scatter_ref_block(const float* dblk, int N, int C, int H, int W, const int* y1, const int* x1, int P,
                           int side, float* dfeat, void* stream);
 
diff --git a/textualdegremoval_amd/_lib.py b/textualdegremoval_amd/_lib.py
--- a/textualdegremoval_amd/_lib.py
+++ b/textualdegremoval_amd/_lib.py
@@ -91,6 +91,10 @@
                 ('wsca', c_fp), ('w3', c_fp), ('w4', c_fp), ('w5', c_fp),
                 ('bsca', c_fp), ('b3', c_fp), ('beta', c_fp), ('lnw', c_fp), ('lnb', c_fp), ('b4', c_fp), ('b5', c_fp), ('gamma', c_fp),
                 ('out', c_fp), ('out_ns', i64)]
+
+
+class TdrTransferLevel(C.Structure):
+    _fields_ = [('feat', c_fp), ('C', i32), ('H', i32), ('W', i32), ('s', i32), ('io', c_fp), ('io_ns', i64), ('dfeat', c_fp)]
 
 
 class TdrNafTailBwdDesc(C.Structure):
@@ -271,6 +275,9 @@
     'tdr_transfer_ws_floats': (i64, [i32, i32, i32, i32, i32, i32, i32, i32]),
     'tdr_transfer_bwd': (i32, [c_fp, i64, c_fp, i32, i32, i32, i32, c_fp, c_fp, c_fp, c_fp, i32, i32, i32, i32, i32, i32,
                                c_fp, c_fp, c_fp, c_fp]),
+    'tdr_transfer_fwd_levels': (i32, [C.POINTER(TdrTransferLevel), i32, i32, c_fp, c_fp, c_fp, c_fp, i32, i32, i32, i32, c_fp]),
+    'tdr_transfer_levels_ws_floats': (i64, [C.POINTER(TdrTransferLevel), i32, i32, i32, i32, i32, i32]),
+    'tdr_transfer_bwd_levels': (i32, [C.POINTER(TdrTransferLevel), i32, i32, c_fp, c_fp, c_fp, c_fp, i32, i32, i32, i32, i32, c_fp, c_fp, c_fp]),
     'tdr_resize_bilinear': (i32, [c_fp, i32, i32, i32, c_fp, i32, i32, c_fp]),
     'tdr_unfold_windows': (i32, [c_fp, i32, i32, i32, i32, i32, i32, c_fp, c_fp]),
     'tdr_patchify': (i32, [c_fp, i32, i32, i32, i32, i32, i32, i32, c_fp, c_fp]),
diff --git a/textualdegremoval_amd/csrc/tdr_masa.hip b/textualdegremoval_amd/csrc/tdr_masa.hip
--- a/textualdegremoval_amd/csrc/tdr_masa.hip
+++ b/textualdegremoval_amd/csrc/tdr_masa.hip
@@ -206,6 +206,13 @@
     if (lane == 0) { index_all[row] = bi; soft_att[row] = best; }
 }
 
+constexpr int FS_CG = 16;
+
+inline size_t fine_search_bwd_lds_words(int K, int D) {
+    const int P = K * K;
+    return (size_t)7 * P + (D * D + 1) + 18 * P + 256 + (size_t)FS_CG * ((K + 2) * (K + 2) + D * D);
+}
+
 __global__ __launch_bounds__(256) void fine_search_bwd_kernel(const float* __restrict__ datt,
                                                              const float* __restrict__ soft_att,
                                                              const int* __restrict__ index_all,
@@ -214,34 +221,72 @@
                                                              int C, int K, int D, float* __restrict__ dlrb,
                                                              float* __restrict__ drefb) {
     extern __shared__ float sm[];
-    const int b = blockIdx.y, c = blockIdx.x;
-    const int P = K * K, BS = K + 2, R1 = D - 2;
+    const int b = blockIdx.y, c0 = blockIdx.x * FS_CG, nc = min(FS_CG, C - c0);
+    const int P = K * K, BS = K + 2, R1 = D - 2, QQ = BS * BS, DD = D * D;
     float* s_da = sm;
     float* s_at = s_da + P;
     float* s_iq = s_at + P;
     float* s_ik = s_iq + P;
-    int* s_ix = reinterpret_cast<int*>(s_ik + P);
-    float* s_q = reinterpret_cast<float*>(s_ix + P);
-    float* s_k = s_q + BS * BS;
-    int* s_ry = reinterpret_cast<int*>(s_k + D * D);
+    int* s_ry = reinterpret_cast<int*>(s_ik + P);
     int* s_rx = s_ry + P;
     int* s_qo = s_rx + P;
-    for (int p = threadIdx.x; p < P; p += 256) {
+    int* s_st = s_qo + P;
+    int* s_ep = s_st + DD + 1;
+    int* s_eq = s_ep + 9 * P;
+    int* s_sc = s_eq + 9 * P;
+    float* s_q = reinterpret_cast<float*>(s_sc + 256);
+    float* s_k = s_q + FS_CG * QQ;
+    const int t = threadIdx.x;
+    for (int p = t; p < P; p += 256) {
         const int ix = index_all[(long)b * P + p];
         s_da[p] = datt[(long)b * P + p];
         s_at[p] = soft_att[(long)b * P + p];
         s_iq[p] = invq[(long)b * P + p];
         s_ik[p] = invk[(long)b * R1 * R1 + ix];
-        s_ix[p] = ix;
         s_ry[p] = ix / R1;
         s_rx[p] = ix % R1;
         s_qo[p] = (p / K) * BS + (p % K);
     }
-    for (int i = threadIdx.x; i < BS * BS; i += 256) s_q[i] = lrb[((long)b * C + c) * BS * BS + i];
-    for (int i = threadIdx.x; i < D * D; i += 256) s_k[i] = refb[((long)b * C + c) * D * D + i];
+    const long qbase = ((long)b * C + c0) * QQ, kbase = ((long)b * C + c0) * DD;
+    for (int i = t; i < nc * QQ; i += 256) s_q[i] = lrb[qbase + i];
+    for (int i = t; i < nc * DD; i += 256) s_k[i] = refb[kbase + i];
     __syncthreads();
-    for (int i = threadIdx.x; i < BS * BS; i += 256) {
+    const int per = (DD + 255) / 256;
+    const int i0 = min(t * per, DD), i1 = min(i0 + per, DD);
+    int cnt = 0;
+    for (int i = i0; i < i1; ++i) {
+        const int v = i / D, u = i % D;
+        for (int p = 0; p < P; ++p) {
+            const int kyy = v - s_ry[p], kxx = u - s_rx[p];
+            cnt += (kyy >= 0 && kyy <= 2 && kxx >= 0 && kxx <= 2) ? 1 : 0;
+        }
+    }
+    s_sc[t] = cnt;
+    __syncthreads();
+    for (int o = 1; o < 256; o <<= 1) {
+        const int add = t >= o ? s_sc[t - o] : 0;
+        __syncthreads();
+        s_sc[t] += add;
+        __syncthreads();
+    }
+    int pos = s_sc[t] - cnt;
+    for (int i = i0; i < i1; ++i) {
+        const int v = i / D, u = i % D;
+        s_st[i] = pos;
+        for (int p = 0; p < P; ++p) {
+            const int kyy = v - s_ry[p], kxx = u - s_rx[p];
+            if (kyy < 0 || kyy > 2 || kxx < 0 || kxx > 2) continue;
+            s_ep[pos] = p;
+            s_eq[pos] = s_qo[p] + kyy * BS + kxx;
+            ++pos;
+        }
+    }
+    if (t == 255) s_st[DD] = s_sc[255];
+    __syncthreads();
+    for (int idx = t; idx < nc * QQ; idx += 256) {
+        const int c = idx / QQ, i = idx - c * QQ;
         const int y = i / BS, x = i % BS;
+        const float* kc = s_k + c * DD;
         float s = 0.f;
 #pragma unroll
         for (int k = 0; k < 9; ++k) {
@@ -249,21 +294,21 @@
             if (pyy < 0 || pyy >= K || pxx < 0 || pxx >= K) continue;
             const int p = pyy * K + pxx;
             const int ry = s_ry[p], rx = s_rx[p];
-            const float kv = s_k[(ry + k / 3) * D + rx + k % 3];
-            s += s_da[p] * s_iq[p] * (kv * s_ik[p] - s_at[p] * s_q[i] * s_iq[p]);
-        }
-        dlrb[((long)b * C + c) * BS * BS + i] = s;
-    }
-    for (int i = threadIdx.x; i < D * D; i += 256) {
-        const int v = i / D, u = i % D;
+            const float kv = kc[(ry + k / 3) * D + rx + k % 3];
+            s += s_da[p] * s_iq[p] * (kv * s_ik[p] - s_at[p] * s_q[idx] * s_iq[p]);
+        }
+        dlrb[qbase + idx] = s;
+    }
+    for (int idx = t; idx < nc * DD; idx += 256) {
+        const int c = idx / DD, i = idx - c * DD;
+        const float* qc = s_q + c * QQ;
         float s = 0.f;
-        for (int p = 0; p < P; ++p) {
-            const int kyy = v - s_ry[p], kxx = u - s_rx[p];
-            if (kyy < 0 || kyy > 2 || kxx < 0 || kxx > 2) continue;
-            const float qv = s_q[s_qo[p] + kyy * BS + kxx];
-            s += s_da[p] * s_ik[p] * (qv * s_iq[p] - s_at[p] * s_k[i] * s_ik[p]);
-        }
-        drefb[((long)b * C + c) * D * D + i] = s;
+        for (int e = s_st[i]; e < s_st[i + 1]; ++e) {
+            const int p = s_ep[e];
+            const float qv = qc[s_eq[e]];
+            s += s_da[p] * s_ik[p] * (qv * s_iq[p] - s_at[p] * s_k[idx] * s_ik[p]);
+        }
+        drefb[kbase + idx] = s;
     }
 }
 
@@ -305,15 +350,83 @@
     g.wgt = (top * (1.f - ly) + bot * ly);
 }
 
+__device__ __forceinline__ int tr_sources(const TrGeom& g, int (&src)[9], float (&mult)[9]) {
+    int nsrc = 0;
+#pragma unroll
+    for (int j = 0; j < 9; ++j) { src[j] = 0; mult[j] = 0.f; }
+#pragma unroll
+    for (int k = 0; k < 9; ++k) {
+        int m = 0;
+        bool first = g.src[k] >= 0;
+#pragma unroll
+        for (int q = 0; q < 9; ++q) {
+            const bool same = g.src[q] == g.src[k];
+            m += same ? 1 : 0;
+            if (q < k && same) first = false;
+        }
+        if (first) {
+#pragma unroll
+            for (int j = 0; j <= k; ++j)
+                if (j == nsrc) { src[j] = g.src[k]; mult[j] = (float)m; }
+            ++nsrc;
+        }
+    }
+#pragma unroll
+    for (int j = 1; j < 9; ++j)
+        if (j >= nsrc) src[j] = src[0];
+    return nsrc;
+}
+
+__device__ __forceinline__ long uniform_off(long v) {
+    const unsigned lo = __builtin_amdgcn_readfirstlane((unsigned)v), hi = __builtin_amdgcn_readfirstlane((unsigned)((unsigned long)v >> 32));
+    return (long)(((unsigned long)hi << 32) | lo);
+}
+template <typename T>
+__device__ __forceinline__ T* at_bytes(T* p, unsigned bytes) {
+    return reinterpret_cast<T*>(reinterpret_cast<char*>(const_cast<typename std::remove_const<T>::type*>(p)) + bytes);
+}
+
 constexpr int TR_CG = 8;
 
-__global__ __launch_bounds__(256) void transfer_fwd_kernel(const float* __restrict__ feat, int C, int H, int W,
-                                                          const int* __restrict__ y1, const int* __restrict__ x1,
-                                                          const int* __restrict__ index_all,
+struct TrLevel {
+    const float* feat;
+    const float* dout;
+    float* out;
+    float* dfeat;
+    unsigned long long* dfacc;
+    const unsigned* amax;
+    float* dA;
+    long io_ns;
+    int C, H, W, s;
+    int pixb;
+    int cgrid;
+    int cpb;
+    int first;
+};
+struct TrLevels {
+    TrLevel lv[TDR_TRANSFER_MAX_LEVELS];
+    int L;
+};
+
+__device__ __forceinline__ int tr_level_of(const TrLevels& T, int bid) {
+    int l = 0;
+#pragma unroll
+    for (int q = 1; q < TDR_TRANSFER_MAX_LEVELS; ++q)
+        if (q < T.L && bid >= T.lv[q].first) l = q;
+    return l;
+}
+
+__global__ __launch_bounds__(256) void transfer_fwd_kernel(const TrLevels T, const int* __restrict__ y1,
+                                                          const int* __restrict__ x1, const int* __restrict__ index_all,
                                                           const float* __restrict__ soft_att, int py, int px, int K,
-                                                          int side, int s, float* __restrict__ out, long out_ns) {
+                                                          int side) {
+    const TrLevel& V = T.lv[tr_level_of(T, blockIdx.x)];
+    const int C = V.C, H = V.H, W = V.W, s = V.s;
+    int r = blockIdx.x - V.first;
+    const int pb = r % V.pixb; r /= V.pixb;
+    const int cg = r % V.cgrid, n = r / V.cgrid;
     const int OW = px * K * s, OH = py * K * s;
-    const int pix = blockIdx.x * 256 + threadIdx.x, n = blockIdx.z;
+    const int pix = pb * 256 + threadIdx.x;
     if (pix >= OH * OW) return;
     const int Y = pix / OW, X = pix % OW;
     const int by = Y / (K * s), bx = X / (K * s);
@@ -321,33 +434,27 @@
     TrGeom g;
     tr_geometry(Y - by * K * s, X - bx * K * s, b, y1, x1, index_all, soft_att, K, side, s, H, W, g);
     const long HWf = (long)H * W, HWo = (long)OH * OW;
+    int src[9];
     float mult[9];
-#pragma unroll
-    for (int k = 0; k < 9; ++k) {
-        int m = 0;
-        bool first = g.src[k] >= 0;
-#pragma unroll
-        for (int q = 0; q < 9; ++q) {
-            const bool same = g.src[q] == g.src[k];
-            m += same ? 1 : 0;
-            if (q < k && same) first = false;
-        }
-        mult[k] = first ? (float)m : 0.f;
-    }
-    const int c0 = blockIdx.y * TR_CG;
+    const int nsrc = tr_sources(g, src, mult);
+    const int c0 = cg * TR_CG;
+    const float* f0 = V.feat + ((long)n * C + c0) * HWf;
     float accs[TR_CG];
 #pragma unroll
-    for (int i = 0; i < TR_CG; ++i) {
-        const float* f = feat + ((long)n * C + min(c0 + i, C - 1)) * HWf;
-        float acc = 0.f;
-#pragma unroll
-        for (int k = 0; k < 9; ++k)
-            if (mult[k] != 0.f) acc += mult[k] * f[g.src[k]];
-        accs[i] = acc;
-    }
+    for (int i = 0; i < TR_CG; ++i) accs[i] = 0.f;
+#pragma unroll
+    for (int j = 0; j < 9; ++j)
+        if (j < nsrc) {
+            float v[TR_CG];
+#pragma unroll
+            for (int i = 0; i < TR_CG; ++i) v[i] = *at_bytes(f0 + uniform_off((long)min(i, C - 1 - c0) * HWf), (unsigned)src[j] * 4u);
+#pragma unroll
+            for (int i = 0; i < TR_CG; ++i) accs[i] += mult[j] * v[i];
+        }
+    float* o = V.out + (long)n * V.io_ns + (long)c0 * HWo + pix;
 #pragma unroll
     for (int i = 0; i < TR_CG; ++i)
-        if (c0 + i < C) out[(long)n * out_ns + (long)(c0 + i) * HWo + pix] = accs[i] * g.inv_cnt * g.wgt;
+        if (c0 + i < C) o[(long)i * HWo] = accs[i] * g.inv_cnt * g.wgt;
 }
 
 __global__ __launch_bounds__(256) void absmax_bits_kernel(const float* __restrict__ x, long x_ns, long per4, int N,
@@ -371,19 +478,54 @@
     for (long i = blockIdx.x * 256L + threadIdx.x; i < n; i += (long)gridDim.x * 256) out[i] += (float)((double)acc[i] * inv);
 }
 
+template <bool FIXED, bool FULL>
+__device__ __forceinline__ void tr_bwd_group(const float* f0, const float* d0, float* df0, unsigned long long* dq0, int nv,
+                                             long HWf, long HWo, int pix, int nsrc, const unsigned (&boff)[9],
+                                             const float (&mult)[9], float coef, float inv_cnt, float fscale, float& da) {
+    float go[TR_CG], acc[TR_CG];
+#pragma unroll
+    for (int i = 0; i < TR_CG; ++i) {
+        const float x = (d0 + uniform_off((long)(FULL ? i : min(i, nv - 1)) * HWo))[pix];
+        go[i] = (FULL || i < nv) ? x : 0.f;
+        acc[i] = 0.f;
+    }
+#pragma unroll
+    for (int j = 0; j < 9; ++j)
+        if (j < nsrc) {
+            float v[TR_CG];
+#pragma unroll
+            for (int i = 0; i < TR_CG; ++i) v[i] = *at_bytes(f0 + uniform_off((long)(FULL ? i : min(i, nv - 1)) * HWf), boff[j]);
+#pragma unroll
+            for (int i = 0; i < TR_CG; ++i) acc[i] += mult[j] * v[i];
+        }
+#pragma unroll
+    for (int i = 0; i < TR_CG; ++i)
+        if (FULL || i < nv) da += go[i] * acc[i] * inv_cnt;
+#pragma unroll
+    for (int j = 0; j < 9; ++j)
+        if (j < nsrc) {
+#pragma unroll
+            for (int i = 0; i < TR_CG; ++i)
+                if (FULL || i < nv) {
+                    const float gv = go[i] * coef;
+                    if (FIXED) atomicAdd(at_bytes(dq0 + uniform_off((long)i * HWf), 2u * boff[j]), (unsigned long long)__float2ll_rn(gv * mult[j] * fscale));
+                    else atomicAdd(at_bytes(df0 + uniform_off((long)i * HWf), boff[j]), gv * mult[j]);
+                }
+        }
+}
+
 template <bool FIXED>
-__global__ __launch_bounds__(256) void transfer_bwd_kernel(const float* __restrict__ dout, long dout_ns,
-                                                          const float* __restrict__ feat, int C, int H, int W,
-                                                          const int* __restrict__ y1, const int* __restrict__ x1,
-                                                          const int* __restrict__ index_all,
+__global__ __launch_bounds__(256, FIXED ? 4 : 8) void transfer_bwd_kernel(const TrLevels T, const int* __restrict__ y1,
+                                                          const int* __restrict__ x1, const int* __restrict__ index_all,
                                                           const float* __restrict__ soft_att, int py, int px, int K,
-                                                          int side, int s, int cpb , int N,
-                                                          const unsigned* __restrict__ amax_bits,
-                                                          unsigned long long* __restrict__ dfacc ,
-                                                          float* __restrict__ dfeat ,
-                                                          float* __restrict__ dA ) {
+                                                          int side, int N) {
+    const TrLevel& V = T.lv[tr_level_of(T, blockIdx.x)];
+    const int C = V.C, H = V.H, W = V.W, s = V.s;
+    int r = blockIdx.x - V.first;
+    const int pb = r % V.pixb; r /= V.pixb;
+    const int cg = r % V.cgrid, n = r / V.cgrid;
     const int OW = px * K * s, OH = py * K * s;
-    const int pix = blockIdx.x * 256 + threadIdx.x, n = blockIdx.z;
+    const int pix = pb * 256 + threadIdx.x;
     if (pix >= OH * OW) return;
     const int Y = pix / OW, X = pix % OW;
     const int by = Y / (K * s), bx = X / (K * s);
@@ -392,69 +534,65 @@
     tr_geometry(Y - by * K * s, X - bx * K * s, b, y1, x1, index_all, soft_att, K, side, s, H, W, g);
     const long HWf = (long)H * W, HWo = (long)OH * OW;
     const float coef = g.inv_cnt * g.wgt;
+    int src[9];
     float mult[9];
-#pragma unroll
-    for (int k = 0; k < 9; ++k) {
-        int m = 0;
-        bool first = g.src[k] >= 0;
-#pragma unroll
-        for (int q = 0; q < 9; ++q) {
-            const bool same = g.src[q] == g.src[k];
-            m += same ? 1 : 0;
-            if (q < k && same) first = false;
-        }
-        mult[k] = first ? (float)m : 0.f;
-    }
+    const int nsrc = tr_sources(g, src, mult);
+    unsigned boff[9];
+#pragma unroll
+    for (int j = 0; j < 9; ++j) boff[j] = (unsigned)src[j] * 4u;
     float da = 0.f;
-    const int c0 = blockIdx.y * cpb, c1 = min(c0 + cpb, C);
-    const float fscale = FIXED ? ldexpf(1.f, fixed_shift(amax_bits[0])) : 1.f;
-    for (int c = c0; c < c1; ++c) {
-        const float* f = feat + ((long)n * C + c) * HWf;
-        const float go = dout[(long)n * dout_ns + (long)c * HWo + pix];
-        float acc = 0.f;
-        const float gv = go * coef;
-#pragma unroll
-        for (int k = 0; k < 9; ++k)
-            if (mult[k] > 0.f) {
-                acc += mult[k] * f[g.src[k]];
-                if (FIXED) atomicAdd(&dfacc[((long)n * C + c) * HWf + g.src[k]], (unsigned long long)__float2ll_rn(gv * mult[k] * fscale));
-                else atomicAdd(&dfeat[((long)n * C + c) * HWf + g.src[k]], gv * mult[k]);
-            }
-        da += go * acc * g.inv_cnt;
-    }
-    dA[((long)blockIdx.y * N + n) * HWo + pix] = da;
-}
-
-__global__ __launch_bounds__(64) void transfer_datt_kernel(const float* __restrict__ dA, int py, int px, int K, int s,
-                                                          int chunks, long chunk_stride, float* __restrict__ datt) {
+    const int c0 = cg * V.cpb, c1 = min(c0 + V.cpb, C);
+    const float fscale = FIXED ? ldexpf(1.f, fixed_shift(V.amax[0])) : 1.f;
+    for (int cb = c0; cb < c1; cb += TR_CG) {
+        const int nv = min(TR_CG, c1 - cb);
+        const float* f0 = V.feat + ((long)n * C + cb) * HWf;
+        const float* d0 = V.dout + (long)n * V.io_ns + (long)cb * HWo;
+        const long o0 = ((long)n * C + cb) * HWf;
+        if (nv == TR_CG)
+            tr_bwd_group<FIXED, true>(f0, d0, V.dfeat + o0, V.dfacc + o0, nv, HWf, HWo, pix, nsrc, boff, mult, coef, g.inv_cnt, fscale, da);
+        else
+            tr_bwd_group<FIXED, false>(f0, d0, V.dfeat + o0, V.dfacc + o0, nv, HWf, HWo, pix, nsrc, boff, mult, coef, g.inv_cnt, fscale, da);
+    }
+    V.dA[((long)cg * N + n) * HWo + pix] = da;
+}
+
+__global__ __launch_bounds__(64) void transfer_datt_kernel(const TrLevels T, int py, int px, int K, int N,
+                                                          float* __restrict__ datt) {
     const int b = blockIdx.x, e = blockIdx.y;
     const int P = py * px, n = b / P, by = (b % P) / px, bx = b % px;
     const int i = e / K, j = e % K;
-    const int OW = px * K * s, OH = py * K * s, KS = K * s;
-    const int ylo = max((i - 1) * s, 0), yhi = min((i + 2) * s, KS);
-    const int xlo = max((j - 1) * s, 0), xhi = min((j + 2) * s, KS);
-    const int nw = xhi - xlo, tot = (yhi - ylo) * nw;
-    float acc = 0.f;
-    for (int t = threadIdx.x; t < tot; t += 64) {
-        const int Yl = ylo + t / nw, Xl = xlo + t % nw;
-        const float fy = fmaxf(((float)Yl + 0.5f) / (float)s - 0.5f, 0.f), fx = fmaxf(((float)Xl + 0.5f) / (float)s - 0.5f, 0.f);
-        const int yy0 = min((int)fy, K - 1), xx0 = min((int)fx, K - 1);
-        const int yy1 = min(yy0 + 1, K - 1), xx1 = min(xx0 + 1, K - 1);
-        const float ly = fy - (float)yy0, lx = fx - (float)xx0;
-        float wgt = 0.f;
-        if (yy0 == i && xx0 == j) wgt += (1.f - ly) * (1.f - lx);
-        if (yy0 == i && xx1 == j) wgt += (1.f - ly) * lx;
-        if (yy1 == i && xx0 == j) wgt += ly * (1.f - lx);
-        if (yy1 == i && xx1 == j) wgt += ly * lx;
-        if (wgt != 0.f) {
-            const long o = (long)n * OH * OW + (long)(by * KS + Yl) * OW + bx * KS + Xl;
-            float v = 0.f;
-            for (int q = 0; q < chunks; ++q) v += dA[q * chunk_stride + o];
-            acc += wgt * v;
-        }
-    }
-    acc = wave_sum(acc);
-    if (threadIdx.x == 0) datt[(long)b * K * K + e] += acc;
+    float total = datt[(long)b * K * K + e];
+    for (int l = 0; l < T.L; ++l) {
+        const TrLevel& V = T.lv[l];
+        const int s = V.s, chunks = V.cgrid;
+        const int OW = px * K * s, OH = py * K * s, KS = K * s;
+        const long chunk_stride = (long)N * OH * OW;
+        const float* dA = V.dA;
+        const int ylo = max((i - 1) * s, 0), yhi = min((i + 2) * s, KS);
+        const int xlo = max((j - 1) * s, 0), xhi = min((j + 2) * s, KS);
+        const int nw = xhi - xlo, tot = (yhi - ylo) * nw;
+        float acc = 0.f;
+        for (int t = threadIdx.x; t < tot; t += 64) {
+            const int Yl = ylo + t / nw, Xl = xlo + t % nw;
+            const float fy = fmaxf(((float)Yl + 0.5f) / (float)s - 0.5f, 0.f), fx = fmaxf(((float)Xl + 0.5f) / (float)s - 0.5f, 0.f);
+            const int yy0 = min((int)fy, K - 1), xx0 = min((int)fx, K - 1);
+            const int yy1 = min(yy0 + 1, K - 1), xx1 = min(xx0 + 1, K - 1);
+            const float ly = fy - (float)yy0, lx = fx - (float)xx0;
+            float wgt = 0.f;
+            if (yy0 == i && xx0 == j) wgt += (1.f - ly) * (1.f - lx);
+            if (yy0 == i && xx1 == j) wgt += (1.f - ly) * lx;
+            if (yy1 == i && xx0 == j) wgt += ly * (1.f - lx);
+            if (yy1 == i && xx1 == j) wgt += ly * lx;
+            if (wgt != 0.f) {
+                const long o = (long)n * OH * OW + (long)(by * KS + Yl) * OW + bx * KS + Xl;
+                float v = 0.f;
+                for (int q = 0; q < chunks; ++q) v += dA[q * chunk_stride + o];
+                acc += wgt * v;
+            }
+        }
+        total += wave_sum(acc);
+    }
+    if (threadIdx.x == 0) datt[(long)b * K * K + e] = total;
 }
 
 inline int grid1d(long total, int cap = 8192) {
@@ -541,10 +679,92 @@
                                    const float* refb, const float* invq, const float* invk, int B, int C, int K, int D,
                                    float* dlrb, float* drefb, void* stream) {
     TDR_REQUIRE(datt && soft_att && index_all && lrb && refb && invq && invk && dlrb && drefb, "tdr_fine_search_bwd: null pointer");
-    const size_t lds = (size_t)(8 * K * K + (K + 2) * (K + 2) + D * D) * sizeof(float);
-    hipLaunchKernelGGL(fine_search_bwd_kernel, dim3(C, B), dim3(256), lds, (hipStream_t)stream, datt, soft_att, index_all, lrb,
-                       refb, invq, invk, C, K, D, dlrb, drefb);
+    TDR_REQUIRE(B > 0 && C > 0 && K > 0 && D > 2, "tdr_fine_search_bwd: bad shape");
+    const size_t lds = fine_search_bwd_lds_words(K, D) * sizeof(float);
+    TDR_REQUIRE(lds <= 64 * 1024, "tdr_fine_search_bwd: K=%d, D=%d need %zu bytes of LDS (64 KiB a workgroup)", K, D, lds);
+    hipLaunchKernelGGL(fine_search_bwd_kernel, dim3(tdr_cdiv(C, FS_CG), B), dim3(256), lds, (hipStream_t)stream, datt, soft_att,
+                       index_all, lrb, refb, invq, invk, C, K, D, dlrb, drefb);
     TDR_LAUNCH_CHECK("fine_search_bwd");
+    return TDR_OK;
+}
+
+static int tdr_transfer_chunks(int N, int C, int py, int px, int K, int s) {
+    const long opix = (long)py * K * s * px * K * s;
+    const long pix_blocks = ((opix + 255) / 256) * N;
+    long chunks = (2048 + pix_blocks - 1) / pix_blocks;
+    if (chunks > C / TR_CG) chunks = C / TR_CG;
+    if (chunks < 1) chunks = 1;
+    return (int)chunks;
+}
+
+extern "C" int64_t tdr_transfer_ws_floats(int N, int C, int H, int W, int py, int px, int K, int s) {
+    const int64_t opix = (int64_t)py * K * s * px * K * s;
+    return (int64_t)tdr_transfer_chunks(N, C, py, px, K, s) * N * opix + 4 + 2 * (int64_t)N * C * H * W;
+}
+
+static int64_t tr_level_ws(const TdrTransferLevel& l, int N, int py, int px, int K, int deterministic) {
+    const int64_t opix = (int64_t)py * K * l.s * px * K * l.s;
+    const int64_t w = deterministic ? tdr_transfer_ws_floats(N, l.C, l.H, l.W, py, px, K, l.s)
+                                    : (int64_t)tdr_transfer_chunks(N, l.C, py, px, K, l.s) * N * opix;
+    return w + (w & 1);
+}
+
+extern "C" int64_t tdr_transfer_levels_ws_floats(const TdrTransferLevel* lv, int L, int N, int py, int px, int K,
+                                                 int deterministic) {
+    if (!lv || L < 1 || L > TDR_TRANSFER_MAX_LEVELS) return 0;
+    int64_t w = 0;
+    for (int l = 0; l < L; ++l) w += tr_level_ws(lv[l], N, py, px, K, deterministic);
+    return w;
+}
+
+static int tr_fill(TrLevels& T, const char* who, const TdrTransferLevel* lv, int L, int N, int py, int px, int K, bool bwd,
+                   long* blocks) {
+    TDR_REQUIRE(lv && L >= 1 && L <= TDR_TRANSFER_MAX_LEVELS, "%s: 1 .. %d levels", who, TDR_TRANSFER_MAX_LEVELS);
+    TDR_REQUIRE(N > 0 && py > 0 && px > 0 && K > 0, "%s: bad shape", who);
+    long first = 0;
+    T.L = L;
+    for (int l = 0; l < L; ++l) {
+        const TdrTransferLevel& d = lv[l];
+        TrLevel& V = T.lv[l];
+        TDR_REQUIRE(d.feat && d.io && (!bwd || d.dfeat), "%s: null pointer (level %d)", who, l);
+        TDR_REQUIRE(d.C > 0 && d.H > 0 && d.W > 0 && d.s > 0, "%s: bad shape (level %d)", who, l);
+        const long opix = (long)py * K * d.s * px * K * d.s;
+        TDR_REQUIRE(opix < (1L << 31) && (long)d.H * d.W < (1L << 29), "%s: level %d is too large (32-bit byte offsets inside a channel plane)", who, l);
+        V = TrLevel{};
+        V.feat = d.feat;
+        V.dout = d.io;
+        V.out = d.io;
+        V.dfeat = d.dfeat;
+        V.io_ns = (long)d.io_ns;
+        V.C = d.C; V.H = d.H; V.W = d.W; V.s = d.s;
+        V.pixb = (int)((opix + 255) / 256);
+        if (bwd) {
+            const int chunks = tdr_transfer_chunks(N, d.C, py, px, K, d.s);
+            V.cpb = tdr_cdiv(d.C, chunks);
+            V.cgrid = tdr_cdiv(d.C, V.cpb);
+        } else {
+            V.cpb = TR_CG;
+            V.cgrid = tdr_cdiv(d.C, TR_CG);
+        }
+        V.first = (int)first;
+        first += (long)V.pixb * V.cgrid * N;
+        TDR_REQUIRE(first < (1L << 31), "%s: more than 2^31 workgroups", who);
+    }
+    *blocks = first;
+    return TDR_OK;
+}
+
+extern "C" int tdr_transfer_fwd_levels(const TdrTransferLevel* lv, int L, int N, const int* y1, const int* x1,
+                                       const int* index_all, const float* soft_att, int py, int px, int K, int side,
+                                       void* stream) {
+    TDR_REQUIRE(y1 && x1 && index_all && soft_att, "tdr_transfer_fwd_levels: null pointer");
+    TrLevels T;
+    long blocks = 0;
+    const int rc = tr_fill(T, "tdr_transfer_fwd_levels", lv, L, N, py, px, K, false, &blocks);
+    if (rc != TDR_OK) return rc;
+    hipLaunchKernelGGL(transfer_fwd_kernel, dim3((unsigned)blocks), dim3(256), 0, (hipStream_t)stream, T, y1, x1, index_all,
+                       soft_att, py, px, K, side);
+    TDR_LAUNCH_CHECK("transfer_fwd");
     return TDR_OK;
 }
 
@@ -552,62 +772,66 @@
                                 const int* index_all, const float* soft_att, int py, int px, int K, int side, int s,
                                 float* out, int64_t out_ns, void* stream) {
     TDR_REQUIRE(feat && y1 && x1 && index_all && soft_att && out, "tdr_transfer_fwd: null pointer");
-    const long opix = (long)py * K * s * px * K * s;
-    hipLaunchKernelGGL(transfer_fwd_kernel, dim3((unsigned)((opix + 255) / 256), tdr_cdiv(C, TR_CG), N), dim3(256), 0,
-                       (hipStream_t)stream, feat, C, H, W, y1, x1, index_all, soft_att, py, px, K, side, s, out, (long)out_ns);
-    TDR_LAUNCH_CHECK("transfer_fwd");
-    return TDR_OK;
-}
-
-static int tdr_transfer_chunks(int N, int C, int py, int px, int K, int s) {
-    const long opix = (long)py * K * s * px * K * s;
-    const long pix_blocks = ((opix + 255) / 256) * N;
-    long chunks = (1024 + pix_blocks - 1) / pix_blocks;
-    if (chunks > C / 8) chunks = C / 8;
-    if (chunks < 1) chunks = 1;
-    return (int)chunks;
-}
-
-extern "C" int64_t tdr_transfer_ws_floats(int N, int C, int H, int W, int py, int px, int K, int s) {
-    const int64_t opix = (int64_t)py * K * s * px * K * s;
-    return (int64_t)tdr_transfer_chunks(N, C, py, px, K, s) * N * opix + 4 + 2 * (int64_t)N * C * H * W;
+    TdrTransferLevel lv{feat, C, H, W, s, out, out_ns, nullptr};
+    return tdr_transfer_fwd_levels(&lv, 1, N, y1, x1, index_all, soft_att, py, px, K, side, stream);
+}
+
+extern "C" int tdr_transfer_bwd_levels(const TdrTransferLevel* lv, int L, int N, const int* y1, const int* x1,
+                                       const int* index_all, const float* soft_att, int py, int px, int K, int side,
+                                       int deterministic, float* datt, float* ws, void* stream) {
+    TDR_REQUIRE(y1 && x1 && index_all && soft_att && datt && ws, "tdr_transfer_bwd_levels: null pointer");
+    TrLevels T;
+    long blocks = 0;
+    const int rc = tr_fill(T, "tdr_transfer_bwd_levels", lv, L, N, py, px, K, true, &blocks);
+    if (rc != TDR_OK) return rc;
+    hipStream_t st = (hipStream_t)stream;
+    float* seg = ws;
+    for (int l = 0; l < L; ++l) {
+        TrLevel& V = T.lv[l];
+        const long opix = (long)py * K * V.s * px * K * V.s;
+        V.dA = seg;
+        if (deterministic) {
+            TDR_REQUIRE(opix % 4 == 0 && V.io_ns % 4 == 0 && (reinterpret_cast<uintptr_t>(V.dout) & 15) == 0,
+                        "tdr_transfer_bwd: dout must be 16-byte aligned");
+            char* tail = reinterpret_cast<char*>(seg + (long)tdr_transfer_chunks(N, V.C, py, px, K, V.s) * N * opix);
+            tail += (8 - reinterpret_cast<uintptr_t>(tail) % 8) % 8;
+            unsigned* amax = reinterpret_cast<unsigned*>(tail);
+            const long nacc = (long)N * V.C * V.H * V.W;
+            if (hipMemsetAsync(tail, 0, 8 + (size_t)nacc * 8, st) != hipSuccess) {
+                tdr_set_error("tdr_transfer_bwd: hipMemsetAsync failed");
+                return TDR_ERR_HIP;
+            }
+            const long per4 = (long)V.C * opix / 4;
+            hipLaunchKernelGGL(absmax_bits_kernel, dim3(grid1d(per4, 512), N), dim3(256), 0, st, V.dout, V.io_ns, per4, N, amax);
+            V.amax = amax;
+            V.dfacc = reinterpret_cast<unsigned long long*>(tail + 8);
+        }
+        seg += tr_level_ws(lv[l], N, py, px, K, deterministic);
+    }
+    if (!deterministic) {
+        hipLaunchKernelGGL(transfer_bwd_kernel<false>, dim3((unsigned)blocks), dim3(256), 0, st, T, y1, x1, index_all, soft_att, py,
+                           px, K, side, N);
+    } else {
+        hipLaunchKernelGGL(transfer_bwd_kernel<true>, dim3((unsigned)blocks), dim3(256), 0, st, T, y1, x1, index_all, soft_att, py,
+                           px, K, side, N);
+        for (int l = 0; l < L; ++l) {
+            const TrLevel& V = T.lv[l];
+            const long nacc = (long)N * V.C * V.H * V.W;
+            hipLaunchKernelGGL(fixed_to_float_kernel, dim3(grid1d(nacc, 4096)), dim3(256), 0, st,
+                               reinterpret_cast<const long long*>(V.dfacc), nacc, V.amax, V.dfeat);
+        }
+    }
+    hipLaunchKernelGGL(transfer_datt_kernel, dim3(N * py * px, K * K), dim3(64), 0, st, T, py, px, K, N, datt);
+    TDR_LAUNCH_CHECK("transfer_bwd");
+    return TDR_OK;
 }
 
 extern "C" int tdr_transfer_bwd(const float* dout, int64_t dout_ns, const float* feat, int N, int C, int H, int W,
                                 const int* y1, const int* x1, const int* index_all, const float* soft_att, int py, int px,
                                 int K, int side, int s, int deterministic, float* dfeat, float* datt, float* ws, void* stream) {
     TDR_REQUIRE(dout && feat && y1 && x1 && index_all && soft_att && dfeat && datt && ws, "tdr_transfer_bwd: null pointer");
-    const long opix = (long)py * K * s * px * K * s;
-    hipStream_t st = (hipStream_t)stream;
-    const int chunks = tdr_transfer_chunks(N, C, py, px, K, s);
-    const int cpb = tdr_cdiv(C, chunks);
-    float* dA = ws;
-    const dim3 grid((unsigned)((opix + 255) / 256), tdr_cdiv(C, cpb), N);
-    if (!deterministic) {
-        hipLaunchKernelGGL(transfer_bwd_kernel<false>, grid, dim3(256), 0, st, dout, (long)dout_ns, feat, C, H, W, y1, x1, index_all,
-                           soft_att, py, px, K, side, s, cpb, N, (const unsigned*)nullptr, (unsigned long long*)nullptr, dfeat, dA);
-    } else {
-        TDR_REQUIRE(opix % 4 == 0 && dout_ns % 4 == 0 && (reinterpret_cast<uintptr_t>(dout) & 15) == 0, "tdr_transfer_bwd: dout must be 16-byte aligned");
-        char* tail = reinterpret_cast<char*>(ws + (long)chunks * N * opix);
-        tail += (8 - reinterpret_cast<uintptr_t>(tail) % 8) % 8;
-        unsigned* amax = reinterpret_cast<unsigned*>(tail);
-        unsigned long long* acc = reinterpret_cast<unsigned long long*>(tail + 8);
-        const long nacc = (long)N * C * H * W;
-        if (hipMemsetAsync(tail, 0, 8 + (size_t)nacc * 8, st) != hipSuccess) {
-            tdr_set_error("tdr_transfer_bwd: hipMemsetAsync failed");
-            return TDR_ERR_HIP;
-        }
-        const long per4 = (long)C * opix / 4;
-        hipLaunchKernelGGL(absmax_bits_kernel, dim3(grid1d(per4, 512), N), dim3(256), 0, st, dout, (long)dout_ns, per4, N, amax);
-        hipLaunchKernelGGL(transfer_bwd_kernel<true>, grid, dim3(256), 0, st, dout, (long)dout_ns, feat, C, H, W, y1, x1, index_all,
-                           soft_att, py, px, K, side, s, cpb, N, amax, acc, (float*)nullptr, dA);
-        hipLaunchKernelGGL(fixed_to_float_kernel, dim3(grid1d(nacc, 4096)), dim3(256), 0, st, reinterpret_cast<const long long*>(acc),
-                           nacc, amax, dfeat);
-    }
-    hipLaunchKernelGGL(transfer_datt_kernel, dim3(N * py * px, K * K), dim3(64), 0, st, ws, py, px, K, s, tdr_cdiv(C, cpb),
-                       (long)N * opix, datt);
-    TDR_LAUNCH_CHECK("transfer_bwd");
-    return TDR_OK;
+    TdrTransferLevel lv{feat, C, H, W, s, const_cast<float*>(dout), dout_ns, dfeat};
+    return tdr_transfer_bwd_levels(&lv, 1, N, y1, x1, index_all, soft_att, py, px, K, side, deterministic, datt, ws, stream);
 }
 
 __global__ __launch_bounds__(256) void absmax_bits_any_kernel(const float* __restrict__ x, long x_ns, long per, unsigned* __restrict__ slot) {
diff --git a/textualdegremoval_amd/engine.py b/textualdegremoval_amd/engine.py
--- a/textualdegremoval_amd/engine.py
+++ b/textualdegremoval_amd/engine.py
@@ -534,14 +534,9 @@
     index_all, soft_att = K.fine_argmax(fdots, finvq, finvk, N * P, Kk * Kk, R1 * R1)
     if not keep:
         lq4 = ref4 = lrb = refb = wp = fdots = finvq = finvk = None
-    warp = []
-    for lvl in range(L):
-        s = 2 ** (L - 1 - lvl)
-        warp.append(K.transfer_fwd(ref_feats[lvl], y1, x1, index_all, soft_att, geo.py, geo.px, Kk, side, s,
-                                   out=None if outs is None else outs[lvl]))
-        if not keep:
-            ref_feats[lvl] = None
-    if not keep:
+    warp = K.transfer_fwd_levels(ref_feats, y1, x1, index_all, soft_att, geo.py, geo.px, Kk, side, outs=outs)
+    if not keep:
+        ref_feats[:] = [None] * L
         return warp, None
     saved = (lrb, refb, finvq, finvk, index, y1, x1, index_all, soft_att)
     return warp, saved
@@ -553,15 +548,11 @@
     L = len(ref_feats)
     dev = lq4.device
     datt = torch.zeros(N * P, Kk * Kk, dtype=torch.float32, device=dev)
-    for lvl in range(L):
-        s = 2 ** (L - 1 - lvl)
-        K.transfer_bwd(dwarp[lvl], ref_feats[lvl], y1, x1, index_all, soft_att, geo.py, geo.px, Kk, side, s,
-                       dref_out[lvl], datt)
+    K.transfer_bwd_levels(dwarp, ref_feats, y1, x1, index_all, soft_att, geo.py, geo.px, Kk, side, dref_out, datt)
     dlrb, drefb = K.fine_search_bwd(datt, soft_att, index_all, lrb, refb, finvq, finvk, Kk, side)
     K.scatter_ref_block(drefb, dref_out[L - 1], y1, x1, P, side)
     _, Cc, H, W = lq4.shape
-    dlq4 = K.lr_blocks_bwd(dlrb, N, Cc, H, W, geo.py, geo.px, Kk, Kk)
-    K.copy_rows(dlq4, Cc * H * W, dlq_out, Cc * H * W, N, Cc * H * W)
+    K.lr_blocks_bwd(dlrb, N, Cc, H, W, geo.py, geo.px, Kk, Kk, out=dlq_out)
 
 
 def _pad_into(src, dst_view):
diff --git a/textualdegremoval_amd/kernels.py b/textualdegremoval_amd/kernels.py
--- a/textualdegremoval_amd/kernels.py
+++ b/textualdegremoval_amd/kernels.py
@@ -1198,8 +1198,9 @@
     return blk
 
 
-def lr_blocks_bwd(dblk, N, Cc, H, W, py, px, ky, kx):
-    dfeat = torch.empty(N, Cc, H, W, dtype=torch.float32, device=dblk.device)
+def lr_blocks_bwd(dblk, N, Cc, H, W, py, px, ky, kx, out=None):
+    dfeat = out if out is not None else torch.empty(N, Cc, H, W, dtype=torch.float32, device=dblk.device)
+    assert tuple(dfeat.shape) == (N, Cc, H, W) and dfeat.is_contiguous()
     check(_lib.load().tdr_lr_blocks_bwd(dblk.data_ptr(), N, Cc, H, W, py, px, ky, kx, dfeat.data_ptr(), _stream()),
           'tdr_lr_blocks_bwd')
     return dfeat
@@ -1281,6 +1282,46 @@
                                        x1.data_ptr(), index_all.data_ptr(), soft_att.data_ptr(), py, px, K, side, s,
                                        1 if DETERMINISTIC else 0, dfeat.data_ptr(), datt.data_ptr(), ws.data_ptr(), _stream()),
           'tdr_transfer_bwd')
+
+
+def _transfer_levels(feats, ios, dfeats, K, py, px):
+    L = len(feats)
+    lv = (_lib.TdrTransferLevel * L)()
+    for l, f in enumerate(feats):
+        N, Cc, H, W = f.shape
+        s = 2 ** (L - 1 - l)
+        assert f.is_contiguous() and tuple(ios[l].shape) == (N, Cc, py * K * s, px * K * s)
+        lv[l].feat, lv[l].C, lv[l].H, lv[l].W, lv[l].s = f.data_ptr(), Cc, H, W, s
+        lv[l].io, lv[l].io_ns = ios[l].data_ptr(), _dense_nchw(ios[l])
+        if dfeats is not None:
+            assert tuple(dfeats[l].shape) == (N, Cc, H, W) and dfeats[l].is_contiguous()
+            lv[l].dfeat = dfeats[l].data_ptr()
+    return lv
+
+
+def transfer_fwd_levels(feats, y1, x1, index_all, soft_att, py, px, K, side, outs=None):
+    N = feats[0].shape[0]
+    L = len(feats)
+    outs = [None] * L if outs is None else list(outs)
+    for l, f in enumerate(feats):
+        if outs[l] is None:
+            s = 2 ** (L - 1 - l)
+            outs[l] = torch.empty(N, f.shape[1], py * K * s, px * K * s, dtype=torch.float32, device=f.device)
+    lv = _transfer_levels(feats, outs, None, K, py, px)
+    check(_lib.load().tdr_transfer_fwd_levels(lv, L, N, y1.data_ptr(), x1.data_ptr(), index_all.data_ptr(), soft_att.data_ptr(),
+                                              py, px, K, side, _stream()), 'tdr_transfer_fwd_levels')
+    return outs
+
+
+def transfer_bwd_levels(douts, feats, y1, x1, index_all, soft_att, py, px, K, side, dfeats, datt):
+    N = feats[0].shape[0]
+    L = len(feats)
+    lv = _transfer_levels(feats, douts, dfeats, K, py, px)
+    lib = _lib.load()
+    ws = workspace(lib.tdr_transfer_levels_ws_floats(lv, L, N, py, px, K, 1 if DETERMINISTIC else 0), feats[0].device, 'transfer')
+    check(lib.tdr_transfer_bwd_levels(lv, L, N, y1.data_ptr(), x1.data_ptr(), index_all.data_ptr(), soft_att.data_ptr(), py, px, K,
+                                      side, 1 if DETERMINISTIC else 0, datt.data_ptr(), ws.data_ptr(), _stream()),
+          'tdr_transfer_bwd_levels')
 
 
 def resize_bilinear(x, Hd, Wd):
```
